# olasanni1/ETOL

Hardware: AMD Instinct MI355X
Metric: collocation-node constraint+Jacobian evals/sec, 6-state VGP N=1024 (higher is better)
Workload: dtype f64

## Files before the change

etol_amd/_lib.py:

```python
import ctypes as C
import os

import torch

_HERE = os.path.dirname(os.path.abspath(__file__))
LIB_PATH = os.path.join(_HERE, "lib", "libemi355x.so")

EMI_OK = 0
STATUS = {0: "EMI_OK", 1: "EMI_ERR_ARG", 2: "EMI_ERR_STATE", 3: "EMI_ERR_HIP",
          4: "EMI_ERR_NO_DEVICE", 5: "EMI_ERR_UNSUPPORTED", 6: "EMI_ERR_COMM"}

MODEL_POINTMASS2D, MODEL_QUADROTOR2D, MODEL_FIXEDWING12 = 0, 1, 2
MODEL_SOURCE = 100
PATH_ELLIPSE, PATH_DISC, PATH_TRACK = 0, 1, 2
PATH_REC = 8
EVAL_NODES, EVAL_DEFECT, EVAL_ALL, EVAL_NOJAC = 1, 2, 3, 4


class EmiError(RuntimeError):
    pass


class Layout(C.Structure):
    _fields_ = [("model", C.c_int), ("ns", C.c_int), ("nc", C.c_int), ("np", C.c_int),
                ("M", C.c_int), ("B", C.c_int), ("nres", C.c_int), ("nvals", C.c_int),
                ("nhess", C.c_int), ("real_bytes", C.c_int), ("px", C.c_int), ("py", C.c_int),
                ("t0", C.c_double), ("tf", C.c_double)]


class PassPlan(C.Structure):
    _fields_ = [(n, C.c_int) for n in ("one_launch", "sw", "ksplit", "ring_stages", "cpart", "cx", "mfma_workgroups", "store_mode",
                                       "block_order", "tiles16", "piece", "tail", "k_tile", "column_tiles", "k_halves")]


_P = C.c_void_p
_D = C.POINTER(C.c_double)
_I = C.POINTER(C.c_int)

SYMBOLS = {
    "emi_abi_version": (C.c_int, []),
    "emi_status_string": (C.c_char_p, [C.c_int]),
    "emi_device_count": (C.c_int, [_I]),
    "emi_lgl": (C.c_int, [C.c_int, _D, _D, _D]),
    "emi_model_dims": (C.c_int, [C.c_int, _I, _I, _I]),
    "emi_edge_ellipse": (C.c_int, [C.c_double] * 4 + [_D]),
    "emi_track_centres": (C.c_int, [C.c_int, _D, _D, _D, C.c_int, _D, _D, _D]),
    "emi_create": (C.c_int, [C.c_int, C.POINTER(_P)]),
    "emi_create_f32": (C.c_int, [C.c_int, C.POINTER(_P)]),
    "emi_destroy": (C.c_int, [_P]),
    "emi_last_error": (C.c_char_p, [_P]),
    "emi_set_stream": (C.c_int, [_P, _P]),
    "emi_get_stream": (C.c_int, [_P, C.POINTER(_P)]),
    "emi_synchronize": (C.c_int, [_P]),
    "emi_set_mesh": (C.c_int, [_P, C.c_int, _D, _D, _D, C.c_double, C.c_double]),
    "emi_set_model": (C.c_int, [_P, C.c_int, _D, C.c_int, C.c_int]),
    "emi_set_model_source": (C.c_int, [_P, C.c_char_p, C.c_char_p, C.c_int, C.c_int, C.c_int, _I, C.c_int, _D, C.c_int, C.c_int]),
    "emi_check_model_source": (C.c_int, [C.c_char_p, C.c_char_p, C.c_int, C.c_int, C.c_int, C.c_int, C.c_int, C.c_char_p, C.c_size_t]),
    "emi_kkt_factor": (C.c_int, [_P, _D, _D, C.POINTER(C.c_ubyte), C.c_double, C.POINTER(C.c_int)]),
    "emi_kkt_solve": (C.c_int, [_P, _D, C.c_int]),
    "emi_kkt_last_regularisation": (C.c_int, [_P, _D, _D]),
    "emi_kkt_factor_batch": (C.c_int, [C.c_int, C.POINTER(_P), C.POINTER(_D), C.POINTER(_D), C.POINTER(C.POINTER(C.c_ubyte)), _D, _I]),
    "emi_kkt_solve_batch": (C.c_int, [C.c_int, C.POINTER(_P), C.POINTER(_D)]),
    "emi_kkt_is_schur": (C.c_int, [_P]),
    "emi_kkt_solve_refined": (C.c_int, [_P, _D, C.c_double, C.c_int, _D, _I, _I, _I]),
    "emi_kkt_solve_refined_batch": (C.c_int, [C.c_int, C.POINTER(_P), C.POINTER(_D), _D, C.c_int, _D, _I, _I, _I]),
    "emi_kkt_lowrank": (C.c_int, [_P, C.c_int, C.POINTER(C.c_int), _D, _D, C.POINTER(C.c_int)]),
    "emi_set_batch": (C.c_int, [_P, C.c_int]),
    "emi_set_path": (C.c_int, [_P, C.c_int, C.c_int, _D, C.c_int, C.c_int]),
    "emi_set_tracks": (C.c_int, [_P, C.c_int, C.c_int, _D, _D]),
    "emi_get_layout": (C.c_int, [_P, C.POINTER(Layout)]),
    "emi_jac_structure": (C.c_int, [_P, _I, _I]),
    "emi_dev_alloc": (C.c_int, [_P, C.c_size_t, C.POINTER(_P)]),
    "emi_dev_free": (C.c_int, [_P, _P]),
    "emi_h2d": (C.c_int, [_P, _P, _P, C.c_size_t]),
    "emi_d2h": (C.c_int, [_P, _P, _P, C.c_size_t]),
    "emi_eval_dev": (C.c_int, [_P, _P, _P, _P, _P, _P, C.c_uint]),
    "emi_eval_host": (C.c_int, [_P, _D, _D, _D, _D, _D, C.c_uint]),
    "emi_hess_dev": (C.c_int, [_P, _P, _P, _P, _P, C.c_double, _P]),
    "emi_hess_host": (C.c_int, [_P, _D, _D, _D, _D, C.c_double, _D]),
    "emi_lagr_grad_dev": (C.c_int, [_P, _P, _P, _P, C.c_double, _P]),
    "emi_lagr_grad_host": (C.c_int, [_P, _D, _D, _D, C.c_double, _D]),
    "emi_kkt_certificate_dev": (C.c_int, [_P, _P, _P, _P, _P, _P, _P, C.c_double, _P, _P, C.c_int, _D, _D, _P, _P]),
    "emi_kkt_certificate_host": (C.c_int, [_P, _D, _D, _D, _D, C.c_double, _D, _D, C.c_int, _D, _D, _D, _D]),
    "emi_lagr_grad_total_dev": (C.c_int, [_P, _P, _P, _P, C.c_double, _P, _P]),
    "emi_lagr_grad_total_host": (C.c_int, [_P, _D, _D, _D, C.c_double, _D, _D]),
    "emi_kkt_certificate_total_dev": (C.c_int, [_P, _P, _P, _P, _P, _P, _P, C.c_double, _P, _P, C.c_int, _D, _D, _P, _P, _P]),
    "emi_kkt_certificate_total_host": (C.c_int, [_P, _D, _D, _D, _D, C.c_double, _D, _D, C.c_int, _D, _D, _D, _D, _D]),
    "emi_timer_start": (C.c_int, [_P]),
    "emi_timer_stop": (C.c_int, [_P, C.POINTER(C.c_float)]),
    "emi_profile_enable": (C.c_int, [_P, C.c_int]),
    "emi_profile_read": (C.c_int, [_P, C.POINTER(C.c_float), _I, C.POINTER(C.c_float), _I, C.POINTER(C.c_float), _I]),
    "emi_set_option": (C.c_int, [_P, C.c_char_p, C.c_int]),
    "emi_last_path": (C.c_int, [_P, _I]),
    "emi_plan_pass": (C.c_int, [_P, C.c_int, C.POINTER(PassPlan)]),
    "emi_last_defect_kernel": (C.c_char_p, [_P]),
    "emi_debug_pass_roles": (C.c_int, [C.c_int, C.c_int, C.c_int, C.POINTER(C.c_int), C.c_int]),
    "emi_debug_tile_order": (C.c_int, [C.c_int, C.c_int, C.c_int, C.c_int, C.c_int, C.POINTER(C.c_int), C.c_int, C.POINTER(C.c_int), C.POINTER(C.c_int), C.POINTER(C.c_int)]),
    "emi_set_delays": (C.c_int, [_P, C.c_int, C.c_int, C.c_double]),
    "emi_get_delays": (C.c_int, [_P, _I, _I, _I]),
    "emi_delay_matrix": (C.c_int, [C.c_int, C.POINTER(C.c_double), C.POINTER(C.c_double), C.c_double, C.c_double, C.c_double, C.POINTER(C.c_double)]),
    "emi_debug_tile_order2": (C.c_int, [C.c_int] * 7 + [C.POINTER(C.c_int), C.c_int, C.POINTER(C.c_int), C.POINTER(C.c_int), C.POINTER(C.c_int)]),
    "emi_comm_unique_id": (C.c_int, [_P]),
    "emi_comm_create": (C.c_int, [C.c_int, C.c_int, C.c_int, _P, C.POINTER(_P)]),
    "emi_comm_gather": (C.c_int, [_P, _P, _P, C.c_size_t, C.c_int, _P]),
    "emi_comm_destroy": (C.c_int, [_P]),
    "emi_comm_last_error": (C.c_char_p, [_P]),
}

_lib = None


def load():
    global _lib
    if _lib is not None:
        return _lib
    if not os.path.exists(LIB_PATH):
        raise EmiError(f"{LIB_PATH} is missing: run `python -c 'import __graft_entry__ as g; g.build()'` "
                       "(or `make lib`) first; there is no CPU fallback")
    lib = C.CDLL(LIB_PATH, mode=C.RTLD_GLOBAL)
    for name, (res, args) in SYMBOLS.items():
        fn = getattr(lib, name)
        fn.restype = res
        fn.argtypes = args
    _lib = lib
    return lib


def check(status, ctx=None, what=""):
    if status == EMI_OK:
        return
    lib = load()
    msg = lib.emi_status_string(status).decode()
    if ctx:
        detail = lib.emi_last_error(ctx).decode()
        if detail:
            msg += ": " + detail
    raise EmiError(f"{what or 'libemi355x'}: {STATUS.get(status, status)} ({msg})")
```

etol_amd/csrc/emi_api.hip:

```cpp
#include <hip/hip_runtime.h>

#include <algorithm>
#include <cstdarg>
#include <cstdio>
#include <cstring>
#include <string>
#include <vector>

#include "emi355x.h"
#include "emi_device_array.hpp"
#include "emi_kernels.hpp"

namespace {

using DevBuf = emi::DeviceArray<unsigned char>;

enum ProfMark { E0, E1, E2, K0, K1, K2, K3, PROF_MARKS };
struct ProfEvents {
    hipEvent_t ev[PROF_MARKS] = {};
    bool has_node = false, has_defect = false, fused = false;
    int level = 0;
};

}

struct emi_ctx_s {
    int device = 0;
    bool f32 = false;
    hipStream_t stream = nullptr;
    bool own_stream = false;
    hipStream_t stream2 = nullptr;
    hipEvent_t ev_fork = nullptr, ev_join = nullptr, ev_join2 = nullptr;
    int cu_split = 0;
    hipStream_t s_mfma = nullptr, s_node = nullptr;
    std::string err;
    std::string last_defect_kernel;

    int M = 0;
    double t0 = 0, tf = 0;
    DevBuf d_w, d_t, d_Ddiag, d_D, d_De, d_Do;
    bool symmetric = false;
    bool points_only = false;
    int allow_fused = 1;
    int sym_ct = 0;
    int sym_order = 1;
    int sym_ablate = 0;
    int small_rows = 24;
    int overlap_mode = 0;
    int node_store = -1;
    unsigned fused_attr_mask = 0;
    std::vector<double> h_tau, h_w;
    int model = -1, ns = 0, nc = 0, maximize = 0;
    double params[EMI_MAX_PARAMS] = {0};
    emi::KktWorkspace* kkt = nullptr;
    int kkt_method = 1;
    emi::RtcModel* rtc = nullptr;
    int B = 0;
    int np = 0, path_sets = 0, px = 0, py = 1;
    int np_model = 0;
    std::vector<int> pvars;
    DevBuf d_path;
    int ntracks = 0, track_sets = 0;
    DevBuf d_trkx, d_trky;
    DevBuf d_cost_part;
    DevBuf d_slab;
    DevBuf d_tile_ticket;
    DevBuf d_cost_part2;
    DevBuf d_ticket;
    int cost_in_kernel = 1;
    int sym_nst = 3;
    int sym_hs = 0;
    int sym_ctc = 0;
    int sym_bk = 0;
    int xh = 0, uh = 0, nch = 0;
    double delay_dt = 0.0;
    bool delay_dirty = true;
    DevBuf d_W;
    bool adjw_dirty = true;
    DevBuf d_adjWT;
    DevBuf d_adj_Gx;
    int adj_fold_tile = 0;
    DevBuf d_uext;
    int f32_ring_wgs = 2;
    int f32_ring = 1;
    int f32_one_launch = 0;
    int slice = 0;
    int sym_ksplit = 0;
    int sym_cpart = 0;
    int sym_gblk = 0, sym_cx = 0;
    int pass_order = -1;
    int sym_combine = 1;
    DevBuf s_X, s_U, s_RES, s_VALS, s_COST, s_LF, s_LC, s_H;
    DevBuf d_adjDT;
    bool adj_dirty = true;
    DevBuf d_adj_pvars;
    std::vector<int> adj_pvars;
    DevBuf d_adj_c;
    DevBuf d_adj_G;
    DevBuf d_adj_op;
    DevBuf s_G, s_cert, s_zl, s_zu, s_Gdel;
    hipEvent_t t_start = nullptr, t_stop = nullptr;
    int profile = 0;
    std::vector<ProfEvents> prof;
    size_t prof_used = 0;
    bool attr_set = false;

    ~emi_ctx_s() {
        (void)hipSetDevice(device);
        if (stream) (void)hipStreamSynchronize(stream);
        for (ProfEvents& pe : prof)
            for (hipEvent_t e : pe.ev)
                if (e) (void)hipEventDestroy(e);
        for (hipStream_t s : {stream2, s_mfma, s_node})
            if (s) { (void)hipStreamSynchronize(s); (void)hipStreamDestroy(s); }
        for (hipEvent_t e : {ev_join2, ev_fork, ev_join, t_start, t_stop})
            if (e) (void)hipEventDestroy(e);
        if (own_stream && stream) (void)hipStreamDestroy(stream);
        emi::rtc_destroy(rtc);
        emi::kkt_destroy(kkt);
    }
};

namespace {

int fail(emi_ctx_t c, int code, const char* fmt, ...) {
    char buf[512];
    va_list ap;
    va_start(ap, fmt);
    vsnprintf(buf, sizeof buf, fmt, ap);
    va_end(ap);
    if (c) c->err = buf;
    return code;
}

#define HIP_TRY(c, call)                                                              \
    do {                                                                              \
        hipError_t e_ = (call);                                                       \
        if (e_ != hipSuccess)                                                         \
            return fail((c), EMI_ERR_HIP, "%s failed: %s (%s:%d)", #call,             \
                        hipGetErrorString(e_), __FILE__, __LINE__);                   \
    } while (0)

#define EMI_TRY(call)              \
    do {                           \
        const int st_ = (call);    \
        if (st_) return st_;       \
    } while (0)

int ensure(emi_ctx_t c, DevBuf& b, size_t bytes) {
    HIP_TRY(c, b.reserve(bytes));
    return EMI_OK;
}

int ensure_zeroed(emi_ctx_t c, DevBuf& b, size_t bytes, hipStream_t s) {
    if (b.bytes() >= bytes) return EMI_OK;
    EMI_TRY(ensure(c, b, bytes));
    HIP_TRY(c, hipMemsetAsync(b.p, 0, bytes, s));
    return EMI_OK;
}

int upload_bytes(emi_ctx_t c, DevBuf& b, const void* src, size_t bytes) {
    EMI_TRY(ensure(c, b, bytes));
    if (bytes == 0) return EMI_OK;
    HIP_TRY(c, hipMemcpyAsync(b.p, src, bytes, hipMemcpyHostToDevice, c->stream));
    HIP_TRY(c, hipStreamSynchronize(c->stream));
    return EMI_OK;
}

int upload_real(emi_ctx_t c, DevBuf& b, const double* src, size_t n) {
    if (!c->f32) return upload_bytes(c, b, src, n * 8);
    std::vector<float> tmp(n);
    for (size_t i = 0; i < n; ++i) tmp[i] = (float)src[i];
    return upload_bytes(c, b, tmp.data(), n * 4);
}

int download_real(emi_ctx_t c, double* dst, const void* dsrc, size_t n) {
    if (!dst || n == 0) return EMI_OK;
    std::vector<float> tmp(c->f32 ? n : 0);
    HIP_TRY(c, hipMemcpyAsync(c->f32 ? (void*)tmp.data() : (void*)dst, dsrc, n * (c->f32 ? 4 : 8), hipMemcpyDeviceToHost, c->stream));
    HIP_TRY(c, hipStreamSynchronize(c->stream));
    for (size_t i = 0; i < tmp.size(); ++i) dst[i] = tmp[i];
    return EMI_OK;
}

bool overlapped_path(emi_ctx_t c) {
    if (c->f32 || !c->allow_fused || !c->symmetric || c->M <= 0 || c->model < 0) return false;
    if (c->model == EMI_MODEL_SOURCE) return emi::rtc_has_symdefect(c->rtc) && c->M % 128 == 0;
    return emi::fused_supported(c->model, c->M, c->sym_ct);
}

bool pass_takes_small_batches(emi_ctx_t c, int B) {
    if (!overlapped_path(c) || (c->overlap_mode != 0 && c->overlap_mode != 3) || c->M % 128 != 0) return false;
    if (c->rtc) return emi::rtc_pass_supported(c->rtc, B, c->M, 1, 1, 0);
    const emi::SymPlan p = emi::plan_symdefect(c->ns, B, c->M, 7, 1, c->sym_cpart, c->sym_gblk, c->sym_cx);
    return emi::pass_supported(c->model, c->ns, B, c->M, p);
}

int np_total(emi_ctx_t c) { return c->np + c->np_model; }
int nvals_of(emi_ctx_t c) { return c->ns * (c->ns + c->nc) + 2 * c->np + c->np_model * (int)c->pvars.size() + (c->ns + c->nc); }
int nres_of(emi_ctx_t c) { return c->ns + np_total(c); }
int nhess_of(emi_ctx_t c) { const int nv = c->ns + c->nc; return nv * (nv + 1) / 2; }

int ready(emi_ctx_t c) {
    if (!c) return EMI_ERR_ARG;
    if (c->M <= 0) return fail(c, EMI_ERR_STATE, "emi_set_mesh has not been called");
    if (c->model < 0) return fail(c, EMI_ERR_STATE, "emi_set_model has not been called");
    if (c->B <= 0) return fail(c, EMI_ERR_STATE, "emi_set_batch has not been called");
    if (c->np > 0 && c->path_sets != 1 && c->path_sets != c->B)
        return fail(c, EMI_ERR_STATE, "path table has %d sets, batch is %d", c->path_sets, c->B);
    if (c->ntracks > 0 && c->track_sets != 1 && c->track_sets != c->B)
        return fail(c, EMI_ERR_STATE, "track table has %d sets, batch is %d", c->track_sets, c->B);
    return EMI_OK;
}

int store_mode_for(emi_ctx_t c, int B) {
    if (c->node_store >= 0) return c->node_store;
    if ((size_t)B * (nvals_of(c) + nres_of(c)) * c->M * (c->f32 ? 4 : 8) > ((size_t)230 << 20)) return 2;
    const int tiles16 = ((B + 15) / 16) * (c->M / 128);
    if (tiles16 > 16 && tiles16 <= 32) return 0;
    return (!c->rtc && !c->f32) ? 1 : 0;
}

struct PassPlan {
    bool one_launch = false;
    emi::SymPlan sym;
    int tiles16 = 0;
    int store_mode = 0;
    int mfma_first = 0;
};

PassPlan plan_pass(emi_ctx_t c, int B, bool jac) {
    PassPlan p;
    p.tiles16 = ((B + 15) / 16) * (c->M / 128);
    p.store_mode = store_mode_for(c, B);
    const bool auto_mode = c->overlap_mode == 0;
    if (!((c->overlap_mode == 3 || auto_mode) && jac) || c->M % 128 != 0) return p;
    const bool auto_ct = auto_mode && (c->sym_ct == 0 || c->sym_ct == 4);
    const int gblk = (c->sym_gblk == 0 && c->sym_cpart == 0 && B > 2048 && B % 256 == 0) ? 2 : c->sym_gblk;
    const int gblk_first = (auto_ct || c->rtc) ? gblk : c->sym_gblk;
    int ct = c->sym_ct;
    const bool deep_base = auto_ct && !c->rtc && c->sym_bk == 0 && c->sym_ksplit == 0 && c->sym_nst == 3;
    const bool deep_mid = deep_base && c->ns % 2 == 0 && c->ns > 2 && p.tiles16 >= 49 && p.tiles16 < 128;
    const bool deep_small = deep_base && c->ns % 2 == 0 && c->ns > 2 && p.tiles16 >= 33 && p.tiles16 < 49;
    if (c->rtc) ct = (p.store_mode == 2 && emi::rtc_pass_sw_large(c->rtc) == 2) ? 6 : 7;
    else if (auto_ct) ct = (p.tiles16 < 128 && !deep_mid) ? 7 : 6;
    emi::SymPlan plan = emi::plan_symdefect(c->ns, B, c->M, ct, 1, c->sym_cpart, gblk_first, c->sym_cx);
    if (plan.ring1) plan = emi::plan_symdefect(c->ns, B, c->M, 5, 1, c->sym_cpart, c->sym_gblk, c->sym_cx);
    int ks_want = c->sym_ksplit;
    if (ks_want == 0 && auto_ct && !deep_mid && !deep_small) ks_want = plan.tiles * 4 <= 256 ? 4 : (plan.tiles * 2 <= 512 ? 2 : 1);
    if (ks_want > 1) {
        const int ct_now = plan.sw == c->ns ? 5 : (plan.sw == 2 ? 6 : (plan.sw == 3 ? 8 : 7));
        plan = emi::plan_symdefect(c->ns, B, c->M, ct_now, ks_want, c->sym_cpart, c->rtc ? gblk : c->sym_gblk, c->sym_cx);
    } else {
        plan.ks = 1;
    }
    plan.nst = c->rtc ? 3 : c->sym_nst;
    const bool deep_large = auto_ct && !c->rtc && c->sym_bk == 0 && c->sym_nst == 3 && c->pass_order < 0 && p.tiles16 >= 208 && p.tiles16 <= 1024;
    const bool deep_band = auto_ct && !c->rtc && c->sym_bk == 0 && c->sym_nst == 3 && c->pass_order < 0 && c->ns % 2 == 0 && c->ns > 2 &&
                           p.tiles16 >= 144 && p.tiles16 < 208;
    const int bk_want = c->sym_bk ? c->sym_bk : ((deep_mid || deep_small || deep_large || deep_band) ? 16 : 8);
    if (bk_want == 16 && !c->rtc && plan.ks == 1 && (plan.sw == 1 || plan.sw == 2) && plan.nst == 3) plan.bk = 16;
    const bool wide_large = auto_ct && c->sym_ctc == 0 && B > 2048 && B % 256 == 0 && c->sym_cpart == 0;
    const int ctc_want = c->sym_ctc ? c->sym_ctc : (wide_large ? 2 : 1);
    if (ctc_want == 2 && !c->rtc && plan.ks == 1 && plan.sw == 2 && plan.nst == 3 && c->M % 256 == 0) {
        const int bk_keep = plan.bk;
        plan = emi::plan_symdefect(c->ns, B, c->M, 6, 1, c->sym_cpart, gblk_first, (wide_large && c->sym_cx == 0) ? 1 : c->sym_cx, bk_keep, 2);
        plan.ks = 1;
        plan.nst = 3;
        plan.bk = bk_keep;
    }
    const int hs_want = c->sym_hs ? c->sym_hs : 1;
    if (hs_want == 2 && !c->rtc && plan.ks == 1 && plan.ct == 1 && (plan.sw == 1 || plan.sw == 2) && plan.nst == 3 &&
        ((c->M / 2) / plan.bk) % 4 == 0)
        plan.hs = 2;
    p.sym = plan;
    p.mfma_first = c->pass_order >= 0 ? c->pass_order
                                      : (deep_band ? 150 : (p.tiles16 < 208 ? 1 : (p.tiles16 < 384 ? 125 : (p.tiles16 < 768 ? 110 : 0))));
    p.one_launch = c->rtc ? emi::rtc_pass_supported(c->rtc, B, c->M, plan.sw, plan.ks, p.store_mode)
                          : emi::pass_supported(c->model, c->ns, B, c->M, plan);
    return p;
}

int plan_piece(emi_ctx_t c, int B) {
    const long long cap = ((0xFFFFFFFFLL / ((long long)c->ns * c->M * 8)) / 256) * 256;
    int piece = 0;
    if (c->slice > 0) { if (B > 2 * c->slice) piece = c->slice; }
    else if (B > 2048) piece = (int)std::min<long long>(cap > 0 ? cap : 256, B - B % 256);
    return piece >= B ? 0 : piece;
}

struct Launch { int first, B; };
struct PassIO { const void *X, *U; void *RES, *VALS, *COST; };

PassIO io_at(emi_ctx_t c, const PassIO& io, int first) {
    const size_t row = (size_t)first * c->M * (c->f32 ? 4 : 8);
    return PassIO{(const char*)io.X + row * c->ns, (const char*)io.U + row * c->nc, (char*)io.RES + row * nres_of(c),
                  io.VALS ? (char*)io.VALS + row * nvals_of(c) : nullptr, (char*)io.COST + (size_t)first * (c->f32 ? 4 : 8)};
}

template <typename T>
void fill_node_args(emi_ctx_t c, Launch L, emi::NodeArgs<T>& a, const PassIO& io) {
    a.X = (const T*)io.X;
    a.U = (const T*)io.U;
    a.RES = (T*)io.RES;
    a.VALS = (T*)io.VALS;
    a.cost_part = (T*)c->d_cost_part.p + (size_t)L.first * emi::node_chunks(c->M);
    a.cost = (T*)io.COST;
    a.cost_ticket = nullptr;
    a.w = (const T*)c->d_w.p;
    a.node_t = (const T*)c->d_t.p;
    a.Ddiag = (const T*)c->d_Ddiag.p;
    a.path = (const T*)c->d_path.p + (c->path_sets > 1 ? (size_t)L.first * c->np * EMI_PATH_REC : 0);
    a.track_x = (const T*)c->d_trkx.p + (c->track_sets > 1 ? (size_t)L.first * c->ntracks * c->M : 0);
    a.track_y = (const T*)c->d_trky.p + (c->track_sets > 1 ? (size_t)L.first * c->ntracks * c->M : 0);
    a.M = c->M;
    a.B = L.B;
    a.np = np_total(c);
    a.nres = nres_of(c);
    a.nvals = nvals_of(c);
    a.path_sets = c->path_sets;
    a.track_sets = c->track_sets;
    a.ntracks = c->ntracks;
    a.px = c->px;
    a.py = c->py;
    a.store_mode = store_mode_for(c, L.B);
    a.h = (T)((c->tf - c->t0) / 2.0);
    a.sgn = c->maximize ? T(-1) : T(1);
    for (int i = 0; i < EMI_MAX_PARAMS; ++i) a.P.p[i] = (T)c->params[i];
}

void delay_matrix(const std::vector<double>& tau, const std::vector<double>& w, double t0, double tf, double delay, double* W) {
    const int M = (int)tau.size();
    std::vector<double> lam(M);
    for (int j = 0; j < M; ++j) lam[j] = ((j & 1) ? -1.0 : 1.0) * std::sqrt(w[j]);
    const double hh = (tf - t0) / 2.0;
    for (int k = 0; k < M; ++k) {
        double ts = t0 + hh * (tau[k] + 1.0) - delay;
        if (ts < t0) ts = t0;
        const double x = (ts - t0) / hh - 1.0;
        double* row = W + (size_t)k * M;
        int hit = -1;
        for (int j = 0; j < M; ++j)
            if (x == tau[j]) hit = j;
        if (ts <= t0) hit = 0;
        if (hit >= 0) {
            for (int j = 0; j < M; ++j) row[j] = j == hit ? 1.0 : 0.0;
            continue;
        }
        double den = 0.0;
        for (int j = 0; j < M; ++j) {
            row[j] = lam[j] / (x - tau[j]);
            den += row[j];
        }
        for (int j = 0; j < M; ++j) row[j] /= den;
    }
}

int ensure_delay_matrices(emi_ctx_t c) {
    if (!c->delay_dirty) return EMI_OK;
    const int M = c->M, nd = std::max(c->xh - 1, c->uh);
    std::vector<double> W((size_t)nd * M * M);
    for (int d = 0; d < nd; ++d) delay_matrix(c->h_tau, c->h_w, c->t0, c->tf, (d + 1) * c->delay_dt, W.data() + (size_t)d * M * M);
    EMI_TRY(upload_real(c, c->d_W, W.data(), W.size()));
    c->delay_dirty = false;
    return EMI_OK;
}

int extend_controls(emi_ctx_t c, const void* dX, const void* dU_free, const void** dU_ext) {
    if (c->f32) return fail(c, EMI_ERR_UNSUPPORTED, "delayed values: f64 contexts only");
    if (c->points_only) return fail(c, EMI_ERR_STATE, "delayed values need a collocation mesh (this context holds a points-only mesh)");
    const int M = c->M, ncf = c->nc - c->nch;
    HIP_TRY(c, hipSetDevice(c->device));
    if (!c->attr_set) {
        HIP_TRY(c, emi::defect_f64_set_attr());
        c->attr_set = true;
    }
    int st;
    if ((st = ensure_delay_matrices(c))) return st;
    const size_t row = (size_t)M * 8;
    if ((st = ensure(c, c->d_uext, (size_t)c->B * c->nc * row))) return st;
    HIP_TRY(c, hipMemsetAsync(c->d_uext.p, 0, (size_t)c->B * c->nc * row, c->stream));
    HIP_TRY(c, hipMemcpy2DAsync(c->d_uext.p, (size_t)c->nc * row, dU_free, (size_t)ncf * row, (size_t)ncf * row, c->B, hipMemcpyDeviceToDevice, c->stream));
    double* base = (double*)c->d_uext.p + (size_t)ncf * M;
    for (int i = 1; i < c->xh; ++i) {
        emi::DefectArgs a{(const double*)dX, (const double*)c->d_W.p + (size_t)(i - 1) * M * M, base + (size_t)(i - 1) * c->ns * M,
                          c->B * c->ns, M, c->ns, c->nc};
        HIP_TRY(c, emi::launch_defect_f64(a, c->stream));
    }
    base += (size_t)std::max(c->xh - 1, 0) * c->ns * M;
    for (int i = 1; i <= c->uh; ++i) {
        emi::DefectArgs a{(const double*)dU_free, (const double*)c->d_W.p + (size_t)(i - 1) * M * M, base + (size_t)(i - 1) * ncf * M,
                          c->B * ncf, M, ncf, c->nc};
        HIP_TRY(c, emi::launch_defect_f64(a, c->stream));
    }
    *dU_ext = c->d_uext.p;
    return EMI_OK;
}

struct OptionRow {
    const char* name;
    int emi_ctx_s::*member;
    bool (*accepts)(int);
    int (*stored)(int);
    const char* message;
};
template <int LO, int HI> bool within(int v) { return v >= LO && v <= HI; }
template <int... VS> bool one_of(int v) { return ((v == VS) || ...); }
bool any_value(int) { return true; }
bool at_least_0(int v) { return v >= 0; }
bool whole_tiles(int v) { return v >= 0 && v % 16 == 0; }
int as_given(int v) { return v; }
int as_flag(int v) { return v != 0; }
int ring_wgs(int v) { return v == 1 ? 1 : 2; }
int block_order(int v) { return v < 0 ? -1 : (v >= 100 ? v : (v != 0)); }

const OptionRow OPTIONS[] = {
    {"overlap", &emi_ctx_s::allow_fused, any_value, as_flag, nullptr},
    {"fused", &emi_ctx_s::allow_fused, any_value, as_flag, nullptr},
    {"sym_ct", &emi_ctx_s::sym_ct, within<0, 8>, as_given,
     "sym_ct must be 0..8 (0/4 = chosen from the batch, 3 = LDS-DMA ring, 5..8 = state-split ring with SW = NS/2/1/3)"},
    {"small_rows", &emi_ctx_s::small_rows, at_least_0, as_given, "small_rows must be >= 0 (0 disables the skinny defect kernel)"},
    {"sym_order", &emi_ctx_s::sym_order, any_value, as_flag, nullptr},
    {"f32_ring", &emi_ctx_s::f32_ring, any_value, as_flag, nullptr},
    {"f32_ring_wgs", &emi_ctx_s::f32_ring_wgs, any_value, ring_wgs, nullptr},
    {"f32_one_launch", &emi_ctx_s::f32_one_launch, any_value, as_flag, nullptr},
    {"slice", &emi_ctx_s::slice, whole_tiles, as_given, "slice must be 0 (never) or a multiple of 16 instances"},
    {"pass_order", &emi_ctx_s::pass_order, any_value, block_order, nullptr},
    {"sym_ablate", &emi_ctx_s::sym_ablate, any_value, as_given, nullptr},
    {"adj_fold_tile", &emi_ctx_s::adj_fold_tile, within<0, 2>, as_given, "adj_fold_tile must be 0 (by size), 1 (48 x 64) or 2 (96 x 128)"},
    {"cost_in_kernel", &emi_ctx_s::cost_in_kernel, any_value, as_flag, nullptr},
    {"sym_nst", &emi_ctx_s::sym_nst, one_of<3, 4>, as_given, "sym_nst must be 3 or 4"},
    {"sym_hs", &emi_ctx_s::sym_hs, within<0, 2>, as_given, "sym_hs must be 0 (by batch size), 1 or 2"},
    {"sym_ctc", &emi_ctx_s::sym_ctc, within<0, 2>, as_given, "sym_ctc must be 0 (by batch size), 1 or 2"},
    {"sym_bk", &emi_ctx_s::sym_bk, one_of<0, 8, 16>, as_given, "sym_bk must be 0 (by batch size), 8 or 16"},
    {"sym_cpart", &emi_ctx_s::sym_cpart, one_of<-1, 0, 1, 2, 4, 8>, as_given, "sym_cpart must be -1 (plain order), 0 (by mesh size), 1, 2, 4 or 8"},
    {"sym_gblk", &emi_ctx_s::sym_gblk, within<0, 64>, as_given, "sym_gblk must be 0 (off) .. 64 instance groups per super-block"},
    {"sym_cx", &emi_ctx_s::sym_cx, within<0, 64>, as_given, "sym_cx must be 0 (default) .. 64 column tiles per block"},
    {"sym_combine", &emi_ctx_s::sym_combine, any_value, as_flag, nullptr},
    {"sym_ksplit", &emi_ctx_s::sym_ksplit, one_of<0, 1, 2, 4, 8>, as_given, "sym_ksplit must be 0 (by batch size), 1, 2, 4 or 8"},
    {"node_store", &emi_ctx_s::node_store, within<-1, 3>, as_given,
     "node_store must be -1 (by size), 0 (plain), 1 (write-through sc1), 2 (non-temporal) or 3 (nt sc1; the one-launch pass only)"},
    {"overlap_mode", &emi_ctx_s::overlap_mode, within<0, 3>, as_given,
     "overlap_mode must be 0 (by batch size), 1 (one stream), 2 (two streams) or 3 (one launch)"},
};


int need_stream2(emi_ctx_t c) {
    if (c->stream2) return EMI_OK;
    if (hipStreamCreateWithFlags(&c->stream2, hipStreamNonBlocking) != hipSuccess) {
        c->stream2 = nullptr;
        return fail(c, EMI_ERR_HIP, "cannot create the second stream of the two-stream pass");
    }
    return EMI_OK;
}

enum class Form {
    PassF64,
    TwoKernelF64,
    PassF32,
    TwoStreamF32,
    Sequential,
};
struct FormChoice {
    Form form = Form::Sequential;
    bool small = false;
    PassPlan plan;
    bool overlapped() const { return form == Form::PassF64 || form == Form::TwoKernelF64; }
};

FormChoice choose_form(emi_ctx_t c, Launch L, unsigned flags) {
    const bool nodes = flags & EMI_EVAL_NODES, defect = flags & EMI_EVAL_DEFECT, jac = !(flags & EMI_EVAL_NOJAC);
    FormChoice ch;
    ch.small = defect && !c->f32 && L.B > 0 && L.B * c->ns <= c->small_rows && emi::defect_small_supported(L.B * c->ns) &&
               !(nodes && jac && pass_takes_small_batches(c, L.B));
    if (nodes && defect && !ch.small && overlapped_path(c)) {
        ch.plan = plan_pass(c, L.B, jac);
        ch.form = ch.plan.one_launch ? Form::PassF64 : Form::TwoKernelF64;
    } else if (c->f32 && nodes && defect && jac && !c->rtc && c->allow_fused) {
        if ((c->overlap_mode == 3 || (c->overlap_mode == 0 && c->f32_one_launch)) && emi::pass_f32_supported(c->model, L.B * c->ns, c->M, L.B))
            ch.form = Form::PassF32;
        else if (c->overlap_mode == 2 && emi::defect_f32_mfma_supported(c->M))
            ch.form = Form::TwoStreamF32;
    }
    return ch;
}

int next_prof_record(emi_ctx_t c, ProfEvents** out) {
    if (c->prof_used == c->prof.size()) c->prof.emplace_back();
    ProfEvents& pe = c->prof[c->prof_used];
    for (hipEvent_t& e : pe.ev)
        if (!e) HIP_TRY(c, hipEventCreate(&e));
    ++c->prof_used;
    *out = &pe;
    return EMI_OK;
}

constexpr unsigned AT1 = 1u << 1, AT2 = 1u << 2, AT3 = 1u << 3, AT_ANY = AT1 | AT2 | AT3;
int prof_mark(emi_ctx_t c, ProfEvents* pe, ProfMark which, unsigned levels, hipStream_t s) {
    if (pe && pe->level > 0 && ((levels >> pe->level) & 1u)) HIP_TRY(c, hipEventRecord(pe->ev[which], s));
    return EMI_OK;
}

const char* const NAME_PASS_F32 = "emi_pass_f32_kernel (MFMA + node roles, one launch)";
const char* const NAME_RING1_F64 = "emi_symdefect_ring_f64_kernel";
const char* name_defect_f32(emi_ctx_t c, bool mfma) {
    return !mfma ? "emi_defect_f32_kernel" : (c->f32_ring ? "emi_defect_f32_ring_kernel" : "emi_defect_f32_mfma_kernel");
}
const char* name_defect_f64(bool small) { return small ? "emi_defect_small_f64_kernel" : "emi_defect_f64_kernel"; }
std::string name_pass_f64(const emi::SymPlan& plan) {
    return "emi_pass_f64_kernel<SW=" + std::to_string(plan.sw) + "> (MFMA + node roles, one launch" +
           (plan.ks > 1 ? ", " + std::to_string(plan.ks) + " K slices per tile" : "") + ")" +
           (plan.bk == 16 ? " [K tiles of 16]" : "") + (plan.ct == 2 ? " [128-column tiles]" : "") + (plan.hs == 2 ? " [K range in two halves per workgroup]" : "");
}
std::string name_symdefect(emi_ctx_t c, const emi::SymPlan& plan, bool in_kernel_combine) {
    if (plan.ring1) return c->sym_ct == 1 || c->sym_ct == 2 ? "emi_symdefect_f64_kernel" : NAME_RING1_F64;
    return "emi_symdefect_ring2_f64_kernel<SW=" + std::to_string(plan.sw) + ">" +
           (plan.ks > 1 ? " x" + std::to_string(plan.ks) + (in_kernel_combine ? " K slices (in-kernel combine)" : " K slices + emi_symdefect_combine_kernel") : "");
}

emi::SymDefectArgs sym_defect_args(emi_ctx_t c, Launch L, const PassIO& io) {
    emi::SymDefectArgs sa;
    sa.X = (const double*)io.X;
    sa.U = (const double*)io.U;
    sa.RES = (double*)io.RES;
    sa.node_t = (const double*)c->d_t.p;
    sa.De = (const double*)c->d_De.p;
    sa.Do = (const double*)c->d_Do.p;
    sa.M = c->M;
    sa.B = L.B;
    sa.nres = nres_of(c);
    sa.h = (c->tf - c->t0) / 2.0;
    sa.order = c->sym_order;
    sa.ablate = c->sym_ablate;
    sa.ksplit = 1;
    sa.slab = nullptr;
    sa.tile_ticket = nullptr;
    sa.cpart = sa.cx = 0;
    sa.mfma_first = 0;
    for (int i = 0; i < EMI_MAX_PARAMS; ++i) sa.P.p[i] = c->params[i];
    return sa;
}

emi::DefectArgsF32 defect_args_f32(emi_ctx_t c, Launch L, const PassIO& io) {
    return emi::DefectArgsF32{(const float*)io.X, (const float*)c->d_D.p, (float*)io.RES, L.B * c->ns, c->M, c->ns, nres_of(c)};
}

int form_pass_f64(emi_ctx_t c, Launch L, const PassIO& io, const PassPlan& pp, ProfEvents* pe) {
    const emi::SymPlan& plan = pp.sym;
    emi::SymDefectArgs sa = sym_defect_args(c, L, io);
    emi::NodeArgs<double> na;
    fill_node_args(c, L, na, io);
    sa.mfma_first = pp.mfma_first;
    sa.cpart = plan.cpart;
    sa.cx = plan.cx;
    if (plan.ks > 1) {
        EMI_TRY(ensure(c, c->d_slab, plan.slab_bytes));
        EMI_TRY(ensure_zeroed(c, c->d_tile_ticket, (size_t)plan.tiles * 4, c->stream));
        sa.ksplit = plan.ks;
        sa.slab = (double*)c->d_slab.p;
        sa.tile_ticket = (unsigned*)c->d_tile_ticket.p;
    }
    EMI_TRY(ensure_zeroed(c, c->d_ticket, (size_t)L.B * 4, c->stream));
    na.cost_ticket = (unsigned*)c->d_ticket.p;
    EMI_TRY(prof_mark(c, pe, K0, AT_ANY, c->stream));
    if (c->rtc) HIP_TRY(c, emi::rtc_launch_pass(c->rtc, sa, na, plan.sw, c->stream));
    else HIP_TRY(c, emi::launch_pass(c->model, sa, na, c->stream, plan));
    EMI_TRY(prof_mark(c, pe, K1, AT_ANY, c->stream));
    if (pe) pe->level = -1;
    c->last_defect_kernel = name_pass_f64(plan);
    return EMI_OK;
}

int launch_symdefect_f64(emi_ctx_t c, Launch L, emi::SymDefectArgs& sa, hipStream_t s) {
    if (c->rtc) {
        HIP_TRY(c, emi::rtc_launch_symdefect(c->rtc, sa, s));
        c->last_defect_kernel = NAME_RING1_F64;
        return EMI_OK;
    }
    const emi::SymPlan plan = emi::plan_symdefect(c->ns, L.B, c->M, c->sym_ct, c->sym_ksplit, c->sym_cpart, c->sym_gblk, c->sym_cx);
    if (plan.slab_bytes) EMI_TRY(ensure(c, c->d_slab, plan.slab_bytes));
    sa.ksplit = plan.ring1 ? 1 : plan.ks;
    sa.slab = (double*)c->d_slab.p;
    sa.cpart = plan.cpart;
    sa.cx = plan.cx;
    if (sa.ksplit > 1 && c->sym_combine) {
        EMI_TRY(ensure_zeroed(c, c->d_tile_ticket, (size_t)plan.tiles * 4, s));
        sa.tile_ticket = (unsigned*)c->d_tile_ticket.p;
    }
    const unsigned bit = 1u << c->sym_ct;
    HIP_TRY(c, emi::launch_symdefect(c->model, sa, s, !(c->fused_attr_mask & bit), c->sym_ct, plan));
    c->fused_attr_mask |= bit;
    c->last_defect_kernel = name_symdefect(c, plan, sa.tile_ticket != nullptr);
    return EMI_OK;
}

int form_two_kernel_f64(emi_ctx_t c, Launch L, const PassIO& io, bool jac, ProfEvents* pe) {
    emi::SymDefectArgs sa = sym_defect_args(c, L, io);
    emi::NodeArgs<double> na;
    fill_node_args(c, L, na, io);
    const bool two = c->overlap_mode != 1;
    const bool split = two && c->cu_split > 0;
    if (two && !split) EMI_TRY(need_stream2(c));
    hipStream_t s1 = split ? c->s_mfma : c->stream;
    hipStream_t s2 = split ? c->s_node : (two ? c->stream2 : c->stream);
    if (two) {
        HIP_TRY(c, hipEventRecord(c->ev_fork, c->stream));
        HIP_TRY(c, hipStreamWaitEvent(s2, c->ev_fork, 0));
        if (split) HIP_TRY(c, hipStreamWaitEvent(s1, c->ev_fork, 0));
    }
    EMI_TRY(prof_mark(c, pe, K0, AT1 | AT2, s1));
    EMI_TRY(launch_symdefect_f64(c, L, sa, s1));
    EMI_TRY(prof_mark(c, pe, K1, AT1 | AT2, s1));
    if (c->cost_in_kernel) {
        EMI_TRY(ensure_zeroed(c, c->d_ticket, (size_t)L.B * 4, s2));
        na.cost_ticket = (unsigned*)c->d_ticket.p;
    }
    EMI_TRY(prof_mark(c, pe, K2, AT1 | AT3, s2));
    if (c->rtc && jac && na.store_mode == 2 && c->M % 2 == 0) HIP_TRY(c, emi::rtc_launch_nodes_nt(c->rtc, na, s2));
    else if (c->rtc) HIP_TRY(c, emi::rtc_launch_nodes<double>(c->rtc, na, jac, false, s2));
    else HIP_TRY(c, emi::launch_nodes<double>(c->model, na, jac, false, s2));
    EMI_TRY(prof_mark(c, pe, K3, AT1 | AT3, s2));
    if (!c->cost_in_kernel) HIP_TRY(c, emi::launch_cost_finish<double>(na.cost_part, na.cost, L.B, emi::node_chunks(c->M), na.sgn * na.h, s2));
    if (two) {
        HIP_TRY(c, hipEventRecord(c->ev_join, s2));
        HIP_TRY(c, hipStreamWaitEvent(c->stream, c->ev_join, 0));
        if (split) {
            HIP_TRY(c, hipEventRecord(c->ev_join2, s1));
            HIP_TRY(c, hipStreamWaitEvent(c->stream, c->ev_join2, 0));
        }
    }
    EMI_TRY(prof_mark(c, pe, E1, AT1, c->stream));
    EMI_TRY(prof_mark(c, pe, E2, AT1, c->stream));
    return EMI_OK;
}

int form_pass_f32(emi_ctx_t c, Launch L, const PassIO& io, ProfEvents* pe) {
    emi::NodeArgs<float> na;
    fill_node_args(c, L, na, io);
    const size_t rowb = (size_t)c->M * 4;
    HIP_TRY(c, hipMemset2DAsync(io.RES, (size_t)nres_of(c) * rowb, 0, (size_t)c->ns * rowb, L.B, c->stream));
    EMI_TRY(ensure_zeroed(c, c->d_ticket, (size_t)L.B * 4, c->stream));
    na.cost_ticket = (unsigned*)c->d_ticket.p;
    EMI_TRY(prof_mark(c, pe, K0, AT_ANY, c->stream));
    HIP_TRY(c, emi::launch_pass_f32(c->model, defect_args_f32(c, L, io), na, c->pass_order >= 0 ? c->pass_order : 0, c->stream));
    EMI_TRY(prof_mark(c, pe, K1, AT_ANY, c->stream));
    if (pe) { pe->level = -1; pe->fused = true; }
    c->last_defect_kernel = NAME_PASS_F32;
    return EMI_OK;
}

int form_two_stream_f32(emi_ctx_t c, Launch L, const PassIO& io, ProfEvents* pe) {
    emi::NodeArgs<float> pre, full;
    PassIO values_only = io;
    values_only.VALS = nullptr;
    fill_node_args(c, L, pre, values_only);
    fill_node_args(c, L, full, io);
    EMI_TRY(ensure(c, c->d_cost_part2, (size_t)L.B * emi::node_chunks(c->M) * 4));
    EMI_TRY(need_stream2(c));
    pre.cost_part = (float*)c->d_cost_part2.p;
    pre.np = 0;
    const bool fork_late = c->f32_ring_wgs == 1;
    if (!fork_late) {
        HIP_TRY(c, hipEventRecord(c->ev_fork, c->stream));
        HIP_TRY(c, hipStreamWaitEvent(c->stream2, c->ev_fork, 0));
    }
    HIP_TRY(c, emi::launch_nodes<float>(c->model, pre, false, true, c->stream));
    if (fork_late) {
        HIP_TRY(c, hipEventRecord(c->ev_fork, c->stream));
        HIP_TRY(c, hipStreamWaitEvent(c->stream2, c->ev_fork, 0));
    }
    EMI_TRY(prof_mark(c, pe, K0, AT1 | AT2, c->stream));
    HIP_TRY(c, emi::launch_defect_f32_mfma(defect_args_f32(c, L, io), c->stream, c->f32_ring, c->f32_ring_wgs));
    EMI_TRY(prof_mark(c, pe, K1, AT1 | AT2, c->stream));
    c->last_defect_kernel = name_defect_f32(c, true);
    EMI_TRY(prof_mark(c, pe, K2, AT1 | AT3, c->stream2));
    HIP_TRY(c, emi::launch_nodes<float>(c->model, full, true, false, c->stream2));
    EMI_TRY(prof_mark(c, pe, K3, AT1 | AT3, c->stream2));
    HIP_TRY(c, emi::launch_cost_finish<float>(full.cost_part, full.cost, L.B, emi::node_chunks(c->M), full.sgn * full.h, c->stream2));
    HIP_TRY(c, hipEventRecord(c->ev_join, c->stream2));
    HIP_TRY(c, hipStreamWaitEvent(c->stream, c->ev_join, 0));
    if (pe) pe->fused = true;
    EMI_TRY(prof_mark(c, pe, E1, AT1, c->stream));
    EMI_TRY(prof_mark(c, pe, E2, AT1, c->stream));
    return EMI_OK;
}

template <typename T>
int launch_nodes_alone(emi_ctx_t c, Launch L, const PassIO& io, bool jac) {
    emi::NodeArgs<T> a;
    fill_node_args(c, L, a, io);
    if (c->rtc) HIP_TRY(c, emi::rtc_launch_nodes<T>(c->rtc, a, jac, true, c->stream));
    else HIP_TRY(c, emi::launch_nodes<T>(c->model, a, jac, true, c->stream));
    HIP_TRY(c, emi::launch_cost_finish<T>(a.cost_part, a.cost, L.B, emi::node_chunks(c->M), a.sgn * a.h, c->stream));
    return EMI_OK;
}

int form_sequential(emi_ctx_t c, Launch L, const PassIO& io, unsigned flags, bool small, ProfEvents* pe) {
    const bool jac = !(flags & EMI_EVAL_NOJAC);
    if (flags & EMI_EVAL_NODES) EMI_TRY(c->f32 ? launch_nodes_alone<float>(c, L, io, jac) : launch_nodes_alone<double>(c, L, io, jac));
    EMI_TRY(prof_mark(c, pe, E1, AT_ANY, c->stream));
    if ((flags & EMI_EVAL_DEFECT) && c->f32) {
        const bool mfma = emi::defect_f32_mfma_supported(c->M) && c->allow_fused;
        if (mfma) HIP_TRY(c, emi::launch_defect_f32_mfma(defect_args_f32(c, L, io), c->stream, c->f32_ring, c->f32_ring_wgs));
        else HIP_TRY(c, emi::launch_defect_f32(defect_args_f32(c, L, io), c->stream));
        c->last_defect_kernel = name_defect_f32(c, mfma);
    } else if (flags & EMI_EVAL_DEFECT) {
        emi::DefectArgs a{(const double*)io.X, (const double*)c->d_D.p, (double*)io.RES, L.B * c->ns, c->M, c->ns, nres_of(c)};
        if (small) HIP_TRY(c, emi::launch_defect_small_f64(a, c->stream));
        else HIP_TRY(c, emi::launch_defect_f64(a, c->stream));
        c->last_defect_kernel = name_defect_f64(small);
    }
    EMI_TRY(prof_mark(c, pe, E2, AT1 | AT2, c->stream));
    return EMI_OK;
}

int eval_launch(emi_ctx_t c, Launch L, const PassIO& io, unsigned flags) {
    const bool nodes = flags & EMI_EVAL_NODES, defect = flags & EMI_EVAL_DEFECT;
    const bool jac = !(flags & EMI_EVAL_NOJAC);
    if (!nodes && !defect) return fail(c, EMI_ERR_ARG, "emi_eval: empty flags");
    if (defect && c->points_only) return fail(c, EMI_ERR_STATE, "emi_eval: the mesh has no differentiation matrix (points-only mesh): EMI_EVAL_NODES only");
    if (!io.X || !io.RES || (nodes && (!io.U || !io.COST || (jac && !io.VALS))))
        return fail(c, EMI_ERR_ARG, "emi_eval: null device pointer");
    HIP_TRY(c, hipSetDevice(c->device));
    if (!c->attr_set) {
        HIP_TRY(c, emi::defect_f64_set_attr());
        c->attr_set = true;
    }
    const FormChoice ch = choose_form(c, L, flags);
    ProfEvents* pe = nullptr;
    if (c->profile) {
        EMI_TRY(next_prof_record(c, &pe));
        pe->has_node = nodes;
// ... 815 lines not shown
    emi::kkt_last_regularisation(c->kkt, dc, dw);
    return EMI_OK;
}

int emi_kkt_solve(emi_ctx_t c, double* rhs, int nrhs) {
    if (!c || !rhs || nrhs < 1) return EMI_ERR_ARG;
    HIP_TRY(c, hipSetDevice(c->device));
    std::string err;
    const int st = emi::kkt_solve(c->kkt, c->stream, (c->ns + c->nc) * c->M, rhs, nrhs, &err);
    if (st) c->err = err;
    return st;
}

int emi_timer_start(emi_ctx_t c) {
    if (!c) return EMI_ERR_ARG;
    HIP_TRY(c, hipEventRecord(c->t_start, c->stream));
    return EMI_OK;
}

int emi_timer_stop(emi_ctx_t c, float* ms) {
    if (!c || !ms) return EMI_ERR_ARG;
    HIP_TRY(c, hipEventRecord(c->t_stop, c->stream));
    HIP_TRY(c, hipEventSynchronize(c->t_stop));
    HIP_TRY(c, hipEventElapsedTime(ms, c->t_start, c->t_stop));
    return EMI_OK;
}

int emi_profile_enable(emi_ctx_t c, int on) {
    if (!c) return EMI_ERR_ARG;
    HIP_TRY(c, hipStreamSynchronize(c->stream));
    c->profile = (on >= 0 && on <= 3) ? on : 1;
    c->prof_used = 0;
    return EMI_OK;
}

int emi_profile_read(emi_ctx_t c, float* node_ms, int* node_launches, float* defect_ms,
                     int* defect_launches, float* pass_ms, int* overlapped_passes) {
    if (!c) return EMI_ERR_ARG;
    HIP_TRY(c, hipStreamSynchronize(c->stream));
    if (c->stream2) HIP_TRY(c, hipStreamSynchronize(c->stream2));
    float nm = 0, dm = 0, fm = 0;
    int nl = 0, dl = 0, fl = 0;
    for (size_t i = 0; i < c->prof_used; ++i) {
        ProfEvents& pe = c->prof[i];
        float ms = 0;
        if (pe.fused && pe.level == -1) {
            HIP_TRY(c, hipEventElapsedTime(&ms, pe.ev[K0], pe.ev[K1]));
            dm += ms; ++dl; fm += ms; ++fl;
            continue;
        }
        if (pe.fused) {
            if (pe.level == 1) {
                HIP_TRY(c, hipEventElapsedTime(&ms, pe.ev[E0], pe.ev[E1]));
                fm += ms;
            }
            ++fl;
            if (pe.level == 1 || pe.level == 2) {
                HIP_TRY(c, hipEventElapsedTime(&ms, pe.ev[K0], pe.ev[K1]));
                dm += ms;
                ++dl;
            }
            if (pe.level == 1 || pe.level == 3) {
                HIP_TRY(c, hipEventElapsedTime(&ms, pe.ev[K2], pe.ev[K3]));
                nm += ms;
                ++nl;
            }
            continue;
        }
        if (pe.has_node && pe.level != 2) {
            HIP_TRY(c, hipEventElapsedTime(&ms, pe.ev[E0], pe.ev[E1]));
            nm += ms;
            ++nl;
        }
        if (pe.has_defect && pe.level != 3) {
            HIP_TRY(c, hipEventElapsedTime(&ms, pe.ev[E1], pe.ev[E2]));
            dm += ms;
            ++dl;
        }
    }
    c->prof_used = 0;
    if (node_ms) *node_ms = nm;
    if (node_launches) *node_launches = nl;
    if (defect_ms) *defect_ms = dm;
    if (defect_launches) *defect_launches = dl;
    if (pass_ms) *pass_ms = fm;
    if (overlapped_passes) *overlapped_passes = fl;
    return EMI_OK;
}

int emi_set_option(emi_ctx_t c, const char* name, int value) {
    if (!c || !name) return EMI_ERR_ARG;
    if (strcmp(name, "cu_split") == 0) {
        hipDeviceProp_t prop;
        HIP_TRY(c, hipGetDeviceProperties(&prop, c->device));
        const int ncu = prop.multiProcessorCount;
        if (value < 0 || value >= ncu) return fail(c, EMI_ERR_ARG, "cu_split must be in [0, %d)", ncu);
        HIP_TRY(c, hipStreamSynchronize(c->stream));
        if (c->s_mfma) { HIP_TRY(c, hipStreamDestroy(c->s_mfma)); c->s_mfma = nullptr; }
        if (c->s_node) { HIP_TRY(c, hipStreamDestroy(c->s_node)); c->s_node = nullptr; }
        c->cu_split = value;
        if (value > 0) {
            const int words = (ncu + 31) / 32;
            std::vector<uint32_t> m1(words, 0u), m2(words, 0u);
            for (int i = 0; i < ncu; ++i) (i < value ? m1 : m2)[i / 32] |= 1u << (i % 32);
            HIP_TRY(c, hipExtStreamCreateWithCUMask(&c->s_mfma, words, m1.data()));
            HIP_TRY(c, hipExtStreamCreateWithCUMask(&c->s_node, words, m2.data()));
            if (!c->ev_join2) HIP_TRY(c, hipEventCreateWithFlags(&c->ev_join2, hipEventDisableTiming));
        }
        return EMI_OK;
    }
    if (strcmp(name, "kkt_method") == 0) {
        if (value != 0 && value != 1) return fail(c, EMI_ERR_ARG, "kkt_method must be 0 (LU) or 1 (Schur complement + Cholesky)");
        c->kkt_method = value;
        return EMI_OK;
    }
    if (strncmp(name, "kkt_", 4) == 0) {
        if (strcmp(name, "kkt_cholesky") == 0 && value != 1 && value != 2)
            return fail(c, EMI_ERR_ARG, "kkt_cholesky must be 1 (one-level blocked Cholesky) or 2 (two-level form from 1024 rows)");
        if (emi::kkt_set_option(name, value)) return EMI_OK;
        return fail(c, EMI_ERR_ARG, "unknown option %s", name);
    }
    for (const OptionRow& o : OPTIONS) {
        if (strcmp(name, o.name) != 0) continue;
        if (!o.accepts(value)) return fail(c, EMI_ERR_ARG, "%s", o.message);
        c->*o.member = o.stored(value);
        return EMI_OK;
    }
    return fail(c, EMI_ERR_ARG, "unknown option '%s'", name);
}

int emi_plan_pass(emi_ctx_t c, int B, emi_pass_plan_t* out) {
    if (!c || !out || B < 1) return EMI_ERR_ARG;
    if (c->M <= 0 || c->model < 0) return fail(c, EMI_ERR_STATE, "emi_plan_pass: mesh and model must be set");
    memset(out, 0, sizeof *out);
    const int piece = (!c->f32 && overlapped_path(c)) ? plan_piece(c, B) : 0;
    const int first = piece > 0 ? piece : B;
    out->piece = piece;
    out->tail = piece > 0 ? B % piece : 0;
    if (!c->f32 && overlapped_path(c)) {
        const PassPlan p = plan_pass(c, first, true);
        out->one_launch = p.one_launch ? 1 : 0;
        out->sw = p.sym.sw;
        out->ksplit = p.sym.ks;
        out->ring_stages = p.sym.nst;
        out->k_tile = p.sym.bk;
        out->column_tiles = p.sym.ct;
        out->k_halves = p.sym.hs;
        out->cpart = p.sym.cpart;
        out->cx = p.sym.cx;
        out->mfma_workgroups = p.sym.tiles * p.sym.ks;
        out->store_mode = p.store_mode;
        out->block_order = p.mfma_first;
        out->tiles16 = p.tiles16;
    }
    return EMI_OK;
}

int emi_last_path(emi_ctx_t c, int* fused) {
    if (!c || !fused) return EMI_ERR_ARG;
    *fused = choose_form(c, Launch{0, c->B}, EMI_EVAL_ALL).overlapped() ? 1 : 0;
    return EMI_OK;
}

int emi_debug_pass_roles(int nm, int nn, int order, int* out_role, int out_cap) {
    if (nm < 0 || nn < 0 || nm + nn < 1 || !out_role || out_cap < nm + nn) return EMI_ERR_ARG;
    for (int j = 0; j < nm + nn; ++j) {
        const emi::PassRole r = emi::pass_role_of(j, nm, nn, order);
        out_role[j] = r.mfma ? r.index : -1 - r.index;
    }
    return EMI_OK;
}

int emi_debug_tile_order(int ns, int B, int M, int sym_ct, int sym_cpart, int* out_tile, int out_cap, int* ntiles_total, int* cpart,
                         int* cx) {
    return emi_debug_tile_order2(ns, B, M, sym_ct, sym_cpart, 0, 0, out_tile, out_cap, ntiles_total, cpart, cx);
}

int emi_debug_tile_order2(int ns, int B, int M, int sym_ct, int sym_cpart, int sym_gblk, int sym_cx, int* out_tile, int out_cap,
                          int* ntiles_total, int* cpart, int* cx) {
    if (ns < 1 || B < 1 || M < 128 || M % 128 != 0 || !ntiles_total) return EMI_ERR_ARG;
    const emi::SymPlan p = emi::plan_symdefect(ns, B, M, sym_ct, 1, sym_cpart, sym_gblk, sym_cx);
    if (p.ring1 || p.sw < 1) return EMI_ERR_UNSUPPORTED;
    const int ntiles = (M / 2) / 64, ngrp = ((B + 15) / 16) * (ns / p.sw), total = ntiles * ngrp;
    *ntiles_total = total;
    if (cpart) *cpart = p.cpart;
    if (cx) *cx = p.cx;
    for (int t = 0; t < total && t < out_cap && out_tile; ++t) {
        const emi::RingTile rt = emi::ring_tile_of(t, ntiles, ngrp, p.cpart, p.cx, ns / p.sw);
        out_tile[t] = rt.ntile + ntiles * rt.grp;
    }
    return EMI_OK;
}

const char* emi_last_defect_kernel(emi_ctx_t c) {
    if (!c) return "";
    return c->last_defect_kernel.c_str();
}

}
```

etol_amd/csrc/emi_kernels.hpp:

```cpp
#pragma once
#include <hip/hip_runtime.h>
#include <stddef.h>

#include <string>

#include "emi355x.h"
#include "emi_args.hpp"

static_assert(EMI_PATH_ELLIPSE == 0 && EMI_PATH_DISC == 1 && EMI_PATH_TRACK == 2 && EMI_PATH_REC == 8,
              "emi_args.hpp and emi355x.h disagree");

namespace emi {

int node_chunks(int M);
template <typename T>
hipError_t launch_nodes(int model, const NodeArgs<T>& a, bool jac, bool defect_rows, hipStream_t s);
template <typename T> hipError_t launch_hess(int model, const HessArgs<T>& a, hipStream_t s);
hipError_t launch_defect_f64(const DefectArgs& a, hipStream_t s);
bool defect_small_supported(int R);
hipError_t launch_defect_small_f64(const DefectArgs& a, hipStream_t s);
hipError_t launch_defect_f32(const DefectArgsF32& a, hipStream_t s);
bool defect_f32_mfma_supported(int M);
hipError_t launch_defect_f32_mfma(const DefectArgsF32& a, hipStream_t s, int ring = 0, int wgs_per_cu = 2);
bool pass_f32_supported(int model, int R, int M, int B);
hipError_t launch_pass_f32(int model, const DefectArgsF32& d, const NodeArgs<float>& n, int order, hipStream_t s);
hipError_t defect_f64_set_attr();
template <typename T>
hipError_t launch_cost_finish(const T* part, T* cost, int B, int nchunks, T scale, hipStream_t s);
bool fused_supported(int model, int M, int ct);
struct SymPlan {
    bool ring1 = false;
    int sw = 0;
    int ks = 1;
    int nst = 3;
    int bk = 8;
    int hs = 1;
    int ct = 1;
    size_t slab_bytes = 0;
    int cpart = 0, cx = 0;
    int tiles = 0;
};
SymPlan plan_symdefect(int ns, int B, int M, int ct, int ksplit_opt, int cpart_opt = 0, int gblk_opt = 0, int cx_opt = 0, int bk_opt = 8, int ct_cols = 1);
hipError_t launch_symdefect(int model, const SymDefectArgs& a, hipStream_t s, bool set_attr, int ct, const SymPlan& plan);
bool pass_supported(int model, int ns, int B, int M, const SymPlan& plan);
hipError_t launch_pass(int model, const SymDefectArgs& sa, const NodeArgs<double>& na, hipStream_t s, const SymPlan& plan);

struct AdjointArgs {
    const double* VALS;
    const double* lamF;
    const double* lamC;
    const double* DT;
    const int* pvars;
    double* G;
    int B, M, ldt, ns, nc, np_table, np_traced, pw, px, py, nvals;
    int add_op;
    double sigma;
};
struct CertArgs {
    const double *X, *U, *RES, *VALS, *lamF, *lamC, *G;
    const double *zl, *zu;
    const double *cl, *cu;
    double* cert;
    int B, M, ns, nc, np, nres, nvals, nsets;
    int ncg;
    double sigma;
};
struct AdjointOpArgs {
    const double* A;
    const double* Bop;
    const double* add;
    double* out;
    int R, rpi, M, ldt, nseg, ldb;
    int a_inst, a_row0, a_seg, out_inst, out_row0, add_inst, add_row0;
};
hipError_t launch_adjoint_transpose(const double* dSrc, double* dDst, int M, int ldt, int ld_dst, int nseg, bool keep_diag, hipStream_t s);
bool adjoint_side_by_side(int B, int ns, int M);
hipError_t launch_adjoint_op(const AdjointArgs& a, hipStream_t s);
hipError_t launch_adjoint_product(const AdjointOpArgs& a, int tile, hipStream_t s);
hipError_t launch_adjoint_nodes(const AdjointArgs& a, hipStream_t s);
hipError_t launch_adjoint_add(const double* dGop, double* dG, int B, int ns, int nv, int M, hipStream_t s);
hipError_t launch_kkt_certificate(const CertArgs& a, hipStream_t s);

struct RtcModel;
int rtc_check(bool f32, const char* struct_name, const char* source, int ns, int nc, int npath, int pw, std::string* log);
int rtc_build(bool f32, const char* struct_name, const char* source, int ns, int nc, int npath, int pw, RtcModel** out, std::string* log);
void rtc_destroy(RtcModel* m);
bool rtc_has_symdefect(const RtcModel* m);
template <typename T>
hipError_t rtc_launch_nodes(RtcModel* m, const NodeArgs<T>& a, bool jac, bool defect_rows, hipStream_t s);
template <typename T> hipError_t rtc_launch_hess(RtcModel* m, const HessArgs<T>& a, hipStream_t s);
hipError_t rtc_launch_symdefect(RtcModel* m, const SymDefectArgs& a, hipStream_t s);
int rtc_pass_sw_large(const RtcModel* m);
bool rtc_pass_supported(const RtcModel* m, int B, int M, int sw, int ks, int store_mode);
hipError_t rtc_launch_pass(RtcModel* m, const SymDefectArgs& sa, const NodeArgs<double>& na, int sw, hipStream_t s);
hipError_t rtc_launch_nodes_nt(RtcModel* m, const NodeArgs<double>& a, hipStream_t s);

struct KktWorkspace;
int kkt_factor(KktWorkspace** w, hipStream_t stream, const double* dD, int M, int ns, int nv, const double* Qblk,
               const double* Jblk, const unsigned char* fixed, double dc, int method, int* info, std::string* err);
int kkt_solve(KktWorkspace* w, hipStream_t stream, int nz, double* rhs, int nrhs, std::string* err);
bool kkt_set_option(const char* name, int value);
int kkt_lowrank(KktWorkspace* w, hipStream_t stream, int nz, int r, const int* node, const double* vec, const double* delta,
                int* exact, std::string* err);
void kkt_destroy(KktWorkspace* w);
void kkt_last_regularisation(const KktWorkspace* w, double* dc, double* dw);
void kkt_mesh_changed(KktWorkspace* w);
bool kkt_is_schur(const KktWorkspace* w);
int kkt_factor_batch(int n, KktWorkspace** const* pws, hipStream_t stream, const double* const* dD, int M, int ns, int nv,
                     const double* const* Qblk, const double* const* Jblk, const unsigned char* const* fixed, const double* dc, int* info,
                     std::string* err);
int kkt_solve_batch(int n, KktWorkspace* const* ws, hipStream_t stream, int nz, double* const* rhs, std::string* err);
int kkt_solve_refined_batch(int n, KktWorkspace* const* ws, hipStream_t stream, double* const* rhs, const double* dc_nominal, int max_steps,
                            double* rel, int* nsolve, int* reverted, int* status, std::string* err);

}
```

etol_amd/csrc/emi_models.hpp:

```cpp
#pragma once
#ifndef __HIPCC_RTC__
#include <hip/hip_runtime.h>
#endif

namespace emi {

#define EMI_MAX_PARAMS 16
#define EMI_DEV __device__ __forceinline__

template <typename T> struct ModelParams { T p[EMI_MAX_PARAMS]; };

EMI_DEV void emi_sincos(double a, double* s, double* c) { sincos(a, s, c); }
EMI_DEV void emi_sincos(float a, float* s, float* c) { sincosf(a, s, c); }

EMI_DEV double emi_sin(double a) { return sin(a); }
EMI_DEV double emi_cos(double a) { return cos(a); }
EMI_DEV double emi_tan(double a) { return tan(a); }
EMI_DEV double emi_exp(double a) { return exp(a); }
EMI_DEV double emi_log(double a) { return log(a); }
EMI_DEV double emi_sqrt(double a) { return sqrt(a); }
EMI_DEV double emi_pow(double a, double c) { return pow(a, c); }
EMI_DEV float emi_sin(float a) { return sinf(a); }
EMI_DEV float emi_cos(float a) { return cosf(a); }
EMI_DEV float emi_tan(float a) { return tanf(a); }
EMI_DEV float emi_exp(float a) { return expf(a); }
EMI_DEV float emi_log(float a) { return logf(a); }
EMI_DEV float emi_sqrt(float a) { return sqrtf(a); }
EMI_DEV float emi_pow(float a, float c) { return powf(a, c); }

template <typename T> struct PointMass2D {
    static constexpr int NS = 2, NC = 2, NV = 4, NPARAM = 0, NPATH = 0;
    EMI_DEV static void f(const ModelParams<T>&, const T* z, T, T* fo) {
        fo[0] = z[2];
        fo[1] = z[3];
    }
    EMI_DEV static void jac(const ModelParams<T>&, const T*, T, T (*J)[NV]) {
        for (int i = 0; i < NS; ++i)
            for (int v = 0; v < NV; ++v) J[i][v] = T(0);
        J[0][2] = T(1);
        J[1][3] = T(1);
    }
    EMI_DEV static T cost(const ModelParams<T>&, const T* z, T) {
        return z[2] * z[2] + z[3] * z[3];
    }
    EMI_DEV static void grad(const ModelParams<T>&, const T* z, T, T* g) {
        g[0] = T(0); g[1] = T(0);
        g[2] = T(2) * z[2];
        g[3] = T(2) * z[3];
    }
    EMI_DEV static void hess(const ModelParams<T>&, const T*, T, T cL, const T*, T* H) {
        H[2 * 3 / 2 + 2] += T(2) * cL;
        H[3 * 4 / 2 + 3] += T(2) * cL;
    }
};

template <typename T> struct Quadrotor2D {
    static constexpr int NS = 6, NC = 2, NV = 8, NPARAM = 5, NPATH = 0;
    EMI_DEV static void f(const ModelParams<T>& P, const T* z, T, T* fo) {
        T s, c;
        emi_sincos(z[2], &s, &c);
        const T a = z[6] / P.p[0];
        fo[0] = z[3];
        fo[1] = z[4];
        fo[2] = z[5];
        fo[3] = -a * s;
        fo[4] = a * c - P.p[2];
        fo[5] = z[7] / P.p[1];
    }
    EMI_DEV static void jac(const ModelParams<T>& P, const T* z, T, T (*J)[NV]) {
        for (int i = 0; i < NS; ++i)
            for (int v = 0; v < NV; ++v) J[i][v] = T(0);
        T s, c;
        emi_sincos(z[2], &s, &c);
        const T im = T(1) / P.p[0];
        const T a = z[6] * im;
        J[0][3] = T(1);
        J[1][4] = T(1);
        J[2][5] = T(1);
        J[3][2] = -a * c;
        J[3][6] = -s * im;
        J[4][2] = -a * s;
        J[4][6] = c * im;
        J[5][7] = T(1) / P.p[1];
    }
    EMI_DEV static T cost(const ModelParams<T>& P, const T* z, T) {
        return P.p[3] * z[6] * z[6] + P.p[4] * z[7] * z[7];
    }
    EMI_DEV static void grad(const ModelParams<T>& P, const T* z, T, T* g) {
        for (int v = 0; v < 6; ++v) g[v] = T(0);
        g[6] = T(2) * P.p[3] * z[6];
        g[7] = T(2) * P.p[4] * z[7];
    }
    EMI_DEV static void hess(const ModelParams<T>& P, const T* z, T, T cL, const T* cf, T* H) {
        T s, c;
        emi_sincos(z[2], &s, &c);
        const T im = T(1) / P.p[0];
        const T a = z[6] * im;
        H[2 * 3 / 2 + 2] += cf[3] * (a * s) + cf[4] * (-a * c);
        H[6 * 7 / 2 + 2] += cf[3] * (-c * im) + cf[4] * (-s * im);
        H[6 * 7 / 2 + 6] += T(2) * P.p[3] * cL;
        H[7 * 8 / 2 + 7] += T(2) * P.p[4] * cL;
    }
};

template <typename T> struct FixedWing12 {
    static constexpr int NS = 12, NC = 4, NV = 16, NPARAM = 16, NPATH = 0;
    struct Pre {
        T sph, cph, sth, cth, sps, cps, tth, icth;
    };
    EMI_DEV static Pre pre(const T* z) {
        Pre q;
        emi_sincos(z[3], &q.sph, &q.cph);
        emi_sincos(z[4], &q.sth, &q.cth);
        emi_sincos(z[5], &q.sps, &q.cps);
        q.icth = T(1) / q.cth;
        q.tth = q.sth * q.icth;
        return q;
    }
    EMI_DEV static void f(const ModelParams<T>& P, const T* z, T, T* fo) {
        const Pre q = pre(z);
        const T u = z[6], v = z[7], w = z[8], p = z[9], qq = z[10], r = z[11];
        const T m = P.p[0], Ixx = P.p[1], Iyy = P.p[2], Izz = P.p[3], g = P.p[4];
        const T qS = P.p[5], iV = T(1) / P.p[13], damp = P.p[14];
        fo[0] = q.cth * q.cps * u + (q.sph * q.sth * q.cps - q.cph * q.sps) * v +
                (q.cph * q.sth * q.cps + q.sph * q.sps) * w;
        fo[1] = q.cth * q.sps * u + (q.sph * q.sth * q.sps + q.cph * q.cps) * v +
                (q.cph * q.sth * q.sps - q.sph * q.cps) * w;
        fo[2] = -q.sth * u + q.sph * q.cth * v + q.cph * q.cth * w;
        fo[3] = p + q.tth * (q.sph * qq + q.cph * r);
        fo[4] = q.cph * qq - q.sph * r;
        fo[5] = (q.sph * qq + q.cph * r) * q.icth;
        const T al = w * iV;
        const T CL = P.p[6] + P.p[7] * al;
        const T CD = P.p[8] + P.p[9] * CL * CL;
        const T X = z[12] - qS * CD;
        const T Y = -damp * v;
        const T Z = -qS * CL;
        fo[6] = r * v - qq * w - g * q.sth + X / m;
        fo[7] = p * w - r * u + g * q.sph * q.cth + Y / m;
        fo[8] = qq * u - p * v + g * q.cph * q.cth + Z / m;
        const T Lm = qS * P.p[10] * z[13] - damp * p;
        const T Mm = qS * P.p[11] * z[14] - damp * qq;
        const T Nm = qS * P.p[12] * z[15] - damp * r;
        fo[9] = ((Iyy - Izz) * qq * r + Lm) / Ixx;
        fo[10] = ((Izz - Ixx) * p * r + Mm) / Iyy;
        fo[11] = ((Ixx - Iyy) * p * qq + Nm) / Izz;
    }
    EMI_DEV static void jac(const ModelParams<T>& P, const T* z, T, T (*J)[NV]) {
        for (int i = 0; i < NS; ++i)
            for (int v = 0; v < NV; ++v) J[i][v] = T(0);
        const Pre q = pre(z);
        const T u = z[6], v = z[7], w = z[8], p = z[9], qq = z[10], r = z[11];
        const T m = P.p[0], Ixx = P.p[1], Iyy = P.p[2], Izz = P.p[3], g = P.p[4];
        const T qS = P.p[5], iV = T(1) / P.p[13], damp = P.p[14];
        const T r01 = q.sph * q.sth * q.cps - q.cph * q.sps;
        const T r02 = q.cph * q.sth * q.cps + q.sph * q.sps;
        const T r11 = q.sph * q.sth * q.sps + q.cph * q.cps;
        const T r12 = q.cph * q.sth * q.sps - q.sph * q.cps;
        J[0][3] = r02 * v - r01 * w;
        J[0][4] = -q.sth * q.cps * u + q.sph * q.cth * q.cps * v + q.cph * q.cth * q.cps * w;
        J[0][5] = -q.cth * q.sps * u - r11 * v - r12 * w;
        J[0][6] = q.cth * q.cps; J[0][7] = r01; J[0][8] = r02;
        J[1][3] = r12 * v - r11 * w;
        J[1][4] = -q.sth * q.sps * u + q.sph * q.cth * q.sps * v + q.cph * q.cth * q.sps * w;
        J[1][5] = q.cth * q.cps * u + r01 * v + r02 * w;
        J[1][6] = q.cth * q.sps; J[1][7] = r11; J[1][8] = r12;
        J[2][3] = q.cph * q.cth * v - q.sph * q.cth * w;
        J[2][4] = -q.cth * u - q.sph * q.sth * v - q.cph * q.sth * w;
        J[2][6] = -q.sth; J[2][7] = q.sph * q.cth; J[2][8] = q.cph * q.cth;
        const T sq = q.sph * qq + q.cph * r;
        const T cq = q.cph * qq - q.sph * r;
        J[3][3] = q.tth * cq;
        J[3][4] = sq * q.icth * q.icth;
        J[3][9] = T(1); J[3][10] = q.tth * q.sph; J[3][11] = q.tth * q.cph;
        J[4][3] = -sq;
        J[4][10] = q.cph; J[4][11] = -q.sph;
        J[5][3] = cq * q.icth;
        J[5][4] = sq * q.tth * q.icth;
        J[5][10] = q.sph * q.icth; J[5][11] = q.cph * q.icth;
        const T al = w * iV;
        const T CL = P.p[6] + P.p[7] * al;
        const T dCL = P.p[7] * iV;
        const T dCD = T(2) * P.p[9] * CL * dCL;
        J[6][4] = -g * q.cth;
        J[6][7] = r; J[6][8] = -qq - qS * dCD / m; J[6][10] = -w; J[6][11] = v;
        J[6][12] = T(1) / m;
        J[7][3] = g * q.cph * q.cth; J[7][4] = -g * q.sph * q.sth;
        J[7][6] = -r; J[7][7] = -damp / m; J[7][8] = p; J[7][9] = w; J[7][11] = -u;
        J[8][3] = -g * q.sph * q.cth; J[8][4] = -g * q.cph * q.sth;
        J[8][6] = qq; J[8][7] = -p; J[8][8] = -qS * dCL / m; J[8][9] = -v; J[8][10] = u;
        J[9][9] = -damp / Ixx; J[9][10] = (Iyy - Izz) * r / Ixx; J[9][11] = (Iyy - Izz) * qq / Ixx;
        J[9][13] = qS * P.p[10] / Ixx;
        J[10][9] = (Izz - Ixx) * r / Iyy; J[10][10] = -damp / Iyy; J[10][11] = (Izz - Ixx) * p / Iyy;
        J[10][14] = qS * P.p[11] / Iyy;
        J[11][9] = (Ixx - Iyy) * qq / Izz; J[11][10] = (Ixx - Iyy) * p / Izz; J[11][11] = -damp / Izz;
        J[11][15] = qS * P.p[12] / Izz;
    }
    EMI_DEV static T cost(const ModelParams<T>& P, const T* z, T) {
        return P.p[15] * (z[12] * z[12] + z[13] * z[13] + z[14] * z[14] + z[15] * z[15]);
    }
    EMI_DEV static void grad(const ModelParams<T>& P, const T* z, T, T* g) {
        for (int v = 0; v < 12; ++v) g[v] = T(0);
        for (int v = 12; v < 16; ++v) g[v] = T(2) * P.p[15] * z[v];
    }
    EMI_DEV static void hess(const ModelParams<T>& P, const T* z, T, T cL, const T* cf, T* H) {
        T cc[NS + 1];
        cc[0] = cL;
        for (int i = 0; i < NS; ++i) cc[1 + i] = cf[i];
        const T v16 = emi_sin(z[3]);
        const T v17 = emi_cos(z[3]);
// ... 198 lines not shown
        const T v734 = v730 + v733;
        const T v735 = v20 * v448;
        const T v736 = -v735;
        const T v737 = v21 * v685;
        const T v738 = v736 + v737;
        const T v739 = v18 * v724;
        const T v740 = -v739;
        const T v741 = v19 * v734;
        const T v742 = v740 + v741;
        const T v743 = v16 * v732;
        const T v744 = -v743;
        const T v745 = v17 * v729;
        const T v746 = v744 + v745;
        const T v748 = -cc[3];
        const T v749 = v20 * cc[2];
        const T v750 = v19 * cc[2];
        const T v751 = v21 * cc[1];
        const T v752 = v749 + v751;
        const T v753 = v19 * cc[1];
        const T v754 = v20 * v753;
        const T v755 = -v754;
        const T v756 = v21 * v750;
        const T v757 = v755 + v756;
        const T v758 = v18 * v752;
        const T v759 = -v758;
        const T v760 = v19 * v748;
        const T v761 = v759 + v760;
        const T v767 = v19 * cc[3];
        const T v768 = v16 * cc[3];
        const T v769 = v40 * cc[2];
        const T v770 = v21 * cc[2];
        const T v771 = v17 * cc[2];
        const T v772 = -cc[1];
        const T v773 = v40 * cc[1];
        const T v774 = v771 + v773;
        const T v775 = v758 + v767;
        const T v776 = v16 * v752;
        const T v777 = v20 * v772;
        const T v778 = v770 + v777;
        const T v779 = v17 * v772;
        const T v780 = v769 + v779;
        const T v781 = v20 * v774;
        const T v782 = -v781;
        const T v783 = v21 * v780;
        const T v784 = v782 + v783;
        const T v785 = v18 * v768;
        const T v786 = -v785;
        const T v787 = v19 * v776;
        const T v788 = v786 + v787;
        const T v789 = v16 * v778;
        const T v790 = -v789;
        const T v791 = v17 * v775;
        const T v792 = v790 + v791;
        const T v794 = v32 * P.p[7];
        const T v796 = P.p[9] * v794;
        const T v797 = v331 * v796;
        const T v799 = v331 * v794;
        const T v820 = P.p[9] * v799;
        const T v821 = v797 + v820;
        const T v824 = P.p[7] * v821;
        const T v827 = v32 * v824;
        const T v830 = v17 * cc[3];
        const T v831 = -cc[2];
        const T v832 = v35 * cc[2];
        const T v833 = v21 * v831;
        const T v834 = v16 * v831;
        const T v835 = v35 * cc[1];
        const T v836 = v834 + v835;
        const T v837 = v17 * v752;
        const T v838 = v20 * cc[1];
        const T v839 = v833 + v838;
        const T v840 = v16 * cc[1];
        const T v841 = v832 + v840;
        const T v846 = v20 * v836;
        const T v847 = -v846;
        const T v848 = v21 * v841;
        const T v849 = v847 + v848;
        const T v850 = v18 * v830;
        const T v851 = -v850;
        const T v852 = v19 * v837;
        const T v853 = v851 + v852;
        const T v854 = v16 * v775;
        const T v855 = -v854;
        const T v856 = v17 * v839;
        const T v857 = v855 + v856;
        const T v863 = v136 * v211;
        const T v869 = v141 * v203;
        const T v881 = v16 * cc[4];
        const T v883 = v16 * cc[6];
        const T v886 = v131 * v223;
        const T v906 = v23 * v881;
        const T v907 = v18 * v881;
        const T v908 = v883 + v907;
        const T v910 = v23 * v908;
        const T v911 = v910 / v19;
        const T v912 = -v911;
        const T v913 = v18 * v912;
        const T v914 = -v913;
        const T v915 = v19 * v906;
        const T v916 = v914 + v915;
        const T v917 = v16 * cc[5];
        const T v918 = -v917;
        const T v919 = v362 + v918;
        const T v920 = v17 * cc[4];
        const T v922 = v17 * cc[6];
        const T v943 = v23 * v920;
        const T v944 = v18 * v920;
        const T v945 = v922 + v944;
        const T v947 = v23 * v945;
        const T v948 = v947 / v19;
        const T v949 = -v948;
        const T v950 = v18 * v949;
        const T v951 = -v950;
        const T v952 = v19 * v943;
        const T v953 = v951 + v952;
        const T v954 = -v358;
        const T v955 = v533 + v954;
        const T v960 = v193 * T(2.00000000000000000e+00);
        H[9] += v571;
        H[13] += v684;
        H[14] += v680;
        H[18] += v746;
        H[19] += v742;
        H[20] += v738;
        H[25] += v761;
        H[26] += v757;
        H[31] += v792;
        H[32] += v788;
        H[33] += v784;
        H[39] += v857;
        H[40] += v853;
        H[41] += v849;
        H[44] += v827;
        H[52] += v267;
        H[53] += cc[8];
        H[58] += v919;
        H[59] += v916;
        H[61] += cc[9];
        H[63] += v301;
        H[64] += v869;
        H[69] += v955;
        H[70] += v953;
        H[72] += v282;
        H[73] += cc[7];
        H[75] += v863;
        H[76] += v886;
        H[90] += v960;
        H[104] += v960;
        H[119] += v960;
        H[135] += v960;
    }
};

}
```

etol_amd/csrc/emi_rtc.hip:

```cpp
#include <hip/hip_runtime.h>
#include <hip/hiprtc.h>

#include <cstdio>
#include <cstring>
#include <map>
#include <mutex>
#include <string>
#include <vector>

#include "emi_kernels.hpp"
#include "emi_rtc_sources.inc"

namespace emi {

struct RtcModel {
    hipModule_t mod = nullptr;
    hipFunction_t nodes[2][2][2] = {};
    hipFunction_t hess = nullptr;
    hipFunction_t ring = nullptr;
    hipFunction_t pass_small = nullptr;
    hipFunction_t pass_large = nullptr;
    hipFunction_t node_nt = nullptr;
    bool f32 = false;
    int ns = 0, nc = 0, sw_large = 0;
    size_t ring_lds = 0;
};

namespace {

bool valid_identifier(const char* s) {
    if (!s || !*s || (*s >= '0' && *s <= '9')) return false;
    for (; *s; ++s)
        if (!((*s >= 'a' && *s <= 'z') || (*s >= 'A' && *s <= 'Z') || (*s >= '0' && *s <= '9') || *s == '_')) return false;
    return true;
}

size_t ring_lds_bytes(int ns) { return (size_t)3 * (2 * ns * FUSED_TI + 2 * 64) * 16 * sizeof(double); }
bool ring_fits(int ns) { return ns <= 8 && ring_lds_bytes(ns) <= 160 * 1024; }

struct Names {
    std::string nodes[2][2][2], hess, ring, pass_small, pass_large, node_nt;
};
int pass_sw_large(int ns) { return (ns % 2 == 0 && ns > 2) ? 2 : 1; }

Names kernel_names(const char* sn, bool f32, bool with_ring, int ns) {
    Names n;
    const std::string T = f32 ? "float" : "double";
    const std::string model = std::string("emi::") + sn + "<" + T + ">";
    for (int v = 0; v < 2; ++v)
        for (int j = 0; j < 2; ++j)
            for (int d = 0; d < 2; ++d)
                n.nodes[v][j][d] = "emi::emi_nodes_kernel<" + T + ", " + model + ", " + (v ? "2" : "1") + ", " +
                                   (j ? "true" : "false") + ", " + (d ? "true" : "false") + ">";
    n.hess = "emi::emi_hess_kernel<" + T + ", " + model + ">";
    if (with_ring) {
        n.ring = "emi::emi_symdefect_ring_f64_kernel<" + model + ">";
        n.pass_small = "emi::emi_pass_f64_kernel<" + model + ", 1, 2, 0, 3>";
        n.pass_large = "emi::emi_pass_f64_kernel<" + model + ", " + std::to_string(pass_sw_large(ns)) + ", 2, 2, 3>";
        n.node_nt = "emi::emi_nodes_kernel<double, " + model + ", 2, true, false, 2>";
    }
    return n;
}

int compile(bool f32, const char* sn, const char* source, int ns, int nc, int npath, int pw, std::vector<char>* code,
            std::vector<std::string>* lowered, bool* has_ring, std::string* log) {
    if (!valid_identifier(sn) || !source || ns < 1 || nc < 0 || ns + nc > 64) {
        if (log) *log = "emi_set_model_source: bad struct name, null source or dimensions out of range";
        return EMI_ERR_ARG;
    }
    const bool with_ring = !f32 && ring_fits(ns);
    std::string prog = "#include \"emi_args.hpp\"\n#include \"emi_node_kernels.hpp\"\n";
    if (with_ring) prog += "#include \"emi_symdefect_kernels.hpp\"\n";
    prog += "namespace emi {\n";
    prog += source;
    prog += "\n}  // namespace emi\n";
    char chk[600];
    snprintf(chk, sizeof chk, "static_assert(emi::%s<double>::NS == %d && emi::%s<double>::NC == %d && emi::%s<double>::NV == %d && "
             "emi::%s<double>::NPATH == %d, \"model struct dimensions differ from emi_set_model_source(ns, nc, npath)\");\n", sn, ns,
             sn, nc, sn, ns + nc, sn, npath);
    prog += chk;
    if (npath > 0) {
        snprintf(chk, sizeof chk, "static_assert(emi::%s<double>::PW == %d, \"the model's traced rows depend on another number of "
                 "variables than emi_set_model_source(n_path_vars) says\");\n", sn, pw);
        prog += chk;
    }

    hiprtcProgram p;
    if (hiprtcCreateProgram(&p, prog.c_str(), "emi_model_program.hip", emi_rtc_nfiles, emi_rtc_texts, emi_rtc_names) !=
        HIPRTC_SUCCESS) {
        if (log) *log = "hiprtcCreateProgram failed";
        return EMI_ERR_HIP;
    }
    const Names nm = kernel_names(sn, f32, with_ring, ns);
    std::vector<const std::string*> order;
    for (int v = 0; v < 2; ++v)
        for (int j = 0; j < 2; ++j)
            for (int d = 0; d < 2; ++d) order.push_back(&nm.nodes[v][j][d]);
    order.push_back(&nm.hess);
    if (with_ring) {
        order.push_back(&nm.ring);
        order.push_back(&nm.pass_small);
        order.push_back(&nm.pass_large);
        order.push_back(&nm.node_nt);
    }
    for (const std::string* s : order) hiprtcAddNameExpression(p, s->c_str());

    const char* opts[] = {"--offload-arch=gfx950", "-O3", "-std=c++17", "-Wno-unused-function", "-Wno-inline-asm"};
    const hiprtcResult r = hiprtcCompileProgram(p, 5, opts);
    size_t ls = 0;
    hiprtcGetProgramLogSize(p, &ls);
    std::string l(ls, '\0');
    if (ls) hiprtcGetProgramLog(p, &l[0]);
    while (!l.empty() && l.back() == '\0') l.pop_back();
    if (r != HIPRTC_SUCCESS) {
        if (log) *log = std::string("model program does not compile (") + hiprtcGetErrorString(r) + "):\n" + l;
        hiprtcDestroyProgram(&p);
        return EMI_ERR_ARG;
    }
    if (log) *log = l;
    lowered->clear();
    for (const std::string* s : order) {
        const char* low = nullptr;
        if (hiprtcGetLoweredName(p, s->c_str(), &low) != HIPRTC_SUCCESS || !low) {
            if (log) *log = "no lowered name for " + *s;
            hiprtcDestroyProgram(&p);
            return EMI_ERR_HIP;
        }
        lowered->push_back(low);
    }
    size_t cs = 0;
    hiprtcGetCodeSize(p, &cs);
    code->resize(cs);
    hiprtcGetCode(p, code->data());
    hiprtcDestroyProgram(&p);
    *has_ring = with_ring;
    return EMI_OK;
}

hipError_t launch(hipFunction_t f, dim3 grid, dim3 block, size_t lds, hipStream_t s, const void* args, size_t bytes) {
    if (!f) return hipErrorInvalidDeviceFunction;
    void* config[] = {HIP_LAUNCH_PARAM_BUFFER_POINTER, const_cast<void*>(args), HIP_LAUNCH_PARAM_BUFFER_SIZE, &bytes,
                      HIP_LAUNCH_PARAM_END};
    return hipModuleLaunchKernel(f, grid.x, grid.y, grid.z, block.x, block.y, block.z, (unsigned)lds, s, nullptr,
                                 config);
}

}

int rtc_check(bool f32, const char* struct_name, const char* source, int ns, int nc, int npath, int pw, std::string* log) {
    std::vector<char> code;
    std::vector<std::string> low;
    bool ring = false;
    return compile(f32, struct_name, source, ns, nc, npath, pw, &code, &low, &ring, log);
}

namespace {
struct CachedProgram {
    std::vector<char> code;
    std::vector<std::string> lowered;
    bool ring = false;
};
std::mutex g_cache_mutex;
std::map<std::string, CachedProgram> g_cache;
}

int rtc_build(bool f32, const char* struct_name, const char* source, int ns, int nc, int npath, int pw, RtcModel** out,
              std::string* log) {
    *out = nullptr;
    std::vector<char> code;
    std::vector<std::string> low;
    bool ring = false;
    const std::string key = std::string(f32 ? "f32|" : "f64|") + (struct_name ? struct_name : "") + "|" + std::to_string(ns) + "|" +
                            std::to_string(nc) + "|" + std::to_string(npath) + "|" + (source ? source : "");
    bool hit = false;
    {
        std::lock_guard<std::mutex> lk(g_cache_mutex);
        auto it = g_cache.find(key);
        if (it != g_cache.end()) {
            code = it->second.code;
            low = it->second.lowered;
            ring = it->second.ring;
            hit = true;
        }
    }
    if (!hit) {
        const int st = compile(f32, struct_name, source, ns, nc, npath, pw, &code, &low, &ring, log);
        if (st) return st;
        std::lock_guard<std::mutex> lk(g_cache_mutex);
        CachedProgram& cp = g_cache[key];
        cp.code = code;
        cp.lowered = low;
        cp.ring = ring;
    }
    RtcModel* m = new RtcModel();
    m->f32 = f32;
    m->ns = ns;
    m->nc = nc;
    hipError_t e = hipModuleLoadData(&m->mod, code.data());
    size_t i = 0;
    for (int v = 0; v < 2 && e == hipSuccess; ++v)
        for (int j = 0; j < 2 && e == hipSuccess; ++j)
            for (int d = 0; d < 2 && e == hipSuccess; ++d) e = hipModuleGetFunction(&m->nodes[v][j][d], m->mod, low[i++].c_str());
    if (e == hipSuccess) e = hipModuleGetFunction(&m->hess, m->mod, low[i++].c_str());
    if (e == hipSuccess && ring) {
        e = hipModuleGetFunction(&m->ring, m->mod, low[i++].c_str());
        m->ring_lds = ring_lds_bytes(ns);
        if (e == hipSuccess) e = hipModuleGetFunction(&m->pass_small, m->mod, low[i++].c_str());
        if (e == hipSuccess) e = hipModuleGetFunction(&m->pass_large, m->mod, low[i++].c_str());
        if (e == hipSuccess) e = hipModuleGetFunction(&m->node_nt, m->mod, low[i++].c_str());
        m->sw_large = pass_sw_large(ns);
    }
    if (e != hipSuccess) {
        if (log) *log = std::string("loading the model code object failed: ") + hipGetErrorString(e);
        rtc_destroy(m);
        return EMI_ERR_HIP;
    }
    *out = m;
    return EMI_OK;
}

void rtc_destroy(RtcModel* m) {
    if (!m) return;
    if (m->mod) (void)hipModuleUnload(m->mod);
    delete m;
}

bool rtc_has_symdefect(const RtcModel* m) { return m && m->ring; }

template <typename T>
hipError_t rtc_launch_nodes(RtcModel* m, const NodeArgs<T>& a, bool jac, bool defect_rows, hipStream_t s) {
    const bool vec2 = a.M % 2 == 0;
    const int per_block = EMI_NODE_THREADS * (vec2 ? 2 : 1);
    dim3 grid((a.M + per_block - 1) / per_block, a.B), block(EMI_NODE_THREADS);
    return launch(m->nodes[vec2][jac][defect_rows], grid, block, 0, s, &a, sizeof a);
}
template hipError_t rtc_launch_nodes<double>(RtcModel*, const NodeArgs<double>&, bool, bool, hipStream_t);
template hipError_t rtc_launch_nodes<float>(RtcModel*, const NodeArgs<float>&, bool, bool, hipStream_t);

template <typename T> hipError_t rtc_launch_hess(RtcModel* m, const HessArgs<T>& a, hipStream_t s) {
    dim3 grid((a.M + EMI_NODE_THREADS - 1) / EMI_NODE_THREADS, a.B), block(EMI_NODE_THREADS);
    return launch(m->hess, grid, block, 0, s, &a, sizeof a);
}
template hipError_t rtc_launch_hess<double>(RtcModel*, const HessArgs<double>&, hipStream_t);
template hipError_t rtc_launch_hess<float>(RtcModel*, const HessArgs<float>&, hipStream_t);

hipError_t rtc_launch_symdefect(RtcModel* m, const SymDefectArgs& a, hipStream_t s) {
    const int mtiles = (a.B + FUSED_TI - 1) / FUSED_TI, ntiles = (a.M / 2) / 64;
    return launch(m->ring, dim3(mtiles * ntiles), dim3(256), m->ring_lds, s, &a, sizeof a);
}

int rtc_pass_sw_large(const RtcModel* m) { return m ? m->sw_large : 0; }

bool rtc_pass_supported(const RtcModel* m, int B, int M, int sw, int ks, int store_mode) {
    if (!m || !m->pass_small || ks < 1 || M % 128 != 0) return false;
    if (!((sw == 1 && store_mode != 2) || (sw == m->sw_large && store_mode == 2))) return false;
    return B >= 1 && m->ns % sw == 0;
}

hipError_t rtc_launch_pass(RtcModel* m, const SymDefectArgs& sa, const NodeArgs<double>& na, int sw, hipStream_t s) {
    PassArgs a;
    a.s = sa;
    a.n = na;
    const int mtiles = (sa.B + FUSED_TI - 1) / FUSED_TI, ntiles = (sa.M / 2) / 64;
    const int nm = mtiles * ntiles * (m->ns / sw) * (sa.ksplit > 1 ? sa.ksplit : 1);
    a.nbx = (na.M + 2 * EMI_NODE_THREADS - 1) / (2 * EMI_NODE_THREADS);
    const int nn = a.nbx * na.B;
    a.nm = nm;
    a.nn = nn;
    a.nm8 = (nm + 7) / 8;
    a.nn8 = (nn + 7) / 8;
    const size_t lds = (size_t)3 * ((2 * sw * FUSED_TI + 2 * 64 + 63) / 64 * 64) * 8 * sizeof(double);
    return launch(na.store_mode == 2 ? m->pass_large : m->pass_small, dim3(8 * (a.nm8 + a.nn8)), dim3(256), lds, s, &a, sizeof a);
}

hipError_t rtc_launch_nodes_nt(RtcModel* m, const NodeArgs<double>& a, hipStream_t s) {
    if (!m->node_nt || a.M % 2) return hipErrorInvalidDeviceFunction;
    dim3 grid((a.M + 2 * EMI_NODE_THREADS - 1) / (2 * EMI_NODE_THREADS), a.B), block(EMI_NODE_THREADS);
    return launch(m->node_nt, grid, block, 0, s, &a, sizeof a);
}

}
```

etol_amd/csrc/emi_symdefect.hip:

```cpp
#include <hip/hip_runtime.h>

#include <algorithm>

#include "emi_kernels.hpp"
#include "emi_models.hpp"
#include "emi_symdefect_kernels.hpp"

namespace emi {

template <class Model>
static hipError_t launch_symdefect_ring_model(const SymDefectArgs& a, hipStream_t s, bool set_attr) {
    constexpr int NS = Model::NS;
    const int mtiles = (a.B + FUSED_TI - 1) / FUSED_TI, ntiles = (a.M / 2) / 64;
    const size_t lds = (size_t)3 * (2 * NS * FUSED_TI + 2 * 64) * 16 * sizeof(double);
    if (set_attr) {
        hipError_t e = hipFuncSetAttribute((const void*)emi_symdefect_ring_f64_kernel<Model>,
                                           hipFuncAttributeMaxDynamicSharedMemorySize, (int)lds);
        if (e != hipSuccess) return e;
    }
    dim3 grid(mtiles * ntiles), block(256);
    hipLaunchKernelGGL((emi_symdefect_ring_f64_kernel<Model>), grid, block, lds, s, a);
    return hipGetLastError();
}

template <class Model, int CT>
static hipError_t launch_symdefect_model(const SymDefectArgs& a, hipStream_t s, bool set_attr) {
    constexpr int NS = Model::NS, TN = 64 * CT;
    const int mtiles = (a.B + FUSED_TI - 1) / FUSED_TI, ntiles = (a.M / 2) / TN;
    const size_t lds = (size_t)2 * (2 * NS * FUSED_TI + 2 * TN) * (FUSED_BK + 2) * sizeof(double);
    if (set_attr) {
        hipError_t e = hipFuncSetAttribute((const void*)emi_symdefect_f64_kernel<Model, CT>,
                                           hipFuncAttributeMaxDynamicSharedMemorySize, (int)lds);
        if (e != hipSuccess) return e;
    }
    dim3 grid(mtiles * ntiles), block(256);
    hipLaunchKernelGGL((emi_symdefect_f64_kernel<Model, CT>), grid, block, lds, s, a);
    return hipGetLastError();
}

template <class Model, int SW>
static hipError_t launch_ring2_model(const SymDefectArgs& a, hipStream_t s) {
    constexpr int NS = Model::NS;
    const int mtiles = (a.B + FUSED_TI - 1) / FUSED_TI, ntiles = (a.M / 2) / 64;
    const size_t lds = (size_t)3 * ((2 * SW * FUSED_TI + 2 * 64 + 63) / 64 * 64) * 8 * sizeof(double);
    static bool attr_done = false;
    if (!attr_done) {
        hipError_t e = hipFuncSetAttribute((const void*)emi_symdefect_ring2_f64_kernel<Model, SW>,
                                           hipFuncAttributeMaxDynamicSharedMemorySize, (int)lds);
        if (e != hipSuccess) return e;
        attr_done = true;
    }
    const int tiles = mtiles * ntiles * (NS / SW), ks = a.ksplit > 1 ? a.ksplit : 1;
    hipLaunchKernelGGL((emi_symdefect_ring2_f64_kernel<Model, SW>), dim3(tiles * ks), dim3(256), lds, s, a);
    if (ks > 1 && a.tile_ticket == nullptr) hipLaunchKernelGGL((emi_symdefect_combine_kernel<Model, SW>), dim3(tiles), dim3(256), 0, s, a);
    return hipGetLastError();
}

SymPlan plan_symdefect(int ns, int B, int M, int ct, int ksplit_opt, int cpart_opt, int gblk_opt, int cx_opt, int bk_opt, int ct_cols) {
    SymPlan p;
    p.bk = bk_opt == 16 ? 16 : 8;
    const int tiles = ((B + FUSED_TI - 1) / FUSED_TI) * ((M / 2) / 64);
    const int nkt = (M / 2) / p.bk;
    if (ct == 0 || ct == 4) {
        if (tiles >= 448) p.sw = (ns % 2 == 0 && ns > 2) ? 2 : ns;
        else if (tiles >= 320) p.sw = ns;
        else if (tiles >= 192) { p.ring1 = true; return p; }
        else p.sw = (tiles <= 96 || ns % 2 != 0 || ns <= 2) ? 1 : 2;
    } else if (ct >= 5 && ct <= 8) {
        p.sw = ct == 5 ? ns : (ct == 6 ? 2 : (ct == 8 ? 3 : 1));
        if (ns % p.sw != 0) p.sw = 1;
    } else {
        p.ring1 = true;
        return p;
    }
    if (ksplit_opt > 0) p.ks = ksplit_opt;
    while (p.ks > 1 && (nkt % p.ks != 0 || nkt / p.ks < 2 || (nkt / p.ks) % 2 != 0)) p.ks >>= 1;
    p.ct = (ct_cols == 2 && p.sw == 2 && p.ks == 1 && M % 256 == 0) ? 2 : 1;
    const int TNp = 64 * p.ct;
    p.tiles = (tiles / p.ct) * (ns / p.sw);
    {
        const int ntiles = (M / 2) / TNp, ngrp = ((B + FUSED_TI - 1) / FUSED_TI) * (ns / p.sw);
        const int target_cols = std::max(1, 4096 / M / p.ct);
        auto valid = [&](int cp) { return cp >= 1 && cp <= 8 && ntiles % cp == 0 && ngrp % (8 / cp) == 0 && (ngrp * ntiles) % 8 == 0; };
        int cp = 0;
        if (cpart_opt > 0) cp = valid(cpart_opt) ? cpart_opt : 0;
        else if (cpart_opt == 0 && tiles >= 192)
            for (int c = 1; c <= 8 && !cp; c *= 2)
                if (valid(c) && (ntiles / c <= target_cols || c == 8 || !valid(2 * c))) cp = c;
        const int mtiles = (B + FUSED_TI - 1) / FUSED_TI;
        if (gblk_opt > 0 && mtiles % (8 * gblk_opt) == 0 && (ngrp * ntiles) % 8 == 0) {
            int cxg = cx_opt > 0 ? cx_opt : 2;
            while (cxg > 1 && ntiles % cxg != 0) --cxg;
            p.cpart = -gblk_opt;
            p.cx = cxg;
        } else if (cp > 0) {
            p.cpart = cp;
            p.cx = 1;
            for (int d = 1; d <= std::min(ntiles / cp, target_cols); ++d)
                if ((ntiles / cp) % d == 0) p.cx = d;
            if (cp == 1 && p.cx == ntiles) p.cpart = p.cx = 0;
        }
    }
    if (p.ks > 1) p.slab_bytes = (size_t)p.tiles * p.ks * (2 * p.sw * 4) * 256 * sizeof(double);
    return p;
}

template <class Model>
static hipError_t launch_ring2_planned(const SymDefectArgs& a, hipStream_t s, const SymPlan& p) {
    constexpr int NS = Model::NS;
    if (p.sw == NS) return launch_ring2_model<Model, NS>(a, s);
    if constexpr (NS > 2 && NS % 2 == 0) {
        if (p.sw == 2) return launch_ring2_model<Model, 2>(a, s);
    }
    if constexpr (NS > 3 && NS % 3 == 0) {
        if (p.sw == 3) return launch_ring2_model<Model, 3>(a, s);
    }
    return launch_ring2_model<Model, 1>(a, s);
}

template <class Model, int SW, int NST, int BK = 8, int CT = 1, int HS = 1>
static hipError_t launch_pass_model(const SymDefectArgs& sa, const NodeArgs<double>& na, hipStream_t s) {
    constexpr int NS = Model::NS;
    PassArgs a;
    a.s = sa;
    a.n = na;
    const int mtiles = (sa.B + FUSED_TI - 1) / FUSED_TI, ntiles = (sa.M / 2) / (64 * CT);
    const int nm = mtiles * ntiles * (NS / SW) * (sa.ksplit > 1 ? sa.ksplit : 1);
    a.nbx = (na.M + 2 * EMI_NODE_THREADS - 1) / (2 * EMI_NODE_THREADS);
    const int nn = a.nbx * na.B;
    a.nm = nm;
    a.nn = nn;
    a.nm8 = (nm + 7) / 8;
    a.nn8 = ((nn + HS - 1) / HS + 7) / 8;
    const size_t lds = (size_t)HS * NST * ((2 * SW * FUSED_TI + 2 * 64 * CT + 63) / 64 * 64) * BK * sizeof(double);
    static bool attr_done[4] = {false, false, false, false};
    const int st = (na.store_mode >= 0 && na.store_mode <= 3) ? na.store_mode : 0;
    auto kern = st == 2 ? emi_pass_f64_kernel<Model, SW, 2, 2, NST, BK, CT, HS>
              : (st == 1 ? emi_pass_f64_kernel<Model, SW, 2, 1, NST, BK, CT, HS>
                         : (st == 3 ? emi_pass_f64_kernel<Model, SW, 2, 3, NST, BK, CT, HS> : emi_pass_f64_kernel<Model, SW, 2, 0, NST, BK, CT, HS>));
    if (!attr_done[st]) {
        hipError_t e = hipFuncSetAttribute((const void*)kern, hipFuncAttributeMaxDynamicSharedMemorySize, (int)lds);
        if (e != hipSuccess) return e;
        attr_done[st] = true;
    }
    hipLaunchKernelGGL(kern, dim3(8 * (a.nm8 + a.nn8)), dim3(256 * HS), lds, s, a);
    return hipGetLastError();
}

template <class Model>
static hipError_t launch_pass_planned(const SymDefectArgs& sa, const NodeArgs<double>& na, hipStream_t s, const SymPlan& p) {
    constexpr int NS = Model::NS;
    if (p.sw == NS) return launch_pass_model<Model, NS, 3>(sa, na, s);
    if constexpr (NS > 2 && NS % 2 == 0) {
        if (p.sw == 2 && p.hs == 2 && p.ct == 1) return p.bk == 16 ? launch_pass_model<Model, 2, 3, 16, 1, 2>(sa, na, s) : launch_pass_model<Model, 2, 3, 8, 1, 2>(sa, na, s);
        if (p.sw == 2 && p.ct == 2) return p.bk == 16 ? launch_pass_model<Model, 2, 3, 16, 2>(sa, na, s) : launch_pass_model<Model, 2, 3, 8, 2>(sa, na, s);
        if (p.sw == 2 && p.bk == 16) return launch_pass_model<Model, 2, 3, 16>(sa, na, s);
        if (p.sw == 2) return p.nst > 3 ? launch_pass_model<Model, 2, 4>(sa, na, s) : launch_pass_model<Model, 2, 3>(sa, na, s);
    }
    if constexpr (NS > 3 && NS % 3 == 0) {
        if (p.sw == 3) return launch_pass_model<Model, 3, 3>(sa, na, s);
    }
    if (p.hs == 2) return p.bk == 16 ? launch_pass_model<Model, 1, 3, 16, 1, 2>(sa, na, s) : launch_pass_model<Model, 1, 3, 8, 1, 2>(sa, na, s);
    if (p.bk == 16) return launch_pass_model<Model, 1, 3, 16>(sa, na, s);
    return p.nst > 3 ? launch_pass_model<Model, 1, 4>(sa, na, s) : launch_pass_model<Model, 1, 3>(sa, na, s);
}

bool pass_supported(int model, int ns, int B, int M, const SymPlan& p) {
    if (p.ring1 || p.sw < 1 || (model != EMI_MODEL_POINTMASS2D && model != EMI_MODEL_QUADROTOR2D)) return false;
    if (M % 128 != 0 || ns % p.sw != 0) return false;
    return B >= 1;
}

hipError_t launch_pass(int model, const SymDefectArgs& sa, const NodeArgs<double>& na, hipStream_t s, const SymPlan& p) {
    if (model == EMI_MODEL_POINTMASS2D) return launch_pass_planned<PointMass2D<double>>(sa, na, s, p);
    if (model == EMI_MODEL_QUADROTOR2D) return launch_pass_planned<Quadrotor2D<double>>(sa, na, s, p);
    return hipErrorInvalidValue;
}

bool fused_supported(int model, int M, int ct) {
    if (ct == 0 || (ct >= 4 && ct <= 8))
        return (model == EMI_MODEL_POINTMASS2D || model == EMI_MODEL_QUADROTOR2D) && M >= 128 && M % 128 == 0;
    const int w = ct == 2 ? 2 : 1;
    return (model == EMI_MODEL_POINTMASS2D || model == EMI_MODEL_QUADROTOR2D) && ct >= 1 && ct <= 3 &&
           M >= 128 * w && M % (128 * w) == 0;
}

hipError_t launch_symdefect(int model, const SymDefectArgs& a, hipStream_t s, bool set_attr, int ct, const SymPlan& plan) {
    if (!plan.ring1) {
        if (model == EMI_MODEL_POINTMASS2D) return launch_ring2_planned<PointMass2D<double>>(a, s, plan);
        if (model == EMI_MODEL_QUADROTOR2D) return launch_ring2_planned<Quadrotor2D<double>>(a, s, plan);
        return hipErrorInvalidValue;
    }
    if (ct == 0 || ct >= 4) {
        ct = 3;
        set_attr = true;
    }
    if (ct == 3) {
        if (model == EMI_MODEL_POINTMASS2D) return launch_symdefect_ring_model<PointMass2D<double>>(a, s, set_attr);
        if (model == EMI_MODEL_QUADROTOR2D) return launch_symdefect_ring_model<Quadrotor2D<double>>(a, s, set_attr);
        return hipErrorInvalidValue;
    }
    if (model == EMI_MODEL_POINTMASS2D)
        return ct == 1 ? launch_symdefect_model<PointMass2D<double>, 1>(a, s, set_attr)
                       : launch_symdefect_model<PointMass2D<double>, 2>(a, s, set_attr);
    if (model == EMI_MODEL_QUADROTOR2D)
        return ct == 1 ? launch_symdefect_model<Quadrotor2D<double>, 1>(a, s, set_attr)
                       : launch_symdefect_model<Quadrotor2D<double>, 2>(a, s, set_attr);
    return hipErrorInvalidValue;
}

}
```

etol_amd/csrc/emi_symdefect_kernels.hpp:

```cpp
#pragma once
#include "emi_args.hpp"
#include "emi_node_kernels.hpp"

namespace emi {

typedef double d4 __attribute__((ext_vector_type(4)));

template <class Model, int CT>
__global__ __launch_bounds__(256, CT == 1 ? 2 : 1) void emi_symdefect_f64_kernel(SymDefectArgs a) {
    constexpr int NS = Model::NS, NC = Model::NC, NV = Model::NV;
    constexpr int TI = FUSED_TI, TM = NS * TI, TN = 64 * CT, BK = FUSED_BK, LDK = BK + 2;
    constexpr int A_PASS = TM * (BK / 2) / 256;
    constexpr int B_PASS = TN * (BK / 2) / 256;
    static_assert(TM * (BK / 2) % 256 == 0 && TN * (BK / 2) % 256 == 0, "staging shape");
    static_assert(TN % 64 == 0 && TI == 16, "wave layout below assumes 16 instances x 64*CT columns");
    constexpr int STAGE = (2 * TM + 2 * TN) * LDK;

    extern __shared__ __attribute__((aligned(16))) double smem[];

    const int M = a.M, Hh = M >> 1, B = a.B;
    const int mtiles = (B + TI - 1) / TI;
    int bid = blockIdx.x;
    {
        const int nwg = gridDim.x, xcd = bid & 7, q = nwg >> 3, rr = nwg & 7;
// ... 181 lines not shown
            const int c = p ^ ((row >> 1) & 7);
            src[t] = (od ? a.Do : a.De) + (size_t)(i0 + row) * Hh + 2 * c;
            kdir[t] = 1;
        }
    }
    const unsigned lds0 = (unsigned)(unsigned long)(emi_lds_ptr_t)smem;
    auto issue = [&](int stage, int kt) {
#pragma unroll
        for (int t = 0; t < L; ++t) {
            const unsigned dst = lds0 + (unsigned)stage * (unsigned)(STAGE * 8) + (unsigned)(wid + 4 * t) * 1024u;
            const double* g = src[t] + (ptrdiff_t)kdir[t] * kt * BK;
            asm volatile("s_mov_b32 m0, %1\n\t" EMI_M0_NOP "global_load_lds_dwordx4 %0, off" ::"v"(g), "s"(dst) : "memory", "m0");
        }
    };

    d4 acc_a[NS], acc_b[NS];
#pragma unroll
    for (int s = 0; s < NS; ++s) {
        acc_a[s] = d4{0.0, 0.0, 0.0, 0.0};
        acc_b[s] = d4{0.0, 0.0, 0.0, 0.0};
    }

    const int nkt = Hh / BK;
    issue(0, 0);
    if (nkt > 1) issue(1, 1);
    for (int kt = 0; kt < nkt; ++kt) {
        if (kt + 1 < nkt) asm volatile("s_waitcnt vmcnt(%0)" ::"n"(L) : "memory");
        else              asm volatile("s_waitcnt vmcnt(0)" ::: "memory");
        asm volatile("s_barrier" ::: "memory");
        if (kt + 2 < nkt && !(a.ablate & 2)) issue((kt + 2) % NST, kt + 2);
        if (a.ablate & 1) continue;
        const double* XF = smem + (size_t)(kt % NST) * STAGE;
        const double* XM = XF + TM * BK;
        const double* DE = XM + TM * BK;
        const double* DO = DE + TN * BK;
        const int rb = wid * 16 + r16, swb = (rb >> 1) & 7;
        double xf_c[NS], xm_c[NS], be_c, bo_c;
        auto frag = [&](int ks, double (&xf)[NS], double (&xm)[NS], double& be, double& bo) {
            const int kk = ks * 4 + kq, km = BK - 1 - kk;
            const int pb = ((kk >> 1) ^ swb) * 2 + (kk & 1);
            be = DE[rb * BK + pb];
            bo = DO[rb * BK + pb];
#pragma unroll
            for (int s = 0; s < NS; ++s) {
                const int r = s * 16 + r16, sw = (r >> 1) & 7;
                xf[s] = XF[r * BK + ((kk >> 1) ^ sw) * 2 + (kk & 1)];
                xm[s] = XM[r * BK + ((km >> 1) ^ sw) * 2 + (km & 1)];
            }
        };
        frag(0, xf_c, xm_c, be_c, bo_c);
#pragma unroll
        for (int ks = 0; ks < BK / 4; ++ks) {
            double xf_n[NS], xm_n[NS], be_n = 0.0, bo_n = 0.0;
            if (ks + 1 < BK / 4) frag(ks + 1, xf_n, xm_n, be_n, bo_n);
#pragma unroll
            for (int s = 0; s < NS; ++s) {
                acc_a[s] = __builtin_amdgcn_mfma_f64_16x16x4f64(xf_c[s] + xm_c[s], be_c, acc_a[s], 0, 0, 0);
                acc_b[s] = __builtin_amdgcn_mfma_f64_16x16x4f64(xf_c[s] - xm_c[s], bo_c, acc_b[s], 0, 0, 0);
            }
            if (ks + 1 < BK / 4) {
#pragma unroll
                for (int s = 0; s < NS; ++s) { xf_c[s] = xf_n[s]; xm_c[s] = xm_n[s]; }
                be_c = be_n;
                bo_c = bo_n;
            }
        }
    }

    const int col = wid * 16 + r16;
    const int node_f = i0 + col, node_m = M - 1 - node_f;
#pragma unroll
    for (int i = 0; i < 4; ++i) {
        const int inst = inst0 + kq + 4 * i;
        if (inst >= B || (a.ablate & 4)) continue;
        const double* __restrict__ Xb = a.X + (size_t)inst * NS * M;
        const double* __restrict__ Ub = a.U + (size_t)inst * NC * M;
        double* __restrict__ Rb = a.RES + (size_t)inst * a.nres * M;
#pragma unroll
        for (int side = 0; side < 2; ++side) {
            const int node = side == 0 ? node_f : node_m;
            double z[NV], f[NS];
#pragma unroll
            for (int v = 0; v < NS; ++v) z[v] = Xb[(size_t)v * M + node];
#pragma unroll
            for (int v = 0; v < NC; ++v) z[NS + v] = Ub[(size_t)v * M + node];
            Model::f(a.P, z, a.node_t[node], f);
#pragma unroll
            for (int s = 0; s < NS; ++s) {
                const double dx = side == 0 ? acc_a[s][i] + acc_b[s][i] : acc_b[s][i] - acc_a[s][i];
                Rb[(size_t)s * M + node] = dx - a.h * f[s];
            }
        }
    }
}

EMI_DEV constexpr int ring_swz(int r) { return (0 - (r >> 2)) & 3; }
#ifndef EMI_EPILOGUE_PREFETCH
#define EMI_EPILOGUE_PREFETCH 0
#endif
template <int BK> EMI_DEV constexpr int ring_swz_k(int r) { return BK == 8 ? ring_swz(r) : ((r >> 1) & 7); }

template <class Model>
EMI_DEV void ring_epilogue_load(const SymDefectArgs& a, double (&z)[2][Model::NV], int inst, int node_f) {
    constexpr int NS = Model::NS, NC = Model::NC;
    const int M = a.M, node_m = M - 1 - node_f;
    inst = inst < a.B ? inst : a.B - 1;
    const double* __restrict__ Xb = a.X + (size_t)inst * NS * M;
    const double* __restrict__ Ub = a.U + (size_t)inst * NC * M;
#pragma unroll
    for (int side = 0; side < 2; ++side) {
        const int node = side == 0 ? node_f : node_m;
#pragma unroll
        for (int v = 0; v < NS; ++v) z[side][v] = Xb[(size_t)v * M + node];
#pragma unroll
        for (int v = 0; v < NC; ++v) z[side][NS + v] = Ub[(size_t)v * M + node];
    }
}
template <class Model, int SW, int S0, bool PRE>
EMI_DEV void ring_epilogue_s0(const SymDefectArgs& a, const d4 (&acc_a)[SW], const d4 (&acc_b)[SW], int inst0, int i0,
                              int wid, int r16, int kq, const double (&zpre)[2][Model::NV]) {
    constexpr int NS = Model::NS, NC = Model::NC, NV = Model::NV;
    const int M = a.M, B = a.B;
    const int col = wid * 16 + r16;
    const int node_f = i0 + col, node_m = M - 1 - node_f;
    const double t_f = a.node_t[node_f], t_m = a.node_t[node_m];
    if constexpr (SW == 1) {
        if (a.ablate & 4) return;
        double zz[4][2][NV];
#pragma unroll
        for (int i = 0; i < 4; ++i) {
            int inst = inst0 + kq + 4 * i;
            inst = inst < B ? inst : B - 1;
            const double* __restrict__ Xb = a.X + (size_t)inst * NS * M;
            const double* __restrict__ Ub = a.U + (size_t)inst * NC * M;
#pragma unroll
            for (int side = 0; side < 2; ++side) {
                const int node = side == 0 ? node_f : node_m;
#pragma unroll
                for (int v = 0; v < NS; ++v) zz[i][side][v] = Xb[(size_t)v * M + node];
#pragma unroll
                for (int v = 0; v < NC; ++v) zz[i][side][NS + v] = Ub[(size_t)v * M + node];
            }
        }
#pragma unroll
        for (int i = 0; i < 4; ++i) {
            const int inst = inst0 + kq + 4 * i;
            if (inst >= B) continue;
            double* __restrict__ Rb = a.RES + (size_t)inst * a.nres * M;
#pragma unroll
            for (int side = 0; side < 2; ++side) {
                double f[NS];
                Model::f(a.P, zz[i][side], side == 0 ? t_f : t_m, f);
                const double dx = side == 0 ? acc_a[0][i] + acc_b[0][i] : acc_b[0][i] - acc_a[0][i];
                Rb[(size_t)S0 * M + (side == 0 ? node_f : node_m)] = dx - a.h * f[S0];
            }
        }
        return;
    }
    if (a.ablate & 4) return;
    auto load_z = [&](double (&z)[2][NV], int i) {
        int inst = inst0 + kq + 4 * i;
        inst = inst < B ? inst : B - 1;
        const double* __restrict__ Xb = a.X + (size_t)inst * NS * M;
        const double* __restrict__ Ub = a.U + (size_t)inst * NC * M;
#pragma unroll
        for (int side = 0; side < 2; ++side) {
            const int node = side == 0 ? node_f : node_m;
#pragma unroll
            for (int v = 0; v < NS; ++v) z[side][v] = Xb[(size_t)v * M + node];
#pragma unroll
            for (int v = 0; v < NC; ++v) z[side][NS + v] = Ub[(size_t)v * M + node];
        }
    };
    double zc[2][NV], zn[2][NV];
    if constexpr (PRE) {
#pragma unroll
        for (int side = 0; side < 2; ++side)
#pragma unroll
            for (int v = 0; v < NV; ++v) zc[side][v] = zpre[side][v];
    } else {
        load_z(zc, 0);
    }
#pragma unroll
    for (int i = 0; i < 4; ++i) {
        if (i < 3) load_z(zn, i + 1);
        const int inst = inst0 + kq + 4 * i;
        if (inst < B) {
            double* __restrict__ Rb = a.RES + (size_t)inst * a.nres * M;
            double hf[2][SW];
#pragma unroll
            for (int side = 0; side < 2; ++side) {
                double f[NS];
                Model::f(a.P, zc[side], side == 0 ? t_f : t_m, f);
#pragma unroll
                for (int s = 0; s < SW; ++s) hf[side][s] = a.h * f[S0 + s];
            }
#pragma unroll
            for (int side = 0; side < 2; ++side) {
                const int node = side == 0 ? node_f : node_m;
#pragma unroll
                for (int s = 0; s < SW; ++s) {
                    const double dx = side == 0 ? acc_a[s][i] + acc_b[s][i] : acc_b[s][i] - acc_a[s][i];
                    Rb[(size_t)(S0 + s) * M + node] = dx - hf[side][s];
                }
            }
        }
        if (i < 3) {
#pragma unroll
            for (int side = 0; side < 2; ++side)
#pragma unroll
                for (int v = 0; v < NV; ++v) zc[side][v] = zn[side][v];
        }
    }
}
template <class Model, int SW, bool PRE, int SG = 0>
EMI_DEV void ring_epilogue_pre(const SymDefectArgs& a, const d4 (&acc_a)[SW], const d4 (&acc_b)[SW], int inst0, int i0,
                               int s0, int wid, int r16, int kq, const double (&zpre)[2][Model::NV]) {
    if constexpr (SG * SW < Model::NS) {
        if (s0 == SG * SW) ring_epilogue_s0<Model, SW, SG * SW, PRE>(a, acc_a, acc_b, inst0, i0, wid, r16, kq, zpre);
        else ring_epilogue_pre<Model, SW, PRE, SG + 1>(a, acc_a, acc_b, inst0, i0, s0, wid, r16, kq, zpre);
    }
}
template <class Model, int SW>
EMI_DEV void ring_epilogue(const SymDefectArgs& a, const d4 (&acc_a)[SW], const d4 (&acc_b)[SW], int inst0, int i0,
                           int s0, int wid, int r16, int kq) {
    const double none[2][Model::NV] = {};
    ring_epilogue_pre<Model, SW, false>(a, acc_a, acc_b, inst0, i0, s0, wid, r16, kq, none);
}

template <class Model, int SW, int NST = 3, int BK = 8, int CT = 1, int HS = 1>
EMI_DEV void emi_ring2_body(const SymDefectArgs& a, const int bid ) {
    constexpr int NS = Model::NS;
    constexpr int TI = FUSED_TI, TM = SW * TI, TN = 64 * CT, CH = BK / 2, NSG = NS / SW;
    static_assert(CT == 1 || CT == 2, "one or two column sub-tiles per wave");
    constexpr int KH = BK / 8;
    constexpr int RPI = 64 / CH;
    static_assert(BK == 8 || BK == 16, "K tiles of 8 or 16");
    constexpr int LOOK = NST - 1;
    constexpr int ROWS = 2 * TM + 2 * TN;
    constexpr int ROWS_PAD = (ROWS + 63) / 64 * 64;
    constexpr int STAGE = ROWS_PAD * BK;
    constexpr int L = ROWS_PAD * CH / 256;
    static_assert(NS % SW == 0, "states split evenly over workgroups");

    extern __shared__ __attribute__((aligned(16))) double smem_all[];
    static_assert(HS == 1 || HS == 2, "the K range whole or in two halves");
    const int half = HS > 1 ? __builtin_amdgcn_readfirstlane((int)(threadIdx.x >> 8)) : 0;
    double* const smem = smem_all + (size_t)half * NST * STAGE;

    const int M = a.M, Hh = M >> 1, B = a.B;
    const int ntiles = Hh / TN;
    const int KS = (HS == 1 && a.ksplit > 1) ? a.ksplit : 1;
    const int kslice = bid % KS;
    const RingTile rt = ring_tile_of(bid / KS, ntiles, (B + TI - 1) / TI * NSG, a.cpart, a.cx, NSG);
    const int ntile = rt.ntile, grp = rt.grp;
    const int tile = grp * ntiles + ntile;
    const int sg = grp % NSG, mtile = grp / NSG;
    const int inst0 = mtile * TI, i0 = ntile * TN, s0 = sg * SW;

    const int tid = threadIdx.x & 255, lane = tid & 63;
    const int wid = __builtin_amdgcn_readfirstlane(tid >> 6);
    const int r16 = lane & 15, kq = lane >> 4;

    unsigned voff[L];
    unsigned long long gbase[L];
    int gstep[L];
#pragma unroll
    for (int t = 0; t < L; ++t) {
        const int row0 = (wid + 4 * t) * RPI;
        const int row = row0 + lane / CH, p = lane % CH;
        if (row0 < 2 * TM) {
            const bool mir = row0 >= TM;
            const int rr = row - (mir ? TM : 0);
            const int c = p ^ ring_swz_k<BK>(rr);
            int inst = inst0 + (rr & 15);
            inst = inst < B ? inst : B - 1;
            if (a.ablate & 8) inst &= 15;
            voff[t] = (unsigned)((((size_t)inst * NS + s0 + (rr >> 4)) * M + 2 * c) * sizeof(double));
            gbase[t] = (unsigned long long)(a.X + (mir ? M - BK : 0));
            gstep[t] = mir ? -(int)(BK * sizeof(double)) : (int)(BK * sizeof(double));
        } else if (row0 < ROWS) {
            const bool od = row0 >= 2 * TM + TN;
            const int rr = row - 2 * TM - (od ? TN : 0);
            const int c = p ^ ring_swz_k<BK>(rr);
            voff[t] = (unsigned)(((size_t)((a.ablate & 64) ? rr : i0 + rr) * Hh + 2 * c) * sizeof(double));
            gbase[t] = (unsigned long long)(od ? a.Do : a.De);
            gstep[t] = (int)(BK * sizeof(double));
        } else {
            voff[t] = (unsigned)(2 * p * sizeof(double));
            gbase[t] = (unsigned long long)a.De;
            gstep[t] = 0;
        }
    }
    const unsigned lds0 = (unsigned)(unsigned long)(emi_lds_ptr_t)smem;
    const int nkt = (Hh / BK) / KS / HS, kt0 = (kslice * HS + half) * nkt;
    unsigned long long gnext[L];
#pragma unroll
    for (int t = 0; t < L; ++t) gnext[t] = gbase[t] + (long long)gstep[t] * kt0;
    unsigned st_dma = 0, st_rd = 0;
    int nd = 0;
    auto issue_one = [&](int t) {
        const unsigned dst = lds0 + st_dma + (unsigned)(wid + 4 * t) * 1024u;
        asm volatile("s_mov_b32 m0, %2\n\t" EMI_M0_NOP "global_load_lds_dwordx4 %0, %1" ::"v"(voff[t]), "s"(gnext[t]), "s"(dst) : "memory", "m0");
        gnext[t] += (long long)gstep[t];
        if (t == L - 1) {
            st_dma = st_dma == (unsigned)((NST - 1) * STAGE * 8) ? 0u : st_dma + (unsigned)(STAGE * 8);
            ++nd;
        }
    };
    auto issue = [&]() {
#pragma unroll
        for (int t = 0; t < L; ++t) issue_one(t);
    };

    d4 acc_a[SW][CT], acc_b[SW][CT];
#pragma unroll
    for (int s = 0; s < SW; ++s)
#pragma unroll
        for (int c = 0; c < CT; ++c) {
            acc_a[s][c] = d4{0.0, 0.0, 0.0, 0.0};
            acc_b[s][c] = d4{0.0, 0.0, 0.0, 0.0};
        }

    constexpr bool EPI_PRE = EMI_EPILOGUE_PREFETCH && SW >= 2 && SW <= 3 && HS == 1 && CT == 1;
    double zpre[2][Model::NV] = {};
    if constexpr (EPI_PRE) ring_epilogue_load<Model>(a, zpre, inst0 + kq, i0 + wid * 16 + r16);

#pragma unroll
    for (int t = 0; t < LOOK; ++t)
        if (t < nkt) issue();
    int off_b[CT][KH], off_f[SW][KH], off_m[SW][KH];
#pragma unroll
    for (int c = 0; c < CT; ++c) {
        const int rb = c * 64 + wid * 16 + r16;
#pragma unroll
        for (int h = 0; h < KH; ++h) off_b[c][h] = rb * BK + (((kq + 4 * h) ^ ring_swz_k<BK>(rb)) << 1);
    }
#pragma unroll
    for (int s = 0; s < SW; ++s) {
        const int r = s * 16 + r16;
#pragma unroll
        for (int h = 0; h < KH; ++h) {
            off_f[s][h] = r * BK + (((kq + 4 * h) ^ ring_swz_k<BK>(r)) << 1);
            off_m[s][h] = (TM + r) * BK + (((CH - 1 - kq - 4 * h) ^ ring_swz_k<BK>(r)) << 1);
        }
    }
    struct Frag {
        double2 be[CT][KH], bo[CT][KH], sp[SW][KH], dm[SW][KH];
    };
    double2 txf[SW][KH], txm[SW][KH];
    constexpr int NRH = 2 * CT + 2 * SW;
    constexpr int NR = NRH * KH, NM = 4 * SW * CT * KH;
    auto read_one = [&](Frag& f, const double* S, int r) {
        const int h = r / NRH, q = r % NRH;
        if (q < 2 * CT) {
            if (q & 1) f.bo[q >> 1][h] = *reinterpret_cast<const double2*>(S + (2 * TM + TN) * BK + off_b[q >> 1][h]);
            else f.be[q >> 1][h] = *reinterpret_cast<const double2*>(S + 2 * TM * BK + off_b[q >> 1][h]);
        } else if (q & 1) txm[(q - 2 * CT) >> 1][h] = *reinterpret_cast<const double2*>(S + off_m[(q - 2 * CT) >> 1][h]);
        else txf[(q - 2 * CT) >> 1][h] = *reinterpret_cast<const double2*>(S + off_f[(q - 2 * CT) >> 1][h]);
    };
    auto sums_one = [&](Frag& f, int s) {
#pragma unroll
        for (int h = 0; h < KH; ++h) {
            f.sp[s][h] = double2{txf[s][h].x + txm[s][h].y, txf[s][h].y + txm[s][h].x};
            f.dm[s][h] = double2{txf[s][h].x - txm[s][h].y, txf[s][h].y - txm[s][h].x};
        }
    };
    auto rd_stage = [&]() -> const double* {
        const double* S = smem + (st_rd >> 3);
        st_rd = st_rd == (unsigned)((NST - 1) * STAGE * 8) ? 0u : st_rd + (unsigned)(STAGE * 8);
        return S;
    };
    auto read_frag = [&](Frag& f) {
        const double* S = rd_stage();
#pragma unroll
        for (int r = 0; r < NR; ++r) read_one(f, S, r);
#pragma unroll
        for (int s = 0; s < SW; ++s) sums_one(f, s);
    };
    auto mfma_one = [&](const Frag& f, int i) {
        const int per = 2 * SW * CT, q = i % per, j = i / per, h = j >> 1;
        const int s = q / (2 * CT), c = (q >> 1) % CT;
        const bool second = j & 1, odd = q & 1;
        if (!odd) acc_a[s][c] = __builtin_amdgcn_mfma_f64_16x16x4f64(second ? f.sp[s][h].y : f.sp[s][h].x, second ? f.be[c][h].y : f.be[c][h].x, acc_a[s][c], 0, 0, 0);
        else      acc_b[s][c] = __builtin_amdgcn_mfma_f64_16x16x4f64(second ? f.dm[s][h].y : f.dm[s][h].x, second ? f.bo[c][h].y : f.bo[c][h].x, acc_b[s][c], 0, 0, 0);
    };
    auto multiply = [&](const Frag& f) {
#pragma unroll
        for (int i = 0; i < NM; ++i) mfma_one(f, i);
    };
    if constexpr (SW <= 3) {
        constexpr int RPG = (NR + (NM - L) - 1) / (NM - L);
        constexpr int GR = (NR + RPG - 1) / RPG;
        static_assert(NM > L && GR + L <= NM, "a gap for every DMA instruction after the reads");
        auto step = [&](const Frag& cur, Frag& nxt, int kt) {
            if (kt + LOOK < nkt) asm volatile("s_waitcnt vmcnt(%0)" ::"n"(L * (LOOK - 1)) : "memory");
            else                 asm volatile("s_waitcnt vmcnt(0)" ::: "memory");
            __builtin_amdgcn_s_waitcnt(0xC07F);
            asm volatile("s_barrier" ::: "memory");
            const bool more = nd < nkt;
            const double* S = rd_stage();
#pragma unroll
            for (int i = 0; i < NM; ++i) {
                mfma_one(cur, i);
                if (i < GR) {
#pragma unroll
                    for (int r = i * RPG; r < (i + 1) * RPG && r < NR; ++r) read_one(nxt, S, r);
                } else if (i < GR + L) {
                    if (more) issue_one(i - GR);
                }
                if (i >= NM - SW) sums_one(nxt, i - (NM - SW));
                __builtin_amdgcn_sched_barrier(0);
            }
        };
        Frag f0, f1;
        if (nkt > LOOK - 1) asm volatile("s_waitcnt vmcnt(%0)" ::"n"(L * (LOOK - 1)) : "memory");
        else                asm volatile("s_waitcnt vmcnt(0)" ::: "memory");
        asm volatile("s_barrier" ::: "memory");
        if (LOOK < nkt) issue();
        __builtin_amdgcn_s_waitcnt(0xC07F);
        read_frag(f0);
        int kt = 0;
        for (; kt + 2 < nkt; kt += 2) {
            step(f0, f1, kt);
            step(f1, f0, kt + 1);
        }
        step(f0, f1, kt);
        multiply(f1);
    } else {
        for (int kt = 0; kt < nkt; ++kt) {
            if (kt + LOOK - 1 < nkt) asm volatile("s_waitcnt vmcnt(%0)" ::"n"(L * (LOOK - 1)) : "memory");
// ... 161 lines not shown
```

etol_amd/evaluator.py:

```python
import ctypes as C

import numpy as np
import torch

from . import _lib as L


def _dp(a):
    return a.ctypes.data_as(C.POINTER(C.c_double))


def lgl(M):
    lib = L.load()
    tau = np.empty(M)
    w = np.empty(M)
    D = np.empty((M, M))
    L.check(lib.emi_lgl(M, _dp(tau), _dp(w), _dp(D)), what="emi_lgl")
    return tau, w, D


def model_dims(model):
    lib = L.load()
    ns, nc, npar = C.c_int(), C.c_int(), C.c_int()
    L.check(lib.emi_model_dims(model, C.byref(ns), C.byref(nc), C.byref(npar)), what="emi_model_dims")
# ... 150 lines not shown
    def eval_host(self, X, U, flags=L.EVAL_ALL, res_in=None):
        lay = self.layout
        X = np.ascontiguousarray(X, dtype=np.float64)
        U = np.ascontiguousarray(U, dtype=np.float64)
        assert X.shape == (lay.B, lay.ns, lay.M) and U.shape == (lay.B, lay.nc - self.n_delayed, lay.M)
        RES = np.zeros((lay.B, lay.nres, lay.M)) if res_in is None else np.ascontiguousarray(res_in, dtype=np.float64).copy()
        VALS = np.zeros((lay.B, lay.nvals, lay.M))
        COST = np.zeros(lay.B)
        self._ck(self.lib.emi_eval_host(self.ctx, _dp(X), _dp(U), _dp(RES), _dp(VALS), _dp(COST), flags), "emi_eval_host")
        return RES, VALS, COST

    def hess_host(self, X, U, lamF, lamC, sigma=1.0):
        lay = self.layout
        X, U, lamF = (np.ascontiguousarray(a, dtype=np.float64) for a in (X, U, lamF))
        lamC = np.ascontiguousarray(lamC if lamC is not None else np.zeros((lay.B, 0, lay.M)), dtype=np.float64)
        H = np.zeros((lay.B, lay.nhess, lay.M))
        self._ck(self.lib.emi_hess_host(self.ctx, _dp(X), _dp(U), _dp(lamF), _dp(lamC) if lamC.size else None,
                                         float(sigma), _dp(H)), "emi_hess_host")
        return H

    CERT_FIELDS = ("stat", "comp", "defect", "viol", "gmax", "lmax")

    def lagr_grad_dev(self, VALS, lamF, lamC, sigma, G):
        ptr = lambda t: C.c_void_p(t.data_ptr()) if t is not None else None
        self._ck(self.lib.emi_lagr_grad_dev(self.ctx, ptr(VALS), ptr(lamF), ptr(lamC), float(sigma), ptr(G)), "emi_lagr_grad_dev")

    def lagr_grad_host(self, VALS, lamF, lamC, sigma=1.0):
        lay = self.layout
        VALS, lamF = (np.ascontiguousarray(a, dtype=np.float64) for a in (VALS, lamF))
        lamC = np.ascontiguousarray(lamC if lamC is not None else np.zeros((lay.B, 0, lay.M)), dtype=np.float64)
        assert VALS.shape == (lay.B, lay.nvals, lay.M) and lamF.shape == (lay.B, lay.ns, lay.M) and lamC.shape == (lay.B, lay.np, lay.M)
        G = np.zeros((lay.B, lay.ns + lay.nc, lay.M))
        self._ck(self.lib.emi_lagr_grad_host(self.ctx, _dp(VALS), _dp(lamF), _dp(lamC) if lamC.size else None, float(sigma), _dp(G)),
                 "emi_lagr_grad_host")
        return G

    def kkt_certificate_dev(self, X, U, RES, VALS, lamF, lamC, sigma, zl, zu, cl, cu, cert, G=None):
        ptr = lambda t: C.c_void_p(t.data_ptr()) if t is not None else None
        cl, cu = (np.ascontiguousarray(a, dtype=np.float64) for a in (cl, cu))
        self._ck(self.lib.emi_kkt_certificate_dev(self.ctx, ptr(X), ptr(U), ptr(RES), ptr(VALS), ptr(lamF), ptr(lamC), float(sigma),
                                                  ptr(zl), ptr(zu), int(zl.shape[0]), _dp(cl) if cl.size else None,
                                                  _dp(cu) if cu.size else None, ptr(cert), ptr(G)), "emi_kkt_certificate_dev")

    def kkt_certificate_host(self, X, U, lamF, lamC, zl, zu, cl=(), cu=(), sigma=1.0):
        lay = self.layout
        X, U, lamF, zl, zu, cl, cu = (np.ascontiguousarray(a, dtype=np.float64) for a in (X, U, lamF, zl, zu, cl, cu))
        lamC = np.ascontiguousarray(lamC if lamC is not None else np.zeros((lay.B, 0, lay.M)), dtype=np.float64)
        nv = lay.ns + lay.nc
        if zl.ndim == 2:
            zl, zu = zl[None], zu[None]
        assert zl.shape == zu.shape and zl.shape[1:] == (nv, lay.M) and cl.shape == cu.shape == (lay.np,)
        cert, G = np.zeros((lay.B, 6)), np.zeros((lay.B, nv, lay.M))
        self._ck(self.lib.emi_kkt_certificate_host(self.ctx, _dp(X), _dp(U), _dp(lamF), _dp(lamC) if lamC.size else None, float(sigma),
                                                   _dp(zl), _dp(zu), zl.shape[0], _dp(cl) if cl.size else None,
                                                   _dp(cu) if cu.size else None, _dp(cert), _dp(G)), "emi_kkt_certificate_host")
        return cert, G

    def lagr_grad_total_dev(self, VALS, lamF, lamC, sigma, G, Gdel=None):
        ptr = lambda t: C.c_void_p(t.data_ptr()) if t is not None else None
        self._ck(self.lib.emi_lagr_grad_total_dev(self.ctx, ptr(VALS), ptr(lamF), ptr(lamC), float(sigma), ptr(G), ptr(Gdel)),
                 "emi_lagr_grad_total_dev")

    def lagr_grad_total_host(self, VALS, lamF, lamC, sigma=1.0):
        lay = self.layout
        VALS, lamF = (np.ascontiguousarray(a, dtype=np.float64) for a in (VALS, lamF))
        lamC = np.ascontiguousarray(lamC if lamC is not None else np.zeros((lay.B, 0, lay.M)), dtype=np.float64)
        assert VALS.shape == (lay.B, lay.nvals, lay.M) and lamF.shape == (lay.B, lay.ns, lay.M) and lamC.shape == (lay.B, lay.np, lay.M)
        nd = self.n_delayed
        G, Gdel = np.zeros((lay.B, lay.ns + lay.nc - nd, lay.M)), np.zeros((lay.B, nd, lay.M))
        self._ck(self.lib.emi_lagr_grad_total_host(self.ctx, _dp(VALS), _dp(lamF), _dp(lamC) if lamC.size else None, float(sigma), _dp(G),
                                                   _dp(Gdel) if nd else None), "emi_lagr_grad_total_host")
        return G, Gdel

    def kkt_certificate_total_dev(self, X, U, RES, VALS, lamF, lamC, sigma, zl, zu, cl, cu, cert, G=None, Gdel=None):
        ptr = lambda t: C.c_void_p(t.data_ptr()) if t is not None else None
        cl, cu = (np.ascontiguousarray(a, dtype=np.float64) for a in (cl, cu))
        self._ck(self.lib.emi_kkt_certificate_total_dev(self.ctx, ptr(X), ptr(U), ptr(RES), ptr(VALS), ptr(lamF), ptr(lamC), float(sigma),
                                                        ptr(zl), ptr(zu), int(zl.shape[0]), _dp(cl) if cl.size else None,
                                                        _dp(cu) if cu.size else None, ptr(cert), ptr(G), ptr(Gdel)),
                 "emi_kkt_certificate_total_dev")

    def kkt_certificate_total_host(self, X, U, lamF, lamC, zl, zu, cl=(), cu=(), sigma=1.0):
        lay = self.layout
        X, U, lamF, zl, zu, cl, cu = (np.ascontiguousarray(a, dtype=np.float64) for a in (X, U, lamF, zl, zu, cl, cu))
        lamC = np.ascontiguousarray(lamC if lamC is not None else np.zeros((lay.B, 0, lay.M)), dtype=np.float64)
        nd = self.n_delayed
        nf = lay.ns + lay.nc - nd
        if zl.ndim == 2:
            zl, zu = zl[None], zu[None]
        assert X.shape == (lay.B, lay.ns, lay.M) and U.shape == (lay.B, nf - lay.ns, lay.M)
        assert zl.shape == zu.shape and zl.shape[1:] == (nf, lay.M) and cl.shape == cu.shape == (lay.np,)
        cert, G, Gdel = np.zeros((lay.B, 6)), np.zeros((lay.B, nf, lay.M)), np.zeros((lay.B, nd, lay.M))
        self._ck(self.lib.emi_kkt_certificate_total_host(self.ctx, _dp(X), _dp(U), _dp(lamF), _dp(lamC) if lamC.size else None,
                                                         float(sigma), _dp(zl), _dp(zu), zl.shape[0], _dp(cl) if cl.size else None,
                                                         _dp(cu) if cu.size else None, _dp(cert), _dp(G), _dp(Gdel) if nd else None),
                 "emi_kkt_certificate_total_host")
        return cert, G, Gdel

    def kkt_factor(self, Qblk, Jblk, fixed, dc=0.0):
        lay = self.layout
        nv = lay.ns + lay.nc
        Qblk = np.ascontiguousarray(Qblk, dtype=np.float64)
        Jblk = np.ascontiguousarray(Jblk, dtype=np.float64)
        fixed = np.ascontiguousarray(fixed, dtype=np.uint8)
        assert Qblk.shape == (lay.nhess, lay.M) and Jblk.shape == (lay.ns * nv, lay.M) and fixed.shape == (nv * lay.M,)
        info = C.c_int(-1)
        self._ck(self.lib.emi_kkt_factor(self.ctx, _dp(Qblk), _dp(Jblk), fixed.ctypes.data_as(C.POINTER(C.c_ubyte)),
                                         float(dc), C.byref(info)), "emi_kkt_factor")
        return info.value

    def kkt_lowrank(self, node, vec, delta):
        node = np.ascontiguousarray(node, dtype=np.int32)
        vec = np.ascontiguousarray(vec, dtype=np.float64)
        delta = np.ascontiguousarray(delta, dtype=np.float64)
        exact = C.c_int(0)
        r = node.size
        self._ck(self.lib.emi_kkt_lowrank(self.ctx, r, node.ctypes.data_as(C.POINTER(C.c_int)) if r else None,
                                          _dp(vec) if r else None, _dp(delta) if r else None, C.byref(exact)), "emi_kkt_lowrank")
        return bool(exact.value)

    def kkt_solve(self, rhs):
        rhs = np.ascontiguousarray(rhs, dtype=np.float64).copy()
        nrhs = 1 if rhs.ndim == 1 else rhs.shape[0]
        self._ck(self.lib.emi_kkt_solve(self.ctx, _dp(rhs), nrhs), "emi_kkt_solve")
        return rhs

    def timer_start(self):
        self._ck(self.lib.emi_timer_start(self.ctx), "emi_timer_start")

    def timer_stop(self):
        ms = C.c_float()
        self._ck(self.lib.emi_timer_stop(self.ctx, C.byref(ms)), "emi_timer_stop")
        return ms.value

    def profile(self, level):
        self._ck(self.lib.emi_profile_enable(self.ctx, int(level)), "emi_profile_enable")

    def profile_read(self):
        nm, dm, fm = C.c_float(), C.c_float(), C.c_float()
        nl, dl, fl = C.c_int(), C.c_int(), C.c_int()
        self._ck(self.lib.emi_profile_read(self.ctx, C.byref(nm), C.byref(nl), C.byref(dm), C.byref(dl), C.byref(fm),
                                           C.byref(fl)), "emi_profile_read")
        return dict(node_ms=nm.value, node_launches=nl.value, defect_ms=dm.value, defect_launches=dl.value,
                    pass_ms=fm.value, overlapped_passes=fl.value)

    def set_option(self, name, value):
        self._ck(self.lib.emi_set_option(self.ctx, name.encode(), int(value)), "emi_set_option")

    def plan(self, B=None):
        p = L.PassPlan()
        self._ck(self.lib.emi_plan_pass(self.ctx, int(B if B is not None else self.layout.B), C.byref(p)), "emi_plan_pass")
        return {n: getattr(p, n) for n, _ in L.PassPlan._fields_}

    @property
    def last_defect_kernel(self):
        return self.lib.emi_last_defect_kernel(self.ctx).decode()

    @property
    def uses_fused_kernel(self):
        f = C.c_int()
        self._ck(self.lib.emi_last_path(self.ctx, C.byref(f)), "emi_last_path")
        return bool(f.value)
```

etol_amd/host/emi_trace.cpp:

```cpp
#include "emi_trace.hpp"

#include <algorithm>

#include <cmath>
#include <cstdio>
#include <cstdlib>
#include <set>
#include <sstream>

namespace ETOL {
namespace mi355x {

Trace& Trace::active() {
    static thread_local Trace t;
    return t;
}

void Trace::clear() {
    _nodes.clear();
    _cse.clear();
}

int Trace::intern(const Node& n) {
    const auto key = std::make_tuple((int)n.op, n.a, n.b, n.c);
// ... 101 lines not shown
        switch (nd.op) {
            case ADD: add(nd.a, g); add(nd.b, g); break;
            case SUB: add(nd.a, g); add(nd.b, unary(NEG, g)); break;
            case MUL: add(nd.a, binary(MUL, g, nd.b)); add(nd.b, binary(MUL, g, nd.a)); break;
            case DIV:
                add(nd.a, binary(DIV, g, nd.b));
                add(nd.b, unary(NEG, binary(DIV, binary(MUL, g, n), nd.b)));
                break;
            case NEG: add(nd.a, unary(NEG, g)); break;
            case SIN: add(nd.a, binary(MUL, g, unary(COS, nd.a))); break;
            case COS: add(nd.a, unary(NEG, binary(MUL, g, unary(SIN, nd.a)))); break;
            case TAN: add(nd.a, binary(MUL, g, binary(ADD, constant(1.0), binary(MUL, n, n)))); break;
            case EXP: add(nd.a, binary(MUL, g, n)); break;
            case LOG: add(nd.a, binary(DIV, g, nd.a)); break;
            case SQRT: add(nd.a, binary(DIV, g, binary(MUL, constant(2.0), n))); break;
            case POWC: add(nd.a, binary(MUL, g, binary(MUL, constant(nd.c), unary(POWC, nd.a, nd.c - 1.0)))); break;
            case MAX: {
                const int sa = unary(STEP, binary(SUB, nd.a, nd.b));
                add(nd.a, binary(MUL, g, sa));
                add(nd.b, binary(MUL, g, binary(SUB, constant(1.0), sa)));
                break;
            }
            case MIN: {
                const int sb = unary(STEP, binary(SUB, nd.b, nd.a));
                add(nd.a, binary(MUL, g, sb));
                add(nd.b, binary(MUL, g, binary(SUB, constant(1.0), sb)));
                break;
            }
            case ABS: add(nd.a, binary(MUL, g, binary(SUB, binary(MUL, constant(2.0), unary(STEP, nd.a)), constant(1.0)))); break;
            case STEP: break;
            default: break;
        }
    }
    return adj;
}

double Trace::eval(int node, const std::vector<double>& x, const std::vector<double>& u, double t,
                   const std::vector<double>& coef) const {
    std::vector<double> v(node + 1, 0.0);
    for (int n = 0; n <= node; ++n) {
        const Node& nd = _nodes[n];
        switch (nd.op) {
            case CONST: v[n] = nd.c; break;
            case IN_STATE: v[n] = x.at(nd.a); break;
            case IN_CONTROL: v[n] = u.at(nd.a); break;
            case IN_TIME: v[n] = t; break;
            case IN_COEF: v[n] = coef.at(nd.a); break;
            case IN_PARAM: v[n] = param_values.at(nd.a); break;
            case ADD: v[n] = v[nd.a] + v[nd.b]; break;
            case SUB: v[n] = v[nd.a] - v[nd.b]; break;
            case MUL: v[n] = v[nd.a] * v[nd.b]; break;
            case DIV: v[n] = v[nd.a] / v[nd.b]; break;
            case NEG: v[n] = -v[nd.a]; break;
            case SIN: v[n] = std::sin(v[nd.a]); break;
            case COS: v[n] = std::cos(v[nd.a]); break;
            case TAN: v[n] = std::tan(v[nd.a]); break;
            case EXP: v[n] = std::exp(v[nd.a]); break;
            case LOG: v[n] = std::log(v[nd.a]); break;
            case SQRT: v[n] = std::sqrt(v[nd.a]); break;
            case POWC: v[n] = std::pow(v[nd.a], nd.c); break;
            case MAX: v[n] = v[nd.a] > v[nd.b] ? v[nd.a] : v[nd.b]; break;
            case MIN: v[n] = v[nd.a] < v[nd.b] ? v[nd.a] : v[nd.b]; break;
            case ABS: v[n] = std::fabs(v[nd.a]); break;
            case STEP: v[n] = v[nd.a] > 0.0 ? 1.0 : 0.0; break;
        }
    }
    return v[node];
}

std::string Trace::emit(const std::vector<int>& outs, const std::vector<std::string>& targets, bool accumulate,
                        const std::string& ind) const {
    std::set<int> need;
    std::vector<int> stack(outs.begin(), outs.end());
    while (!stack.empty()) {
        const int n = stack.back();
        stack.pop_back();
        if (n < 0 || need.count(n)) continue;
        need.insert(n);
        const Node& nd = _nodes[n];
        if (nd.op >= ADD) {
            stack.push_back(nd.a);
            if (nd.b >= 0) stack.push_back(nd.b);
        }
    }
    std::ostringstream o;
    o.precision(17);
    auto ref = [&](int n) -> std::string {
        const Node& nd = _nodes[n];
        std::ostringstream r;
        r.precision(17);
        switch (nd.op) {
            case CONST: r << "T(" << std::scientific << nd.c << ")"; return r.str();
            case IN_STATE: r << "z[" << nd.a << "]"; return r.str();
            case IN_CONTROL: r << "z[NS + " << nd.a << "]"; return r.str();
            case IN_TIME: return "tk";
            case IN_COEF: r << "cc[" << nd.a << "]"; return r.str();
            case IN_PARAM: r << "P.p[" << nd.a << "]"; return r.str();
            default: r << "v" << n; return r.str();
        }
    };
    for (int n : need) {
        const Node& nd = _nodes[n];
        if (nd.op < ADD) continue;
        o << ind << "const T v" << n << " = ";
        switch (nd.op) {
            case ADD: o << ref(nd.a) << " + " << ref(nd.b); break;
            case SUB: o << ref(nd.a) << " - " << ref(nd.b); break;
            case MUL: o << ref(nd.a) << " * " << ref(nd.b); break;
            case DIV: o << ref(nd.a) << " / " << ref(nd.b); break;
            case NEG: o << "-" << ref(nd.a); break;
            case SIN: o << "emi_sin(" << ref(nd.a) << ")"; break;
            case COS: o << "emi_cos(" << ref(nd.a) << ")"; break;
            case TAN: o << "emi_tan(" << ref(nd.a) << ")"; break;
            case EXP: o << "emi_exp(" << ref(nd.a) << ")"; break;
            case LOG: o << "emi_log(" << ref(nd.a) << ")"; break;
            case SQRT: o << "emi_sqrt(" << ref(nd.a) << ")"; break;
            case POWC: o << "emi_pow(" << ref(nd.a) << ", T(" << std::scientific << nd.c << "))"; break;
            case MAX: o << "(" << ref(nd.a) << " > " << ref(nd.b) << " ? " << ref(nd.a) << " : " << ref(nd.b) << ")"; break;
            case MIN: o << "(" << ref(nd.a) << " < " << ref(nd.b) << " ? " << ref(nd.a) << " : " << ref(nd.b) << ")"; break;
            case ABS: o << "(" << ref(nd.a) << " < T(0) ? -" << ref(nd.a) << " : " << ref(nd.a) << ")"; break;
            case STEP: o << "(" << ref(nd.a) << " > T(0) ? T(1) : T(0))"; break;
            default: break;
        }
        o << ";\n";
    }
    for (size_t i = 0; i < outs.size(); ++i) {
        if (outs[i] < 0) continue;
        o << ind << targets[i] << (accumulate ? " += " : " = ") << ref(outs[i]) << ";\n";
    }
    return o.str();
}

std::vector<int> Trace::dependencies(int out, int ns, int nc) {
    std::vector<int> deps;
    std::set<int> seen;
    std::vector<int> stack = {out};
    while (!stack.empty()) {
        const int n = stack.back();
        stack.pop_back();
        if (n < 0 || seen.count(n)) continue;
        seen.insert(n);
        const Node& nd = _nodes[n];
        if (nd.op == IN_STATE && nd.a < ns) deps.push_back(nd.a);
        else if (nd.op == IN_CONTROL && nd.a < nc) deps.push_back(ns + nd.a);
        else if (nd.op >= ADD) {
            stack.push_back(nd.a);
            if (nd.b >= 0) stack.push_back(nd.b);
        }
    }
    std::sort(deps.begin(), deps.end());
    return deps;
}

std::string Trace::generate_model(const std::string& name, int ns, int nc, const std::vector<int>& f, int L,
                                  const std::vector<int>& paths, std::vector<int>* path_vars, std::string* err) {
    const int nv = ns + nc;
    (void)err;
    auto in_node = [&](int v) { return v < ns ? input(IN_STATE, v) : input(IN_CONTROL, v - ns); };
    const int npath = (int)paths.size();
    std::vector<int> pv;
    for (int j = 0; j < npath; ++j)
        for (int v : dependencies(paths[j], ns, nc))
            if (std::find(pv.begin(), pv.end(), v) == pv.end()) pv.push_back(v);
    std::sort(pv.begin(), pv.end());
    if (npath > 0 && pv.empty()) pv.push_back(0);
    const int pw = (int)pv.size();
    if (path_vars) *path_vars = pv;
    std::vector<std::vector<int>> cd(npath, std::vector<int>(pw, -1));
    std::vector<int> PH;
    std::vector<std::string> PHt;
    if (npath > 0) {
        for (int j = 0; j < npath; ++j) {
            const std::vector<int> adj = adjoints(paths[j]);
            for (int q = 0; q < pw; ++q) {
                const int n = in_node(pv[q]);
                cd[j][q] = n < (int)adj.size() ? adj[n] : -1;
            }
        }
        int psi = -1;
        for (int j = 0; j < npath; ++j) {
            const int term = binary(MUL, input(IN_COEF, j), paths[j]);
            psi = psi < 0 ? term : binary(ADD, psi, term);
        }
        const std::vector<int> a1 = adjoints(psi);
        for (int qa = 0; qa < pw; ++qa) {
            const int na = in_node(pv[qa]);
            const int ga = na < (int)a1.size() ? a1[na] : -1;
            if (ga < 0) continue;
            const std::vector<int> a2 = adjoints(ga);
            for (int qb = 0; qb <= qa; ++qb) {
                const int nb = in_node(pv[qb]);
                const int h = nb < (int)a2.size() ? a2[nb] : -1;
                double c;
                if (h < 0 || (is_const(h, &c) && c == 0.0)) continue;
                PH.push_back(h);
                PHt.push_back("H[" + std::to_string(pv[qa] * (pv[qa] + 1) / 2 + pv[qb]) + "]");
            }
        }
    }
    std::vector<std::vector<int>> J(ns, std::vector<int>(nv, -1));
    for (int i = 0; i < ns; ++i) {
        const std::vector<int> adj = adjoints(f[i]);
        for (int v = 0; v < nv; ++v) {
            const int n = in_node(v);
            J[i][v] = n < (int)adj.size() ? adj[n] : -1;
        }
    }
    std::vector<int> gL(nv, -1);
    {
        const std::vector<int> adj = adjoints(L);
        for (int v = 0; v < nv; ++v) {
            const int n = in_node(v);
            gL[v] = n < (int)adj.size() ? adj[n] : -1;
        }
    }
    int phi = binary(MUL, input(IN_COEF, 0), L);
    for (int i = 0; i < ns; ++i) phi = binary(ADD, phi, binary(MUL, input(IN_COEF, 1 + i), f[i]));
    std::vector<int> g(nv, -1);
    {
        const std::vector<int> adj = adjoints(phi);
        for (int v = 0; v < nv; ++v) {
            const int n = in_node(v);
            g[v] = n < (int)adj.size() ? adj[n] : -1;
        }
    }
    std::vector<int> H;
    std::vector<std::string> Ht;
    for (int v = 0; v < nv; ++v) {
        std::vector<int> adj;
        if (g[v] >= 0) adj = adjoints(g[v]);
        for (int q = 0; q <= v; ++q) {
            const int n = in_node(q);
            int h = (g[v] >= 0 && n < (int)adj.size()) ? adj[n] : -1;
            double c;
            if (h >= 0 && is_const(h, &c) && c == 0.0) h = -1;
            H.push_back(h);
            Ht.push_back("H[" + std::to_string(v * (v + 1) / 2 + q) + "]");
        }
    }

    std::ostringstream o;
    o << "template <typename T> struct " << name << " {\n";
    o << "    static constexpr int NS = " << ns << ", NC = " << nc << ", NV = " << nv << ", NPARAM = 0, NPATH = " << npath
      << ", PW = " << pw << ";\n";
    if (npath > 0) {
        o << "    EMI_DEV static constexpr int pvar(int q) { return ";
        for (int q = 0; q + 1 < pw; ++q) o << "q == " << q << " ? " << pv[q] << " : ";
        o << pv[pw - 1] << "; }\n";
    }
    o << "    EMI_DEV static void f(const ModelParams<T>&, const T* z, T tk, T* fo) {\n";
    {
        std::vector<std::string> t;
        for (int i = 0; i < ns; ++i) t.push_back("fo[" + std::to_string(i) + "]");
        o << emit(f, t, false, "        ");
    }
    o << "        (void)tk;\n    }\n";
    o << "    EMI_DEV static void jac(const ModelParams<T>&, const T* z, T tk, T (*J)[NV]) {\n";
    o << "        for (int i = 0; i < NS; ++i)\n            for (int v = 0; v < NV; ++v) J[i][v] = T(0);\n";
    {
        std::vector<int> outs;
        std::vector<std::string> t;
        for (int i = 0; i < ns; ++i)
            for (int v = 0; v < nv; ++v) {
                double c;
                if (J[i][v] < 0 || (is_const(J[i][v], &c) && c == 0.0)) continue;
                outs.push_back(J[i][v]);
                t.push_back("J[" + std::to_string(i) + "][" + std::to_string(v) + "]");
            }
        o << emit(outs, t, false, "        ");
    }
    o << "        (void)tk; (void)z;\n    }\n";
    o << "    EMI_DEV static T cost(const ModelParams<T>&, const T* z, T tk) {\n        T Lv;\n";
    o << emit({L}, {"Lv"}, false, "        ");
    o << "        (void)tk;\n        return Lv;\n    }\n";
    o << "    EMI_DEV static void grad(const ModelParams<T>&, const T* z, T tk, T* g) {\n";
    o << "        for (int v = 0; v < NV; ++v) g[v] = T(0);\n";
    {
        std::vector<int> outs;
        std::vector<std::string> t;
        for (int v = 0; v < nv; ++v) {
            if (gL[v] < 0) continue;
            outs.push_back(gL[v]);
            t.push_back("g[" + std::to_string(v) + "]");
        }
        o << emit(outs, t, false, "        ");
    }
    o << "        (void)tk; (void)z;\n    }\n";
    o << "    EMI_DEV static void hess(const ModelParams<T>&, const T* z, T tk, T cL, const T* cf, T* H) {\n";
    o << "        T cc[NS + 1];\n        cc[0] = cL;\n        for (int i = 0; i < NS; ++i) cc[1 + i] = cf[i];\n";
    o << emit(H, Ht, true, "        ");
    o << "        (void)tk; (void)z; (void)cc;\n    }\n";
    if (npath > 0) {
        o << "    EMI_DEV static void path(const ModelParams<T>&, const T* z, T tk, T* c, T* cd) {\n";
        o << "        for (int j = 0; j < NPATH * PW; ++j) cd[j] = T(0);\n";
        {
            std::vector<int> outs;
            std::vector<std::string> t;
            for (int j = 0; j < npath; ++j) {
                outs.push_back(paths[j]);
                t.push_back("c[" + std::to_string(j) + "]");
                for (int q = 0; q < pw; ++q) {
                    double cc;
                    if (cd[j][q] < 0 || (is_const(cd[j][q], &cc) && cc == 0.0)) continue;
                    outs.push_back(cd[j][q]);
                    t.push_back("cd[" + std::to_string(j * pw + q) + "]");
                }
            }
            o << emit(outs, t, false, "        ");
        }
        o << "        (void)tk; (void)z;\n    }\n";
        o << "    EMI_DEV static void path_hess(const ModelParams<T>&, const T* z, T tk, const T* cc, T* H) {\n";
        o << emit(PH, PHt, true, "        ");
        o << "        (void)tk; (void)z; (void)cc; (void)H;\n    }\n";
    }
    o << "};\n";
    return o.str();
}

std::string Trace::generate_hess_body(int ns, int nc, const std::vector<int>& f, int L) {
    const int nv = ns + nc;
    auto in_node = [&](int v) { return v < ns ? input(IN_STATE, v) : input(IN_CONTROL, v - ns); };
    int phi = binary(MUL, input(IN_COEF, 0), L);
    for (int i = 0; i < ns; ++i) phi = binary(ADD, phi, binary(MUL, input(IN_COEF, 1 + i), f[i]));
    std::vector<int> g(nv, -1);
    {
        const std::vector<int> adj = adjoints(phi);
        for (int v = 0; v < nv; ++v) {
            const int n = in_node(v);
            g[v] = n < (int)adj.size() ? adj[n] : -1;
        }
    }
    std::vector<int> H;
    std::vector<std::string> Ht;
    for (int v = 0; v < nv; ++v) {
        std::vector<int> adj;
        if (g[v] >= 0) adj = adjoints(g[v]);
        for (int q = 0; q <= v; ++q) {
            const int n = in_node(q);
            int h = (g[v] >= 0 && n < (int)adj.size()) ? adj[n] : -1;
            double c;
            if (h >= 0 && is_const(h, &c) && c == 0.0) h = -1;
            if (h < 0) continue;
            H.push_back(h);
            Ht.push_back("H[" + std::to_string(v * (v + 1) / 2 + q) + "]");
        }
    }
    return emit(H, Ht, true, "        ");
}

namespace {
int node_of(const Var& v) {
    if (v.node < 0) {
        fprintf(stderr, "mi355x::Var used outside a callback trace\n");
        exit(EXIT_FAILURE);
    }
    return v.node;
}
Var wrap(int n) {
    Var r;
    r.kind = Var::EXPR;
    r.node = n;
    return r;
}
}

Var::Var(double constant) : kind(EXPR), index(0), node(Trace::active().constant(constant)) {}
Var::Var(Kind k, size_t i) : kind(k), index(i), node(-1) {
    Trace& t = Trace::active();
    node = t.input(k == STATE ? Trace::IN_STATE : (k == CONTROL ? Trace::IN_CONTROL : Trace::IN_TIME), (int)i);
}
Var operator+(const Var& a, const Var& b) { return wrap(Trace::active().binary(Trace::ADD, node_of(a), node_of(b))); }
Var operator-(const Var& a, const Var& b) { return wrap(Trace::active().binary(Trace::SUB, node_of(a), node_of(b))); }
Var operator*(const Var& a, const Var& b) { return wrap(Trace::active().binary(Trace::MUL, node_of(a), node_of(b))); }
Var operator/(const Var& a, const Var& b) { return wrap(Trace::active().binary(Trace::DIV, node_of(a), node_of(b))); }
Var operator-(const Var& a) { return wrap(Trace::active().unary(Trace::NEG, node_of(a))); }
Var sin(const Var& a) { return wrap(Trace::active().unary(Trace::SIN, node_of(a))); }
Var cos(const Var& a) { return wrap(Trace::active().unary(Trace::COS, node_of(a))); }
Var tan(const Var& a) { return wrap(Trace::active().unary(Trace::TAN, node_of(a))); }
Var exp(const Var& a) { return wrap(Trace::active().unary(Trace::EXP, node_of(a))); }
Var log(const Var& a) { return wrap(Trace::active().unary(Trace::LOG, node_of(a))); }
Var sqrt(const Var& a) { return wrap(Trace::active().unary(Trace::SQRT, node_of(a))); }
Var max(const Var& a, const Var& b) { return wrap(Trace::active().binary(Trace::MAX, node_of(a), node_of(b))); }
Var min(const Var& a, const Var& b) { return wrap(Trace::active().binary(Trace::MIN, node_of(a), node_of(b))); }
Var abs(const Var& a) { return wrap(Trace::active().unary(Trace::ABS, node_of(a))); }
Var interp1(const std::vector<double>& tw, const std::vector<double>& vw, const Var& t) {
    if (tw.size() != vw.size() || tw.empty()) {
        fprintf(stderr, "mi355x::interp1: table sizes differ or are empty\n");
        exit(EXIT_FAILURE);
    }
    Var out(vw[0]);
    for (size_t i = 0; i + 1 < tw.size(); ++i) {
        if (!(tw[i + 1] > tw[i])) continue;
        const double slope = (vw[i + 1] - vw[i]) / (tw[i + 1] - tw[i]);
        out = out + slope * (min(max(t, Var(tw[i])), Var(tw[i + 1])) - tw[i]);
    }
    return out;
}
Var pow(const Var& a, double c) { return wrap(Trace::active().unary(Trace::POWC, node_of(a), c)); }

}
}
```

etol_amd/host/emi_trace.hpp:

```cpp
#ifndef ETOL_MI355X_EMI_TRACE_HPP_
#define ETOL_MI355X_EMI_TRACE_HPP_

#include <map>
#include <string>
#include <tuple>
#include <vector>

#include <ETOL/eMI355X_Types.hpp>

namespace ETOL {
namespace mi355x {

class Trace {
 public:
    enum Op { CONST, IN_STATE, IN_CONTROL, IN_TIME, IN_COEF, IN_PARAM, ADD, SUB, MUL, DIV, MAX, MIN, NEG, SIN, COS, TAN, EXP, LOG, SQRT, POWC,
              ABS, STEP };
    struct Node {
        Op op;
        int a, b;
        double c;
    };

    void clear();
    int constant(double c);
    int input(Op kind, int index);
    int unary(Op op, int a, double c = 0.0);
    int binary(Op op, int a, int b);
    const std::vector<Node>& nodes() const { return _nodes; }

    std::vector<int> adjoints(int out);

    std::string generate_model(const std::string& name, int ns, int nc, const std::vector<int>& f, int L,
                               const std::vector<int>& paths = {}, std::vector<int>* path_vars = nullptr,
                               std::string* err = nullptr);
    std::vector<int> dependencies(int out, int ns, int nc);

    double eval(int node, const std::vector<double>& x, const std::vector<double>& u, double t,
                const std::vector<double>& coef = {}) const;

    std::string generate_hess_body(int ns, int nc, const std::vector<int>& f, int L);
    std::vector<double> param_values;

    static Trace& active();

 private:
    std::vector<Node> _nodes;
    std::map<std::tuple<int, int, int, double>, int> _cse;
    int intern(const Node& n);
    bool is_const(int n, double* v = nullptr) const;
    std::string emit(const std::vector<int>& outs, const std::vector<std::string>& targets, bool accumulate,
                     const std::string& indent) const;
};

}
}
#endif
```

include/emi355x.h:

```cpp
#ifndef EMI355X_H_
#define EMI355X_H_

#include <stddef.h>

#ifdef __cplusplus
extern "C" {
#endif

#define EMI_ABI_VERSION 2

typedef struct emi_ctx_s* emi_ctx_t;

enum {
    EMI_OK = 0,
    EMI_ERR_ARG = 1,
    EMI_ERR_STATE = 2,
    EMI_ERR_HIP = 3,
    EMI_ERR_NO_DEVICE = 4,
    EMI_ERR_UNSUPPORTED = 5,
    EMI_ERR_COMM = 6
};

enum {
    EMI_MODEL_POINTMASS2D = 0,
    EMI_MODEL_QUADROTOR2D = 1,
    EMI_MODEL_FIXEDWING12 = 2,
    EMI_MODEL_SOURCE = 100
};

enum {
    EMI_PATH_ELLIPSE = 0,
    EMI_PATH_DISC = 1,
    EMI_PATH_TRACK = 2
};
#define EMI_PATH_REC 8

enum {
    EMI_EVAL_NODES = 1u,
    EMI_EVAL_DEFECT = 2u,
    EMI_EVAL_ALL = 3u,
    EMI_EVAL_NOJAC = 4u
};

typedef struct {
    int model, ns, nc, np, M, B;
    int nres;
    int nvals;
    int nhess;
    int real_bytes;
    int px, py;
    double t0, tf;
} emi_layout_t;

int emi_abi_version(void);
const char* emi_status_string(int status);
int emi_device_count(int* count);

int emi_lgl(int M, double* tau, double* w, double* D);
int emi_model_dims(int model, int* ns, int* nc, int* nparams);
int emi_edge_ellipse(double xa, double ya, double xb, double yb, double* rec8);
int emi_track_centres(int nway, const double* t, const double* x, const double* y,
                      int M, const double* node_t, double* xc, double* yc);

int emi_create(int device_id, emi_ctx_t* out);
int emi_create_f32(int device_id, emi_ctx_t* out);
int emi_destroy(emi_ctx_t ctx);
const char* emi_last_error(emi_ctx_t ctx);
int emi_set_stream(emi_ctx_t ctx, void* hip_stream);
int emi_get_stream(emi_ctx_t ctx, void** hip_stream);
int emi_synchronize(emi_ctx_t ctx);

int emi_set_mesh(emi_ctx_t ctx, int M, const double* tau, const double* w,
                 const double* D, double t0, double tf);
int emi_set_model(emi_ctx_t ctx, int model, const double* params, int nparams,
                  int maximize);
int emi_set_model_source(emi_ctx_t ctx, const char* struct_name, const char* source,
                         int ns, int nc, int npath, const int* path_vars, int n_path_vars,
                         const double* params, int nparams, int maximize);
int emi_check_model_source(const char* struct_name, const char* source, int ns,
                           int nc, int npath, int n_path_vars, int f32, char* log, size_t log_len);
int emi_set_batch(emi_ctx_t ctx, int B);
int emi_set_delays(emi_ctx_t ctx, int x_horizon, int u_horizon, double dt);
int emi_get_delays(emi_ctx_t ctx, int* x_horizon, int* u_horizon, int* n_delayed);
int emi_delay_matrix(int M, const double* tau, const double* w, double t0, double tf, double delay, double* W);
int emi_set_path(emi_ctx_t ctx, int np, int nsets, const double* recs,
                 int px_state, int py_state);
int emi_set_tracks(emi_ctx_t ctx, int ntracks, int nsets, const double* xc,
                   const double* yc);
int emi_get_layout(emi_ctx_t ctx, emi_layout_t* out);

int emi_kkt_factor(emi_ctx_t ctx, const double* Qblk, const double* Jblk,
                   const unsigned char* fixed, double dc, int* info);
int emi_kkt_lowrank(emi_ctx_t ctx, int r, const int* node, const double* vec,
                    const double* delta, int* exact);
int emi_kkt_factor_batch(int n, const emi_ctx_t* ctxs, const double* const* Qblk,
                         const double* const* Jblk, const unsigned char* const* fixed,
                         const double* dc, int* info);
int emi_kkt_solve_batch(int n, const emi_ctx_t* ctxs, double* const* rhs);
int emi_kkt_is_schur(emi_ctx_t ctx);
int emi_kkt_solve_refined(emi_ctx_t ctx, double* rhs, double dc_nominal, int max_steps,
                          double* rel, int* nsolve, int* reverted, int* status);
int emi_kkt_solve_refined_batch(int n, const emi_ctx_t* ctxs, double* const* rhs,
                                const double* dc_nominal, int max_steps, double* rel,
                                int* nsolve, int* reverted, int* status);
int emi_kkt_last_regularisation(emi_ctx_t ctx, double* dc, double* dw);
int emi_kkt_solve(emi_ctx_t ctx, double* rhs, int nrhs);

typedef struct emi_pass_plan {
  int one_launch;
  int sw;
  int ksplit;
  int ring_stages;
  int cpart, cx;
  int mfma_workgroups;
  int store_mode;
  int block_order;
  int tiles16;
  int piece, tail;
  int k_tile;
  int column_tiles;
  int k_halves;
} emi_pass_plan_t;
int emi_plan_pass(emi_ctx_t ctx, int B, emi_pass_plan_t* out);

int emi_jac_structure(emi_ctx_t ctx, int* rows, int* cols);

int emi_dev_alloc(emi_ctx_t ctx, size_t bytes, void** dptr);
int emi_dev_free(emi_ctx_t ctx, void* dptr);
int emi_h2d(emi_ctx_t ctx, void* dst, const void* src, size_t bytes);
int emi_d2h(emi_ctx_t ctx, void* dst, const void* src, size_t bytes);

int emi_eval_dev(emi_ctx_t ctx, const void* dX, const void* dU, void* dRES,
                 void* dVALS, void* dCOST, unsigned flags);
int emi_eval_host(emi_ctx_t ctx, const double* X, const double* U, double* RES,
                  double* VALS, double* COST, unsigned flags);

int emi_hess_dev(emi_ctx_t ctx, const void* dX, const void* dU,
                 const void* dLamF, const void* dLamC, double sigma, void* dH);
int emi_hess_host(emi_ctx_t ctx, const double* X, const double* U,
                  const double* LamF, const double* LamC, double sigma,
                  double* H);

int emi_lagr_grad_dev(emi_ctx_t ctx, const void* dVALS, const void* dLamF, const void* dLamC, double sigma, void* dG);
int emi_lagr_grad_host(emi_ctx_t ctx, const double* VALS, const double* LamF, const double* LamC, double sigma, double* G);
int emi_kkt_certificate_dev(emi_ctx_t ctx, const void* dX, const void* dU, const void* dRES, const void* dVALS,
                            const void* dLamF, const void* dLamC, double sigma, const void* dZl, const void* dZu, int nsets,
                            const double* cl, const double* cu, void* dCert, void* dG);
int emi_kkt_certificate_host(emi_ctx_t ctx, const double* X, const double* U, const double* LamF, const double* LamC,
                             double sigma, const double* zl, const double* zu, int nsets, const double* cl, const double* cu,
                             double* cert, double* G);
int emi_lagr_grad_total_dev(emi_ctx_t ctx, const void* dVALS, const void* dLamF, const void* dLamC, double sigma, void* dG,
                            void* dGdel);
int emi_lagr_grad_total_host(emi_ctx_t ctx, const double* VALS, const double* LamF, const double* LamC, double sigma, double* G,
                             double* Gdel);
int emi_kkt_certificate_total_dev(emi_ctx_t ctx, const void* dX, const void* dU, const void* dRES, const void* dVALS,
                                  const void* dLamF, const void* dLamC, double sigma, const void* dZl, const void* dZu, int nsets,
                                  const double* cl, const double* cu, void* dCert, void* dG, void* dGdel);
int emi_kkt_certificate_total_host(emi_ctx_t ctx, const double* X, const double* U, const double* LamF, const double* LamC,
                                   double sigma, const double* zl, const double* zu, int nsets, const double* cl, const double* cu,
                                   double* cert, double* G, double* Gdel);

int emi_timer_start(emi_ctx_t ctx);
int emi_timer_stop(emi_ctx_t ctx, float* elapsed_ms);
int emi_profile_enable(emi_ctx_t ctx, int level);
int emi_profile_read(emi_ctx_t ctx, float* node_ms, int* node_launches,
                     float* defect_ms, int* defect_launches,
                     float* fused_ms, int* fused_launches);

int emi_set_option(emi_ctx_t ctx, const char* name, int value);
int emi_last_path(emi_ctx_t ctx, int* fused);
int emi_debug_tile_order(int ns, int B, int M, int sym_ct, int sym_cpart, int* out_tile, int out_cap, int* ntiles_total,
                         int* cpart, int* cx);
int emi_debug_tile_order2(int ns, int B, int M, int sym_ct, int sym_cpart, int sym_gblk, int sym_cx, int* out_tile, int out_cap,
                          int* ntiles_total, int* cpart, int* cx);
int emi_debug_pass_roles(int nm, int nn, int order, int* out_role, int out_cap);
const char* emi_last_defect_kernel(emi_ctx_t ctx);

#define EMI_COMM_ID_BYTES 128
typedef struct emi_comm_s* emi_comm_t;
int emi_comm_unique_id(void* id );
int emi_comm_create(int device_id, int world, int rank, const void* id, emi_comm_t* out);
int emi_comm_gather(emi_comm_t comm, const void* dsend, void* drecv, size_t bytes, int root, void* hip_stream);
int emi_comm_destroy(emi_comm_t comm);
const char* emi_comm_last_error(emi_comm_t comm);

#ifdef __cplusplus
}
#endif
#endif
```

Baseline: 5.137 billion.

## Group states sharing dynamics subexpressions into the same ring-defect work slice

```diff
diff --git a/etol_amd/_lib.py b/etol_amd/_lib.py
--- a/etol_amd/_lib.py
+++ b/etol_amd/_lib.py
@@ -30,7 +30,7 @@
 
 class PassPlan(C.Structure):
     _fields_ = [(n, C.c_int) for n in ("one_launch", "sw", "ksplit", "ring_stages", "cpart", "cx", "mfma_workgroups", "store_mode",
-                                       "block_order", "tiles16", "piece", "tail", "k_tile", "column_tiles", "k_halves")]
+                                       "block_order", "tiles16", "piece", "tail", "k_tile", "column_tiles", "k_halves", "state_grouping")]
 
 
 _P = C.c_void_p
@@ -93,6 +93,8 @@
     "emi_set_option": (C.c_int, [_P, C.c_char_p, C.c_int]),
     "emi_last_path": (C.c_int, [_P, _I]),
     "emi_plan_pass": (C.c_int, [_P, C.c_int, C.POINTER(PassPlan)]),
+    "emi_state_order": (C.c_int, [_P, C.c_int, _I]),
+    "emi_model_state_order": (C.c_int, [C.c_int, C.c_int, _I]),
     "emi_last_defect_kernel": (C.c_char_p, [_P]),
     "emi_debug_pass_roles": (C.c_int, [C.c_int, C.c_int, C.c_int, C.POINTER(C.c_int), C.c_int]),
     "emi_debug_tile_order": (C.c_int, [C.c_int, C.c_int, C.c_int, C.c_int, C.c_int, C.POINTER(C.c_int), C.c_int, C.POINTER(C.c_int), C.POINTER(C.c_int), C.POINTER(C.c_int)]),
diff --git a/etol_amd/csrc/emi_api.hip b/etol_amd/csrc/emi_api.hip
--- a/etol_amd/csrc/emi_api.hip
+++ b/etol_amd/csrc/emi_api.hip
@@ -72,6 +72,7 @@
     int sym_hs = 0;
     int sym_ctc = 0;
     int sym_bk = 0;
+    int sym_sgroup = 1;
     int xh = 0, uh = 0, nch = 0;
     double delay_dt = 0.0;
     bool delay_dirty = true;
@@ -221,6 +222,11 @@
     return (!c->rtc && !c->f32) ? 1 : 0;
 }
 
+bool state_order_of(emi_ctx_t c, int sw, int* out) {
+    if (c->rtc) return emi::rtc_state_order(c->rtc, sw, out);
+    return emi::ring_state_order(c->model, sw, out);
+}
+
 struct PassPlan {
     bool one_launch = false;
     emi::SymPlan sym;
@@ -273,6 +279,7 @@
     if (hs_want == 2 && !c->rtc && plan.ks == 1 && plan.ct == 1 && (plan.sw == 1 || plan.sw == 2) && plan.nst == 3 &&
         ((c->M / 2) / plan.bk) % 4 == 0)
         plan.hs = 2;
+    plan.sgroup = (c->rtc || c->sym_sgroup) ? 1 : 0;
     p.sym = plan;
     p.mfma_first = c->pass_order >= 0 ? c->pass_order
                                       : (deep_band ? 150 : (p.tiles16 < 208 ? 1 : (p.tiles16 < 384 ? 125 : (p.tiles16 < 768 ? 110 : 0))));
@@ -433,6 +440,7 @@
     {"sym_hs", &emi_ctx_s::sym_hs, within<0, 2>, as_given, "sym_hs must be 0 (by batch size), 1 or 2"},
     {"sym_ctc", &emi_ctx_s::sym_ctc, within<0, 2>, as_given, "sym_ctc must be 0 (by batch size), 1 or 2"},
     {"sym_bk", &emi_ctx_s::sym_bk, one_of<0, 8, 16>, as_given, "sym_bk must be 0 (by batch size), 8 or 16"},
+    {"sym_sgroup", &emi_ctx_s::sym_sgroup, within<0, 1>, as_given, "sym_sgroup must be 1 (the model's state groups) or 0 (contiguous states)"},
     {"sym_cpart", &emi_ctx_s::sym_cpart, one_of<-1, 0, 1, 2, 4, 8>, as_given, "sym_cpart must be -1 (plain order), 0 (by mesh size), 1, 2, 4 or 8"},
     {"sym_gblk", &emi_ctx_s::sym_gblk, within<0, 64>, as_given, "sym_gblk must be 0 (off) .. 64 instance groups per super-block"},
     {"sym_cx", &emi_ctx_s::sym_cx, within<0, 64>, as_given, "sym_cx must be 0 (default) .. 64 column tiles per block"},
@@ -577,7 +585,8 @@
         c->last_defect_kernel = NAME_RING1_F64;
         return EMI_OK;
     }
-    const emi::SymPlan plan = emi::plan_symdefect(c->ns, L.B, c->M, c->sym_ct, c->sym_ksplit, c->sym_cpart, c->sym_gblk, c->sym_cx);
+    emi::SymPlan plan = emi::plan_symdefect(c->ns, L.B, c->M, c->sym_ct, c->sym_ksplit, c->sym_cpart, c->sym_gblk, c->sym_cx);
+    plan.sgroup = c->sym_sgroup;
     if (plan.slab_bytes) EMI_TRY(ensure(c, c->d_slab, plan.slab_bytes));
     sa.ksplit = plan.ring1 ? 1 : plan.ks;
     sa.slab = (double*)c->d_slab.p;
@@ -1699,8 +1708,25 @@
         out->store_mode = p.store_mode;
         out->block_order = p.mfma_first;
         out->tiles16 = p.tiles16;
-    }
-    return EMI_OK;
+        int order[64];
+        if (p.sym.sgroup && !p.sym.ring1 && p.sym.sw >= 1 && state_order_of(c, p.sym.sw, order))
+            for (int q = 0; q < c->ns; ++q)
+                if (order[q] != q) out->state_grouping = 1;
+    }
+    return EMI_OK;
+}
+
+int emi_state_order(emi_ctx_t c, int sw, int* out) {
+    if (!c || !out) return EMI_ERR_ARG;
+    if (c->model < 0) return fail(c, EMI_ERR_STATE, "emi_state_order: the model must be set");
+    if (sw < 1 || c->ns % sw != 0) return fail(c, EMI_ERR_ARG, "emi_state_order: sw must divide the number of states");
+    if (!state_order_of(c, sw, out)) return fail(c, EMI_ERR_UNSUPPORTED, "emi_state_order: no state order for this model");
+    return EMI_OK;
+}
+
+int emi_model_state_order(int model, int sw, int* out) {
+    if (!out || sw < 1) return EMI_ERR_ARG;
+    return emi::ring_state_order(model, sw, out) ? EMI_OK : EMI_ERR_ARG;
 }
 
 int emi_last_path(emi_ctx_t c, int* fused) {
diff --git a/etol_amd/csrc/emi_kernels.hpp b/etol_amd/csrc/emi_kernels.hpp
--- a/etol_amd/csrc/emi_kernels.hpp
+++ b/etol_amd/csrc/emi_kernels.hpp
@@ -39,11 +39,13 @@
     size_t slab_bytes = 0;
     int cpart = 0, cx = 0;
     int tiles = 0;
+    int sgroup = 1;
 };
 SymPlan plan_symdefect(int ns, int B, int M, int ct, int ksplit_opt, int cpart_opt = 0, int gblk_opt = 0, int cx_opt = 0, int bk_opt = 8, int ct_cols = 1);
 hipError_t launch_symdefect(int model, const SymDefectArgs& a, hipStream_t s, bool set_attr, int ct, const SymPlan& plan);
 bool pass_supported(int model, int ns, int B, int M, const SymPlan& plan);
 hipError_t launch_pass(int model, const SymDefectArgs& sa, const NodeArgs<double>& na, hipStream_t s, const SymPlan& plan);
+bool ring_state_order(int model, int sw, int* out);
 
 struct AdjointArgs {
     const double* VALS;
@@ -91,6 +93,7 @@
 template <typename T> hipError_t rtc_launch_hess(RtcModel* m, const HessArgs<T>& a, hipStream_t s);
 hipError_t rtc_launch_symdefect(RtcModel* m, const SymDefectArgs& a, hipStream_t s);
 int rtc_pass_sw_large(const RtcModel* m);
+bool rtc_state_order(const RtcModel* m, int sw, int* out);
 bool rtc_pass_supported(const RtcModel* m, int B, int M, int sw, int ks, int store_mode);
 hipError_t rtc_launch_pass(RtcModel* m, const SymDefectArgs& sa, const NodeArgs<double>& na, int sw, hipStream_t s);
 hipError_t rtc_launch_nodes_nt(RtcModel* m, const NodeArgs<double>& a, hipStream_t s);
diff --git a/etol_amd/csrc/emi_models.hpp b/etol_amd/csrc/emi_models.hpp
--- a/etol_amd/csrc/emi_models.hpp
+++ b/etol_amd/csrc/emi_models.hpp
@@ -56,6 +56,9 @@
 
 template <typename T> struct Quadrotor2D {
     static constexpr int NS = 6, NC = 2, NV = 8, NPARAM = 5, NPATH = 0;
+    template <int SW> static constexpr int ring_state(int q) {
+        return SW == 2 ? (q == 2 ? 3 : (q == 3 ? 4 : (q == 4 ? 2 : q))) : q;
+    }
     EMI_DEV static void f(const ModelParams<T>& P, const T* z, T, T* fo) {
         T s, c;
         emi_sincos(z[2], &s, &c);
@@ -560,4 +563,17 @@
     }
 };
 
+template <class Model, int SW, class = void> struct RingOrder {
+    static constexpr int state(int q) { return q; }
+};
+template <class Model, int SW> struct RingOrder<Model, SW, decltype(void(Model::template ring_state<SW>(0)))> {
+    static constexpr int state(int q) { return Model::template ring_state<SW>(q); }
+};
+template <class Model, int SW> constexpr bool ring_order_is_contiguous(int n = Model::NS) {
+    return n == 0 || (RingOrder<Model, SW>::state(n - 1) == n - 1 && ring_order_is_contiguous<Model, SW>(n - 1));
 }
+template <class Model> struct ContiguousStates : Model {
+    template <int SW> static constexpr int ring_state(int q) { return q; }
+};
+
+}
diff --git a/etol_amd/csrc/emi_rtc.hip b/etol_amd/csrc/emi_rtc.hip
--- a/etol_amd/csrc/emi_rtc.hip
+++ b/etol_amd/csrc/emi_rtc.hip
@@ -24,6 +24,7 @@
     bool f32 = false;
     int ns = 0, nc = 0, sw_large = 0;
     size_t ring_lds = 0;
+    std::vector<int> order_large;
 };
 
 namespace {
@@ -79,6 +80,12 @@
              "emi::%s<double>::NPATH == %d, \"model struct dimensions differ from emi_set_model_source(ns, nc, npath)\");\n", sn, ns,
              sn, nc, sn, ns + nc, sn, npath);
     prog += chk;
+    if (with_ring) {
+        const std::string ro = std::string("emi::RingOrder<emi::") + sn + "<double>, " + std::to_string(pass_sw_large(ns)) + ">::state(";
+        prog += "extern \"C\" __device__ int emi_ring_order_large[" + std::to_string(ns) + "] = {";
+        for (int q = 0; q < ns; ++q) prog += (q ? ", " : "") + ro + std::to_string(q) + ")";
+        prog += "};\n";
+    }
     if (npath > 0) {
         snprintf(chk, sizeof chk, "static_assert(emi::%s<double>::PW == %d, \"the model's traced rows depend on another number of "
                  "variables than emi_set_model_source(n_path_vars) says\");\n", sn, pw);
@@ -209,6 +216,19 @@
         if (e == hipSuccess) e = hipModuleGetFunction(&m->pass_large, m->mod, low[i++].c_str());
         if (e == hipSuccess) e = hipModuleGetFunction(&m->node_nt, m->mod, low[i++].c_str());
         m->sw_large = pass_sw_large(ns);
+        hipDeviceptr_t dorder = nullptr;
+        size_t obytes = 0;
+        if (e == hipSuccess) e = hipModuleGetGlobal(&dorder, &obytes, m->mod, "emi_ring_order_large");
+        if (e == hipSuccess && obytes != (size_t)ns * sizeof(int)) e = hipErrorInvalidValue;
+        if (e == hipSuccess) {
+            m->order_large.resize(ns);
+            e = hipMemcpyDtoH(m->order_large.data(), dorder, obytes);
+        }
+        for (int q = 0; q < ns && e == hipSuccess; ++q) {
+            int seen = 0;
+            for (int r = 0; r < ns; ++r) seen += m->order_large[r] == q;
+            if (seen != 1) e = hipErrorInvalidValue;
+        }
     }
     if (e != hipSuccess) {
         if (log) *log = std::string("loading the model code object failed: ") + hipGetErrorString(e);
@@ -250,6 +270,12 @@
 }
 
 int rtc_pass_sw_large(const RtcModel* m) { return m ? m->sw_large : 0; }
+
+bool rtc_state_order(const RtcModel* m, int sw, int* out) {
+    if (!m || sw < 1 || m->ns % sw != 0) return false;
+    for (int q = 0; q < m->ns; ++q) out[q] = (sw == m->sw_large && sw > 1 && !m->order_large.empty()) ? m->order_large[q] : q;
+    return true;
+}
 
 bool rtc_pass_supported(const RtcModel* m, int B, int M, int sw, int ks, int store_mode) {
     if (!m || !m->pass_small || ks < 1 || M % 128 != 0) return false;
diff --git a/etol_amd/csrc/emi_symdefect.hip b/etol_amd/csrc/emi_symdefect.hip
--- a/etol_amd/csrc/emi_symdefect.hip
+++ b/etol_amd/csrc/emi_symdefect.hip
@@ -105,17 +105,24 @@
     return p;
 }
 
+template <class Model, int SW>
+static hipError_t launch_ring2_grouped(const SymDefectArgs& a, hipStream_t s, const SymPlan& p) {
+    if constexpr (!ring_order_is_contiguous<Model, SW>()) {
+        if (!p.sgroup) return launch_ring2_model<ContiguousStates<Model>, SW>(a, s);
+    }
+    return launch_ring2_model<Model, SW>(a, s);
+}
 template <class Model>
 static hipError_t launch_ring2_planned(const SymDefectArgs& a, hipStream_t s, const SymPlan& p) {
     constexpr int NS = Model::NS;
-    if (p.sw == NS) return launch_ring2_model<Model, NS>(a, s);
+    if (p.sw == NS) return launch_ring2_grouped<Model, NS>(a, s, p);
     if constexpr (NS > 2 && NS % 2 == 0) {
-        if (p.sw == 2) return launch_ring2_model<Model, 2>(a, s);
+        if (p.sw == 2) return launch_ring2_grouped<Model, 2>(a, s, p);
     }
     if constexpr (NS > 3 && NS % 3 == 0) {
-        if (p.sw == 3) return launch_ring2_model<Model, 3>(a, s);
-    }
-    return launch_ring2_model<Model, 1>(a, s);
+        if (p.sw == 3) return launch_ring2_grouped<Model, 3>(a, s, p);
+    }
+    return launch_ring2_grouped<Model, 1>(a, s, p);
 }
 
 template <class Model, int SW, int NST, int BK = 8, int CT = 1, int HS = 1>
@@ -147,22 +154,31 @@
     return hipGetLastError();
 }
 
+template <class Model, int SW>
+static hipError_t launch_pass_narrow(const SymDefectArgs& sa, const NodeArgs<double>& na, hipStream_t s, const SymPlan& p) {
+    if (p.hs == 2 && p.ct == 1) return p.bk == 16 ? launch_pass_model<Model, SW, 3, 16, 1, 2>(sa, na, s) : launch_pass_model<Model, SW, 3, 8, 1, 2>(sa, na, s);
+    if constexpr (SW == 2) {
+        if (p.ct == 2) return p.bk == 16 ? launch_pass_model<Model, 2, 3, 16, 2>(sa, na, s) : launch_pass_model<Model, 2, 3, 8, 2>(sa, na, s);
+    }
+    if (p.bk == 16) return launch_pass_model<Model, SW, 3, 16>(sa, na, s);
+    return p.nst > 3 ? launch_pass_model<Model, SW, 4>(sa, na, s) : launch_pass_model<Model, SW, 3>(sa, na, s);
+}
 template <class Model>
 static hipError_t launch_pass_planned(const SymDefectArgs& sa, const NodeArgs<double>& na, hipStream_t s, const SymPlan& p) {
     constexpr int NS = Model::NS;
     if (p.sw == NS) return launch_pass_model<Model, NS, 3>(sa, na, s);
     if constexpr (NS > 2 && NS % 2 == 0) {
-        if (p.sw == 2 && p.hs == 2 && p.ct == 1) return p.bk == 16 ? launch_pass_model<Model, 2, 3, 16, 1, 2>(sa, na, s) : launch_pass_model<Model, 2, 3, 8, 1, 2>(sa, na, s);
-        if (p.sw == 2 && p.ct == 2) return p.bk == 16 ? launch_pass_model<Model, 2, 3, 16, 2>(sa, na, s) : launch_pass_model<Model, 2, 3, 8, 2>(sa, na, s);
-        if (p.sw == 2 && p.bk == 16) return launch_pass_model<Model, 2, 3, 16>(sa, na, s);
-        if (p.sw == 2) return p.nst > 3 ? launch_pass_model<Model, 2, 4>(sa, na, s) : launch_pass_model<Model, 2, 3>(sa, na, s);
+        if (p.sw == 2) {
+            if constexpr (!ring_order_is_contiguous<Model, 2>()) {
+                if (!p.sgroup) return launch_pass_narrow<ContiguousStates<Model>, 2>(sa, na, s, p);
+            }
+            return launch_pass_narrow<Model, 2>(sa, na, s, p);
+        }
     }
     if constexpr (NS > 3 && NS % 3 == 0) {
         if (p.sw == 3) return launch_pass_model<Model, 3, 3>(sa, na, s);
     }
-    if (p.hs == 2) return p.bk == 16 ? launch_pass_model<Model, 1, 3, 16, 1, 2>(sa, na, s) : launch_pass_model<Model, 1, 3, 8, 1, 2>(sa, na, s);
-    if (p.bk == 16) return launch_pass_model<Model, 1, 3, 16>(sa, na, s);
-    return p.nst > 3 ? launch_pass_model<Model, 1, 4>(sa, na, s) : launch_pass_model<Model, 1, 3>(sa, na, s);
+    return launch_pass_narrow<Model, 1>(sa, na, s, p);
 }
 
 bool pass_supported(int model, int ns, int B, int M, const SymPlan& p) {
@@ -175,6 +191,26 @@
     if (model == EMI_MODEL_POINTMASS2D) return launch_pass_planned<PointMass2D<double>>(sa, na, s, p);
     if (model == EMI_MODEL_QUADROTOR2D) return launch_pass_planned<Quadrotor2D<double>>(sa, na, s, p);
     return hipErrorInvalidValue;
+}
+
+template <class Model, int SW> static void ring_order_into(int* out) {
+    for (int q = 0; q < Model::NS; ++q) out[q] = RingOrder<Model, SW>::state(q);
+}
+template <class Model> static bool ring_state_order_model(int sw, int* out) {
+    constexpr int NS = Model::NS;
+    if (sw < 1 || NS % sw != 0) return false;
+    if (sw == 2 && NS > 2) ring_order_into<Model, 2>(out);
+    else if (sw == 3 && NS > 3) ring_order_into<Model, 3>(out);
+    else if (sw == NS) ring_order_into<Model, NS>(out);
+    else if (sw == 1) ring_order_into<Model, 1>(out);
+    else for (int q = 0; q < NS; ++q) out[q] = q;
+    return true;
+}
+bool ring_state_order(int model, int sw, int* out) {
+    if (model == EMI_MODEL_POINTMASS2D) return ring_state_order_model<PointMass2D<double>>(sw, out);
+    if (model == EMI_MODEL_QUADROTOR2D) return ring_state_order_model<Quadrotor2D<double>>(sw, out);
+    if (model == EMI_MODEL_FIXEDWING12) return ring_state_order_model<FixedWing12<double>>(sw, out);
+    return false;
 }
 
 bool fused_supported(int model, int M, int ct) {
diff --git a/etol_amd/csrc/emi_symdefect_kernels.hpp b/etol_amd/csrc/emi_symdefect_kernels.hpp
--- a/etol_amd/csrc/emi_symdefect_kernels.hpp
+++ b/etol_amd/csrc/emi_symdefect_kernels.hpp
@@ -357,7 +357,8 @@
                 double f[NS];
                 Model::f(a.P, zz[i][side], side == 0 ? t_f : t_m, f);
                 const double dx = side == 0 ? acc_a[0][i] + acc_b[0][i] : acc_b[0][i] - acc_a[0][i];
-                Rb[(size_t)S0 * M + (side == 0 ? node_f : node_m)] = dx - a.h * f[S0];
+                constexpr int st = RingOrder<Model, SW>::state(S0);
+                Rb[(size_t)st * M + (side == 0 ? node_f : node_m)] = dx - a.h * f[st];
             }
         }
         return;
@@ -398,7 +399,7 @@
                 double f[NS];
                 Model::f(a.P, zc[side], side == 0 ? t_f : t_m, f);
 #pragma unroll
-                for (int s = 0; s < SW; ++s) hf[side][s] = a.h * f[S0 + s];
+                for (int s = 0; s < SW; ++s) hf[side][s] = a.h * f[RingOrder<Model, SW>::state(S0 + s)];
             }
 #pragma unroll
             for (int side = 0; side < 2; ++side) {
@@ -406,7 +407,7 @@
 #pragma unroll
                 for (int s = 0; s < SW; ++s) {
                     const double dx = side == 0 ? acc_a[s][i] + acc_b[s][i] : acc_b[s][i] - acc_a[s][i];
-                    Rb[(size_t)(S0 + s) * M + node] = dx - hf[side][s];
+                    Rb[(size_t)RingOrder<Model, SW>::state(S0 + s) * M + node] = dx - hf[side][s];
                 }
             }
         }
@@ -481,7 +482,8 @@
             int inst = inst0 + (rr & 15);
             inst = inst < B ? inst : B - 1;
             if (a.ablate & 8) inst &= 15;
-            voff[t] = (unsigned)((((size_t)inst * NS + s0 + (rr >> 4)) * M + 2 * c) * sizeof(double));
+            const int st = RingOrder<Model, SW>::state(s0 + (rr >> 4));
+            voff[t] = (unsigned)((((size_t)inst * NS + st) * M + 2 * c) * sizeof(double));
             gbase[t] = (unsigned long long)(a.X + (mir ? M - BK : 0));
             gstep[t] = mir ? -(int)(BK * sizeof(double)) : (int)(BK * sizeof(double));
         } else if (row0 < ROWS) {
diff --git a/etol_amd/evaluator.py b/etol_amd/evaluator.py
--- a/etol_amd/evaluator.py
+++ b/etol_amd/evaluator.py
@@ -326,6 +326,11 @@
         self._ck(self.lib.emi_plan_pass(self.ctx, int(B if B is not None else self.layout.B), C.byref(p)), "emi_plan_pass")
         return {n: getattr(p, n) for n, _ in L.PassPlan._fields_}
 
+    def state_order(self, sw):
+        out = (C.c_int * self.layout.ns)()
+        self._ck(self.lib.emi_state_order(self.ctx, int(sw), out), "emi_state_order")
+        return list(out)
+
     @property
     def last_defect_kernel(self):
         return self.lib.emi_last_defect_kernel(self.ctx).decode()
diff --git a/etol_amd/host/emi_trace.cpp b/etol_amd/host/emi_trace.cpp
--- a/etol_amd/host/emi_trace.cpp
+++ b/etol_amd/host/emi_trace.cpp
@@ -277,6 +277,85 @@
     return deps;
 }
 
+std::vector<int> Trace::state_order(int ns, const std::vector<int>& f, int sw) const {
+    std::vector<int> order(ns);
+    for (int q = 0; q < ns; ++q) order[q] = q;
+    if (sw <= 1 || sw >= ns || ns % sw != 0 || (int)f.size() < ns) return order;
+    auto weight = [](Op op) { return op == DIV || op == SQRT ? 16 : ((op >= SIN && op <= POWC && op != SQRT) ? 64 : 1); };
+    std::vector<std::map<std::pair<int, int>, int>> cost(ns);
+    for (int i = 0; i < ns; ++i) {
+        std::set<int> seen;
+        std::vector<int> stack = {f[i]};
+        while (!stack.empty()) {
+            const int n = stack.back();
+            stack.pop_back();
+            if (n < 0 || seen.count(n)) continue;
+            seen.insert(n);
+            const Node& nd = _nodes[n];
+            if (nd.op < ADD) continue;
+            const bool trig = nd.op == SIN || nd.op == COS || nd.op == TAN;
+            cost[i][trig ? std::make_pair(1, nd.a) : std::make_pair(0, n)] = weight(nd.op);
+            stack.push_back(nd.a);
+            if (nd.b >= 0) stack.push_back(nd.b);
+        }
+    }
+    std::vector<std::vector<long>> S(ns, std::vector<long>(ns, 0));
+    for (int i = 0; i < ns; ++i)
+        for (int j = i + 1; j < ns; ++j) {
+            long s = 0;
+            for (const auto& kv : cost[i])
+                if (cost[j].count(kv.first)) s += kv.second;
+            S[i][j] = S[j][i] = s;
+        }
+    std::vector<bool> placed(ns, false);
+    std::vector<std::vector<int>> bound;
+    for (;;) {
+        int bi = -1, bj = -1;
+        for (int i = 0; i < ns; ++i)
+            for (int j = i + 1; j < ns; ++j)
+                if (!placed[i] && !placed[j] && S[i][j] > 0 && (bi < 0 || S[i][j] > S[bi][bj])) { bi = i; bj = j; }
+        if (bi < 0) break;
+        std::vector<int> g = {bi, bj};
+        placed[bi] = placed[bj] = true;
+        while ((int)g.size() < sw) {
+            int bk = -1;
+            long best = 0;
+            for (int k = 0; k < ns; ++k) {
+                if (placed[k]) continue;
+                long s = 0;
+                for (int m : g) s += S[k][m];
+                if (s > best) { best = s; bk = k; }
+            }
+            if (bk < 0) break;
+            g.push_back(bk);
+            placed[bk] = true;
+        }
+        bound.push_back(g);
+    }
+    if (bound.empty()) return order;
+    const int nslots = ns / sw;
+    std::vector<std::vector<int>> slot(nslots);
+    std::sort(bound.begin(), bound.end(), [](const std::vector<int>& a, const std::vector<int>& b) {
+        return *std::min_element(a.begin(), a.end()) < *std::min_element(b.begin(), b.end());
+    });
+    for (const std::vector<int>& g : bound) {
+        int s = *std::min_element(g.begin(), g.end()) / sw;
+        while (!slot[s].empty()) s = (s + 1) % nslots;
+        slot[s] = g;
+    }
+    int next = 0;
+    for (int s = 0; s < nslots; ++s) {
+        while ((int)slot[s].size() < sw) {
+            while (placed[next]) ++next;
+            slot[s].push_back(next);
+            placed[next] = true;
+        }
+        std::sort(slot[s].begin(), slot[s].end());
+        for (int q = 0; q < sw; ++q) order[s * sw + q] = slot[s][q];
+    }
+    return order;
+}
+
 std::string Trace::generate_model(const std::string& name, int ns, int nc, const std::vector<int>& f, int L,
                                   const std::vector<int>& paths, std::vector<int>* path_vars, std::string* err) {
     const int nv = ns + nc;
@@ -373,6 +452,19 @@
         for (int q = 0; q + 1 < pw; ++q) o << "q == " << q << " ? " << pv[q] << " : ";
         o << pv[pw - 1] << "; }\n";
     }
+    o << "    template <int SW> static constexpr int ring_state(int q) { return ";
+    for (int sw = 2; sw < ns; ++sw) {
+        if (ns % sw != 0) continue;
+        const std::vector<int> order = state_order(ns, f, sw);
+        bool same = true;
+        for (int q = 0; q < ns; ++q) same = same && order[q] == q;
+        if (same) continue;
+        o << "SW == " << sw << " ? (";
+        for (int q = 0; q < ns; ++q)
+            if (order[q] != q) o << "q == " << q << " ? " << order[q] << " : ";
+        o << "q) : ";
+    }
+    o << "q; }\n";
     o << "    EMI_DEV static void f(const ModelParams<T>&, const T* z, T tk, T* fo) {\n";
     {
         std::vector<std::string> t;
diff --git a/etol_amd/host/emi_trace.hpp b/etol_amd/host/emi_trace.hpp
--- a/etol_amd/host/emi_trace.hpp
+++ b/etol_amd/host/emi_trace.hpp
@@ -34,6 +34,7 @@
                                const std::vector<int>& paths = {}, std::vector<int>* path_vars = nullptr,
                                std::string* err = nullptr);
     std::vector<int> dependencies(int out, int ns, int nc);
+    std::vector<int> state_order(int ns, const std::vector<int>& f, int sw) const;
 
     double eval(int node, const std::vector<double>& x, const std::vector<double>& u, double t,
                 const std::vector<double>& coef = {}) const;
diff --git a/include/emi355x.h b/include/emi355x.h
--- a/include/emi355x.h
+++ b/include/emi355x.h
@@ -120,8 +120,11 @@
   int k_tile;
   int column_tiles;
   int k_halves;
+  int state_grouping;
 } emi_pass_plan_t;
 int emi_plan_pass(emi_ctx_t ctx, int B, emi_pass_plan_t* out);
+int emi_state_order(emi_ctx_t ctx, int sw, int* out);
+int emi_model_state_order(int model, int sw, int* out);
 
 int emi_jac_structure(emi_ctx_t ctx, int* rows, int* cols);
 
```

Result: no change. 5.158 billion, median of 5 (+0.4%).
